# jondo2010/rust-ida

Hardware: AMD Instinct MI355X
Metric: Newton iters/sec (fp64), batched dense DAE N=512 B=4096 (higher is better)
Workload: dtype f64

## Files before the change

### bindings/rust/ida-hip-sys/src/lib.rs

```rust
#![allow(non_camel_case_types, non_upper_case_globals)]
use std::os::raw::{c_char, c_double, c_int, c_long, c_void};

#[repr(C)]
pub struct idahip_ctx {
    _private: [u8; 0],
}
#[repr(C)]
pub struct idaens {
    _private: [u8; 0],
}

pub type idahip_res_fn = Option<
    unsafe extern "C" fn(sys: c_int, tt: c_double, yy: *const c_double, yp: *const c_double, resval: *mut c_double, user: *mut c_void) -> c_int,
>;
pub type idahip_jac_fn = Option<
    unsafe extern "C" fn(
        sys: c_int,
        tt: c_double,
        cj: c_double,
        yy: *const c_double,
        yp: *const c_double,
        resvec: *const c_double,
        jac: *mut c_double,
        user: *mut c_void,
    ) -> c_int,
>;
pub type idahip_band_jac_fn = Option<
    unsafe extern "C" fn(
        sys: c_int,
        tt: c_double,
        cj: c_double,
        yy: *const c_double,
        yp: *const c_double,
        resvec: *const c_double,
        jac: *mut c_double,
        ldab: c_int,
        user: *mut c_void,
    ) -> c_int,
>;
pub type idaens_root_fn = Option<
    unsafe extern "C" fn(user: *mut c_void, sys: i32, t: c_double, yy: *const c_double, yp: *const c_double, nroots: i32, gout: *mut c_double) -> c_int,
>;

#[repr(C)]
pub struct idahip_root_state {
    pub glo: [c_double; 4],
    pub ghi: [c_double; 4],
    pub grout: [c_double; 4],
    pub iroots: [c_double; 4],
    pub gactive: [i32; 4],
}

#[repr(C)]
pub struct idahip_tiny_call {
    pub touts: *const c_double,
    pub ntout: c_int,
    pub recycle: c_int,
    pub resume: c_int,
    pub max_rounds: c_long,
    pub mxstep: c_long,
    pub maxord: c_int,
    pub maxnef: c_long,
    pub maxncf: c_long,
    pub epcon: c_double,
    pub hmax_inv: c_double,
    pub t0: c_double,
    pub start_round: *const i64,
    pub round_base: i64,
    pub nroots: c_int,
    pub root_comps: *const i32,
    pub root_thresholds: *const c_double,
    pub root_states: *mut idahip_root_state,
}

pub const IDAHIP_ROBERTS: c_int = 0;
pub const IDAHIP_LORENZ63: c_int = 1;
pub const IDAHIP_LINEAR_DENSE: c_int = 2;
pub const IDAHIP_HEAT1D: c_int = 3;
pub const IDAHIP_HOST_CALLBACK: c_int = 4;
pub const IDAHIP_F_YY: c_int = 0;
pub const IDAHIP_F_YP: c_int = 1;
pub const IDAHIP_F_YYPREDICT: c_int = 2;
pub const IDAHIP_F_YPPREDICT: c_int = 3;
pub const IDAHIP_F_EWT: c_int = 4;
pub const IDAHIP_F_EE: c_int = 5;
pub const IDAHIP_F_DELTA: c_int = 6;
pub const IDAHIP_F_SAVRES: c_int = 7;
pub const IDAHIP_F_PHI0: c_int = 8;
pub const IDAHIP_F_PHI5: c_int = 13;
pub const IDAHIP_LS_DIRECT: c_int = 0;
pub const IDAHIP_LS_ITERATIVE: c_int = 1;
pub const IDAHIP_LS_MATRIX_ITERATIVE: c_int = 2;
pub const IDAHIP_K_NEWTON_ITER: c_int = 0;
pub const IDAHIP_K_SYS: c_int = 1;
pub const IDAHIP_K_JAC: c_int = 2;
pub const IDAHIP_K_LU: c_int = 3;
pub const IDAHIP_K_VECTOR: c_int = 4;
pub const IDAHIP_K_SOLVE: c_int = 5;
pub const IDAHIP_K_SYS_JAC: c_int = 6;
pub const IDAHIP_K_LU_PANEL: c_int = 7;
pub const IDAHIP_K_LU_TRAIL: c_int = 8;
pub const IDAHIP_K_LU_FINALIZE: c_int = 9;
pub const IDAHIP_K_COUNT: c_int = 10;

pub const IDAENS_NORMAL: c_int = 0;
pub const IDAENS_ONE_STEP: c_int = 1;
pub const IDAENS_SUCCESS: c_int = 0;
pub const IDAENS_TSTOP_RETURN: c_int = 1;
pub const IDAENS_ROOT_RETURN: c_int = 2;
pub const IDAENS_UNFINISHED: c_int = 99;
pub const IDAENS_TOO_MUCH_WORK: c_int = -1;
pub const IDAENS_TOO_MUCH_ACC: c_int = -2;
pub const IDAENS_ERR_FAIL: c_int = -3;
pub const IDAENS_CONV_FAIL: c_int = -4;
pub const IDAENS_LSETUP_FAIL: c_int = -6;
pub const IDAENS_CLOSE_ROOTS: c_int = -10;
pub const IDAENS_RTFUNC_FAIL: c_int = -12;
pub const IDAENS_ILL_INPUT: c_int = -22;
pub const IDAENS_BAD_K: c_int = -25;
pub const IDAENS_BAD_T: c_int = -26;
pub const IDAENS_C_NST: c_int = 0;
pub const IDAENS_C_NRE: c_int = 1;
pub const IDAENS_C_NJE: c_int = 2;
pub const IDAENS_C_NSETUPS: c_int = 3;
pub const IDAENS_C_NNI: c_int = 4;
pub const IDAENS_C_NETF: c_int = 5;
pub const IDAENS_C_NCFN: c_int = 6;
pub const IDAENS_C_NATTEMPTS: c_int = 7;
pub const IDAENS_C_NLS_NCONVFAILS: c_int = 8;
pub const IDAENS_C_KUSED: c_int = 9;
pub const IDAENS_C_KK: c_int = 10;
pub const IDAENS_C_NGE: c_int = 11;
pub const IDAENS_C_NLUFAIL: c_int = 12;
pub const IDAENS_C_NCONV_JCUR: c_int = 13;
pub const IDAENS_C_NFAIL_FIRST: c_int = 14;
pub const IDAENS_C_NLI: c_int = 15;
pub const IDAENS_C_NCFL: c_int = 16;
pub const IDAENS_C_NRE_DQ: c_int = 17;
pub const IDAENS_R_TN: c_int = 0;
pub const IDAENS_R_HUSED: c_int = 1;
pub const IDAENS_R_HH: c_int = 2;
pub const IDAENS_R_H0U: c_int = 3;
pub const IDAENS_R_TOLSF: c_int = 4;

#[link(name = "idahip")]
extern "C" {
    pub fn idahip_create(ctx: *mut *mut idahip_ctx, device: c_int, n: c_int, batch: c_int, kind: c_int, hip_stream: *mut c_void) -> c_int;
    pub fn idahip_destroy(ctx: *mut idahip_ctx) -> c_int;
    pub fn idahip_create_band(ctx: *mut *mut idahip_ctx, device: c_int, n: c_int, batch: c_int, kind: c_int, hip_stream: *mut c_void, ml: c_int, mu: c_int) -> c_int;
    pub fn idahip_band(ctx: *const idahip_ctx, ml: *mut c_int, mu: *mut c_int) -> c_int;
    pub fn idahip_set_host_band_problem(ctx: *mut idahip_ctx, res: idahip_res_fn, bjac: idahip_band_jac_fn, user: *mut c_void) -> c_int;
    pub fn idahip_download_lu_band(ctx: *mut idahip_ctx, sys: c_int, h_ab: *mut c_double, h_piv: *mut i64) -> c_int;
    pub fn idahip_ls_setup_band(ctx: *mut idahip_ctx, ml: c_int, mu: c_int, d_ab: *mut c_double, d_piv: *mut i64, h_info: *mut i32, h_idx: *const i32, nsys: c_int) -> c_int;
    pub fn idahip_ls_solve_band(ctx: *mut idahip_ctx, ml: c_int, mu: c_int, d_ab: *const c_double, d_piv: *const i64, d_x: *mut c_double, d_b: *const c_double, tol: c_double, h_idx: *const i32, nsys: c_int) -> c_int;
    pub fn idahip_concurrent_streams(device: c_int, count: c_int, streams_out: *mut *mut c_void, nconcurrent: *mut c_int) -> c_int;
    pub fn idahip_release_streams(device: c_int, count: c_int, streams: *mut *mut c_void) -> c_int;
    pub fn idahip_stream_pair_share(device: c_int, stream_a: *mut c_void, stream_b: *mut c_void, frac: *mut c_double) -> c_int;
    pub fn idahip_last_error(ctx: *const idahip_ctx) -> *const c_char;
    pub fn idahip_sync(ctx: *mut idahip_ctx) -> c_int;
    pub fn idahip_n(ctx: *const idahip_ctx) -> c_int;
    pub fn idahip_batch(ctx: *const idahip_ctx) -> c_int;
    pub fn idahip_kind(ctx: *const idahip_ctx) -> c_int;
    pub fn idahip_set_tolerances(ctx: *mut idahip_ctx, rtol: c_double, h_atol: *const c_double, natol: c_int) -> c_int;
    pub fn idahip_set_problem_params(ctx: *mut idahip_ctx, first: c_int, count: c_int, h_params: *const c_double, nparam: c_int) -> c_int;
    pub fn idahip_set_linear_dense(ctx: *mut idahip_ctx, first: c_int, count: c_int, h_a: *const c_double, h_b: *const c_double, h_c: *const c_double) -> c_int;
    pub fn idahip_set_host_problem(ctx: *mut idahip_ctx, res: idahip_res_fn, jac: idahip_jac_fn, user: *mut c_void) -> c_int;
    pub fn idahip_upload(ctx: *mut idahip_ctx, f: c_int, first: c_int, count: c_int, h: *const c_double) -> c_int;
    pub fn idahip_download(ctx: *mut idahip_ctx, f: c_int, first: c_int, count: c_int, h: *mut c_double) -> c_int;
    pub fn idahip_download_lu(ctx: *mut idahip_ctx, sys: c_int, h_lu: *mut c_double, h_piv: *mut i64) -> c_int;
    pub fn idahip_dev_alloc(ctx: *mut idahip_ctx, bytes: usize) -> *mut c_void;
    pub fn idahip_dev_free(ctx: *mut idahip_ctx, d: *mut c_void) -> c_int;
    pub fn idahip_memcpy_h2d(ctx: *mut idahip_ctx, d: *mut c_void, h: *const c_void, bytes: usize) -> c_int;
    pub fn idahip_memcpy_d2h(ctx: *mut idahip_ctx, h: *mut c_void, d: *const c_void, bytes: usize) -> c_int;
    pub fn idahip_ls_setup(ctx: *mut idahip_ctx, d_a: *mut c_double, d_piv: *mut i64, h_info: *mut i32, h_idx: *const i32, nsys: c_int) -> c_int;
    pub fn idahip_ls_solve(ctx: *mut idahip_ctx, d_lu: *const c_double, d_piv: *const i64, d_x: *mut c_double, d_b: *const c_double, tol: c_double, h_idx: *const i32, nsys: c_int) -> c_int;
    pub fn idahip_ls_type(ctx: *const idahip_ctx) -> c_int;
    pub fn idahip_ls_num_iters(ctx: *const idahip_ctx) -> c_int;
    pub fn idahip_ls_res_norm(ctx: *const idahip_ctx) -> c_double;
    pub fn idahip_wrms(ctx: *mut idahip_ctx, d_x: *const c_double, d_w: *const c_double, h_out: *mut c_double, h_idx: *const i32, nsys: c_int) -> c_int;
    pub fn idahip_nls_sys_setup(ctx: *mut idahip_ctx, h_tn: *const c_double, h_cj: *const c_double, reset_ee: c_int, h_info: *mut i32, h_idx: *const i32, nsys: c_int) -> c_int;
    pub fn idahip_nls_sys(ctx: *mut idahip_ctx, h_tn: *const c_double, h_cj: *const c_double, reset_ee: c_int, h_idx: *const i32, nsys: c_int) -> c_int;
    pub fn idahip_nls_lsetup(ctx: *mut idahip_ctx, h_tn: *const c_double, h_cj: *const c_double, h_info: *mut i32, h_idx: *const i32, nsys: c_int) -> c_int;
    pub fn idahip_set_jacobian_dq(ctx: *mut idahip_ctx, on: c_int) -> c_int;
    pub fn idahip_jacobian_dq(ctx: *const idahip_ctx) -> c_int;
    pub fn idahip_set_host_residual(ctx: *mut idahip_ctx, res: idahip_res_fn, user: *mut c_void) -> c_int;
    pub fn idahip_nls_lsetup_dq(ctx: *mut idahip_ctx, h_tn: *const c_double, h_cj: *const c_double, h_hh: *const c_double, h_info: *mut i32, h_idx: *const i32, nsys: c_int) -> c_int;
    pub fn idahip_jac_dq(ctx: *mut idahip_ctx, h_tn: *const c_double, h_cj: *const c_double, h_hh: *const c_double, h_j: *mut c_double, h_idx: *const i32, nsys: c_int) -> c_int;
    pub fn idahip_newton_iter(ctx: *mut idahip_ctx, h_scale: *const c_double, h_delnrm: *mut c_double, h_idx: *const i32, nsys: c_int) -> c_int;
    pub fn idahip_newton_iter2(ctx: *mut idahip_ctx, h_scale: *const c_double, h_tn: *const c_double, h_cj: *const c_double, h_toldel: *const c_double, h_ss: *const c_double, h_eps_newt: *const c_double, h_delnrm: *mut c_double, h_conv: *mut i32, h_idx: *const i32, nsys: c_int) -> c_int;
    pub fn idahip_init_first(ctx: *mut idahip_ctx, h_ypnorm: *mut c_double, h_phi0_nrm: *mut c_double, h_idx: *const i32, nsys: c_int) -> c_int;
    pub fn idahip_scale_phi1(ctx: *mut idahip_ctx, h_fac: *const c_double, h_idx: *const i32, nsys: c_int) -> c_int;
    pub fn idahip_predict(ctx: *mut idahip_ctx, h_kk_ns: *const i32, h_beta: *const c_double, h_gamma: *const c_double, h_idx: *const i32, nsys: c_int) -> c_int;
    pub fn idahip_post_newton(ctx: *mut idahip_ctx, h_cj: *const c_double, h_kk: *const i32, h_norms: *mut c_double, h_idx: *const i32, nsys: c_int) -> c_int;
    pub fn idahip_restore(ctx: *mut idahip_ctx, h_kk_ns: *const i32, h_cvals: *const c_double, h_idx: *const i32, nsys: c_int) -> c_int;
    pub fn idahip_complete_step(ctx: *mut idahip_ctx, h_kused: *const i32, h_ck: *const c_double, maxord: c_int, h_phi0_nrm: *mut c_double, h_ewt_bad: *mut i32, h_idx: *const i32, nsys: c_int) -> c_int;
    pub fn idahip_get_solution(ctx: *mut idahip_ctx, h_kord: *const i32, h_cvals: *const c_double, h_dvals: *const c_double, h_idx: *const i32, nsys: c_int) -> c_int;
    pub fn idahip_get_dky(ctx: *mut idahip_ctx, h_kfirst: *const i32, h_klast: *const i32, h_cjk: *const c_double, h_out: *mut c_double, h_idx: *const i32, nsys: c_int) -> c_int;
    pub fn idahip_snapshot_initial(ctx: *mut idahip_ctx) -> c_int;
    pub fn idahip_restore_initial(ctx: *mut idahip_ctx, h_idx: *const i32, nsys: c_int) -> c_int;
    pub fn idahip_tiny_solve(ctx: *mut idahip_ctx, h_sys: *mut c_void, sys_bytes: usize, call: *const idahip_tiny_call, h_rounds_done: *mut i64, h_acc: *mut u64, h_yout: *mut c_double, h_ypout: *mut c_double) -> c_int;
    pub fn idahip_pow_batch(ctx: *mut idahip_ctx, h_x: *const c_double, h_y: *const c_double, h_out: *mut c_double, count: usize) -> c_int;
    pub fn idahip_round_solve(ctx: *mut idahip_ctx, h_sys: *mut c_void, sys_bytes: usize, call: *const idahip_tiny_call, h_rounds_done: *mut i64, h_acc: *mut u64, h_yout: *mut c_double, h_ypout: *mut c_double, rounds_run: *mut i64) -> c_int;
    pub fn idahip_set_lu_variant(ctx: *mut idahip_ctx, variant: c_int) -> c_int;
    pub fn idahip_lu_variant(ctx: *const idahip_ctx) -> c_int;
    pub fn idahip_set_lu_superpanel(ctx: *mut idahip_ctx, on: c_int) -> c_int;
    pub fn idahip_lu_superpanel(ctx: *const idahip_ctx) -> c_int;
    pub fn idahip_set_lu_period(ctx: *mut idahip_ctx, rounds: c_int) -> c_int;
    pub fn idahip_lu_period(ctx: *const idahip_ctx) -> c_int;
    pub fn idahip_timing_build() -> c_int;
    pub fn idahip_timing_enable(ctx: *mut idahip_ctx, on: c_int) -> c_int;
    pub fn idahip_timing_get(ctx: *mut idahip_ctx, k: c_int, ms: *mut c_double, launches: *mut i64, systems: *mut i64) -> c_int;
    pub fn idahip_timing_reset(ctx: *mut idahip_ctx) -> c_int;
}

#[link(name = "idaens")]
extern "C" {
    pub fn idaens_create(e: *mut *mut idaens, ctx: *mut idahip_ctx, h_yy0: *const c_double, h_yp0: *const c_double) -> c_int;
    pub fn idaens_destroy(e: *mut idaens) -> c_int;
    pub fn idaens_last_error(e: *const idaens) -> *const c_char;
    pub fn idaens_set_max_num_steps(e: *mut idaens, mxstep: c_long) -> c_int;
    pub fn idaens_set_max_ord(e: *mut idaens, maxord: c_int) -> c_int;
    pub fn idaens_set_fused_newton(e: *mut idaens, on: c_int) -> c_int;
    pub fn idaens_set_device_controller(e: *mut idaens, on: c_int) -> c_int;
    pub fn idaens_device_controller_active(e: *const idaens) -> c_int;
    pub fn idaens_set_roots(e: *mut idaens, nroots: c_int, comps: *const i32, thresholds: *const c_double) -> c_int;
    pub fn idaens_get_roots(e: *const idaens, out: *mut i32) -> c_int;
    pub fn idaens_set_root_fn(e: *mut idaens, nroots: c_int, fn_: idaens_root_fn, user: *mut c_void) -> c_int;
    pub fn idaens_solve(e: *mut idaens, tout: c_double, itask: c_int, h_tret: *mut c_double, h_status: *mut i32, max_rounds: c_long) -> c_int;
    pub fn idaens_solve_schedule(e: *mut idaens, touts: *const c_double, ntout: c_int, h_tret: *mut c_double, h_status: *mut i32, h_reached: *mut i32, h_yout: *mut c_double, h_ypout: *mut c_double, max_rounds: c_long) -> c_int;
    pub fn idaens_stream(e: *mut idaens, touts: *const c_double, ntout: c_int, max_rounds: c_long, stagger_rounds: c_long, passes_done: *mut i64) -> c_int;
    pub fn idaens_stream_group(ens: *mut *mut idaens, ngroups: c_int, touts: *const c_double, ntout: c_int, max_rounds: c_long, stagger_rounds: c_long, offset_us: c_long, passes_done: *mut i64) -> c_int;
    pub fn idaens_solve_schedule_group(ens: *mut *mut idaens, ngroups: c_int, touts: *const c_double, ntout: c_int, h_tret: *mut *mut c_double, h_status: *mut *mut i32, h_reached: *mut *mut i32, max_rounds: c_long) -> c_int;
    pub fn idaens_get_counter(e: *const idaens, which: c_int, out: *mut i64) -> c_int;
    pub fn idaens_get_real(e: *const idaens, which: c_int, out: *mut c_double) -> c_int;
    pub fn idaens_get_yy(e: *mut idaens, h_yy: *mut c_double) -> c_int;
    pub fn idaens_get_yp(e: *mut idaens, h_yp: *mut c_double) -> c_int;
    pub fn idaens_get_dky(e: *mut idaens, t: c_double, k: c_int, h_dky: *mut c_double, h_status: *mut i32) -> c_int;
    pub fn idaens_total_newton_iters(e: *const idaens) -> i64;
    pub fn idaens_total_rounds(e: *const idaens) -> i64;
    pub fn idaens_trace_system(e: *mut idaens, sys: c_int) -> c_int;
    pub fn idaens_trace_len(e: *const idaens) -> c_long;
    pub fn idaens_trace_get(e: *const idaens, out: *mut c_double) -> c_int;
}
```

### include/ida_hip.h

```cpp
#ifndef IDA_HIP_H
#define IDA_HIP_H

#include <stddef.h>
#include <stdint.h>

#ifdef __cplusplus
extern "C" {
#endif

typedef struct idahip_ctx idahip_ctx;

typedef enum {
    IDAHIP_ROBERTS = 0,
    IDAHIP_LORENZ63 = 1,
    IDAHIP_LINEAR_DENSE = 2,
    IDAHIP_HEAT1D = 3,
    IDAHIP_HOST_CALLBACK = 4
} idahip_problem;

typedef int (*idahip_res_fn)(int sys, double tt, const double* yy, const double* yp, double* resval, void* user);
typedef int (*idahip_jac_fn)(int sys, double tt, double cj, const double* yy, const double* yp, const double* resvec, double* J,
                             void* user);

typedef int (*idahip_band_jac_fn)(int sys, double tt, double cj, const double* yy, const double* yp, const double* resvec, double* AB,
                                  int ldab, void* user);

typedef enum {
    IDAHIP_F_YY = 0,
    IDAHIP_F_YP = 1,
    IDAHIP_F_YYPREDICT = 2,
    IDAHIP_F_YPPREDICT = 3,
    IDAHIP_F_EWT = 4,
    IDAHIP_F_EE = 5,
    IDAHIP_F_DELTA = 6,
    IDAHIP_F_SAVRES = 7,
    IDAHIP_F_PHI0 = 8,
    IDAHIP_F_PHI5 = 13
} idahip_field;

int idahip_create(idahip_ctx** ctx, int device, int n, int batch, idahip_problem kind, void* hip_stream );
int idahip_destroy(idahip_ctx* ctx);
int idahip_create_band(idahip_ctx** ctx, int device, int n, int batch, idahip_problem kind, void* hip_stream, int ml, int mu);
int idahip_band(const idahip_ctx* ctx, int* ml, int* mu);
int idahip_set_host_band_problem(idahip_ctx* ctx, idahip_res_fn res, idahip_band_jac_fn bjac, void* user);
int idahip_download_lu_band(idahip_ctx* ctx, int sys, double* hAB, int64_t* hPiv);
int idahip_ls_setup_band(idahip_ctx* ctx, int ml, int mu, double* dAB, int64_t* dPiv, int32_t* hInfo, const int32_t* hIdx, int nsys);
int idahip_ls_solve_band(idahip_ctx* ctx, int ml, int mu, const double* dAB, const int64_t* dPiv, double* dX, const double* dB, double tol,
                         const int32_t* hIdx, int nsys);
int idahip_concurrent_streams(int device, int count, void** streams_out, int* nconcurrent);
int idahip_release_streams(int device, int count, void** streams);
int idahip_stream_pair_share(int device, void* streamA, void* streamB, double* frac);
const char* idahip_last_error(const idahip_ctx* ctx);
int idahip_sync(idahip_ctx* ctx);
int idahip_n(const idahip_ctx* ctx);
int idahip_batch(const idahip_ctx* ctx);
int idahip_kind(const idahip_ctx* ctx);

int idahip_set_tolerances(idahip_ctx* ctx, double rtol, const double* hAtol, int natol);
int idahip_set_problem_params(idahip_ctx* ctx, int first, int count, const double* hParams, int nparam);
int idahip_set_linear_dense(idahip_ctx* ctx, int first, int count, const double* hA, const double* hB, const double* hC);
int idahip_set_host_problem(idahip_ctx* ctx, idahip_res_fn res, idahip_jac_fn jac, void* user);
int idahip_upload(idahip_ctx* ctx, idahip_field f, int first, int count, const double* h);
int idahip_download(idahip_ctx* ctx, idahip_field f, int first, int count, double* h);
int idahip_download_lu(idahip_ctx* ctx, int sys, double* hLU, int64_t* hPiv);

void* idahip_dev_alloc(idahip_ctx* ctx, size_t bytes);
int idahip_dev_free(idahip_ctx* ctx, void* d);
int idahip_memcpy_h2d(idahip_ctx* ctx, void* d, const void* h, size_t bytes);
int idahip_memcpy_d2h(idahip_ctx* ctx, void* h, const void* d, size_t bytes);

int idahip_ls_setup(idahip_ctx* ctx, double* dA, int64_t* dPiv, int32_t* hInfo, const int32_t* hIdx, int nsys);
int idahip_ls_solve(idahip_ctx* ctx, const double* dLU, const int64_t* dPiv, double* dX, const double* dB, double tol,
                    const int32_t* hIdx, int nsys);
typedef enum { IDAHIP_LS_DIRECT = 0, IDAHIP_LS_ITERATIVE = 1, IDAHIP_LS_MATRIX_ITERATIVE = 2 } idahip_ls_kind;
int idahip_ls_type(const idahip_ctx* ctx);
int idahip_ls_num_iters(const idahip_ctx* ctx);
double idahip_ls_res_norm(const idahip_ctx* ctx);
int idahip_wrms(idahip_ctx* ctx, const double* dX, const double* dW, double* hOut, const int32_t* hIdx, int nsys);

int idahip_nls_sys_setup(idahip_ctx* ctx, const double* hTn, const double* hCj, int reset_ee, int32_t* hInfo,
                         const int32_t* hIdx, int nsys);

int idahip_nls_sys(idahip_ctx* ctx, const double* hTn, const double* hCj, int reset_ee, const int32_t* hIdx, int nsys);
int idahip_nls_lsetup(idahip_ctx* ctx, const double* hTn, const double* hCj, int32_t* hInfo, const int32_t* hIdx, int nsys);

int idahip_set_jacobian_dq(idahip_ctx* ctx, int on);
int idahip_jacobian_dq(const idahip_ctx* ctx);
int idahip_set_host_residual(idahip_ctx* ctx, idahip_res_fn res, void* user);
int idahip_nls_lsetup_dq(idahip_ctx* ctx, const double* hTn, const double* hCj, const double* hHh, int32_t* hInfo, const int32_t* hIdx,
                         int nsys);
int idahip_jac_dq(idahip_ctx* ctx, const double* hTn, const double* hCj, const double* hHh, double* hJ, const int32_t* hIdx, int nsys);
int idahip_newton_iter(idahip_ctx* ctx, const double* hScale, double* hDelnrm, const int32_t* hIdx, int nsys);
int idahip_newton_iter2(idahip_ctx* ctx, const double* hScale, const double* hTn, const double* hCj, const double* hToldel,
                        const double* hSs, const double* hEpsNewt, double* hDelnrm, int32_t* hConv, const int32_t* hIdx, int nsys);

int idahip_init_first(idahip_ctx* ctx, double* hYpnorm, double* hPhi0Nrm, const int32_t* hIdx, int nsys);
int idahip_scale_phi1(idahip_ctx* ctx, const double* hFac, const int32_t* hIdx, int nsys);
int idahip_predict(idahip_ctx* ctx, const int32_t* hKkNs, const double* hBeta, const double* hGamma, const int32_t* hIdx, int nsys);
int idahip_post_newton(idahip_ctx* ctx, const double* hCj, const int32_t* hKk, double* hNorms, const int32_t* hIdx, int nsys);
int idahip_restore(idahip_ctx* ctx, const int32_t* hKkNs, const double* hCvals, const int32_t* hIdx, int nsys);
int idahip_complete_step(idahip_ctx* ctx, const int32_t* hKused, const double* hCk, int maxord, double* hPhi0Nrm,
                         int32_t* hEwtBad, const int32_t* hIdx, int nsys);
int idahip_get_solution(idahip_ctx* ctx, const int32_t* hKord, const double* hCvals, const double* hDvals,
                        const int32_t* hIdx, int nsys);
int idahip_get_dky(idahip_ctx* ctx, const int32_t* hKfirst, const int32_t* hKlast, const double* hCjk , double* hOut,
                   const int32_t* hIdx, int nsys);

int idahip_snapshot_initial(idahip_ctx* ctx);
int idahip_restore_initial(idahip_ctx* ctx, const int32_t* hIdx, int nsys);

#define IDAHIP_MAX_ROOTS 4
typedef struct idahip_root_state {
    double glo[IDAHIP_MAX_ROOTS], ghi[IDAHIP_MAX_ROOTS], grout[IDAHIP_MAX_ROOTS], iroots[IDAHIP_MAX_ROOTS];
    int32_t gactive[IDAHIP_MAX_ROOTS];
} idahip_root_state;
typedef struct idahip_tiny_call {
    const double* touts;
    int ntout;
    int recycle;
    int resume;
    long max_rounds;
    long mxstep;
    int maxord;
    long maxnef, maxncf;
    double epcon, hmax_inv, t0;
    const int64_t* start_round;
    int64_t round_base;
    int nroots;
    const int32_t* root_comps;
    const double* root_thresholds;
    idahip_root_state* root_states;
} idahip_tiny_call;
int idahip_tiny_solve(idahip_ctx* ctx, void* hSys, size_t sys_bytes, const idahip_tiny_call* call, int64_t* hRoundsDone, uint64_t* hAcc,
                      double* hYout, double* hYPout);
int idahip_pow_batch(idahip_ctx* ctx, const double* hX, const double* hY, double* hOut, size_t count);
int idahip_round_solve(idahip_ctx* ctx, void* hSys, size_t sys_bytes, const idahip_tiny_call* call, int64_t* hRoundsDone, uint64_t* hAcc,
                       double* hYout, double* hYPout, int64_t* rounds_run);

int idahip_set_lu_variant(idahip_ctx* ctx, int variant);
int idahip_lu_variant(const idahip_ctx* ctx);
int idahip_set_lu_superpanel(idahip_ctx* ctx, int on);
int idahip_lu_superpanel(const idahip_ctx* ctx);
int idahip_set_lu_period(idahip_ctx* ctx, int rounds);
int idahip_lu_period(const idahip_ctx* ctx);
int idahip_timing_build(void);

typedef enum {
    IDAHIP_K_NEWTON_ITER = 0, IDAHIP_K_SYS = 1, IDAHIP_K_JAC = 2, IDAHIP_K_LU = 3, IDAHIP_K_VECTOR = 4, IDAHIP_K_SOLVE = 5,
    IDAHIP_K_SYS_JAC = 6,
    IDAHIP_K_LU_PANEL = 7,
    IDAHIP_K_LU_TRAIL = 8,
    IDAHIP_K_LU_FINALIZE = 9,
    IDAHIP_K_COUNT = 10
} idahip_kclass;
int idahip_timing_enable(idahip_ctx* ctx, int on);
int idahip_timing_get(idahip_ctx* ctx, idahip_kclass k, double* ms, int64_t* launches, int64_t* systems);
int idahip_timing_reset(idahip_ctx* ctx);

#ifdef __cplusplus
}
#endif
#endif
```

### rust-ida_amd/csrc/common.hpp

```cpp
#pragma once
#include <hip/hip_runtime.h>

#include <cstdarg>
#include <cstdlib>
#include <cstdint>
#include <cstdio>
#include <cstring>
#include <string>
#include <type_traits>
#include <vector>

#include "../../include/ida_hip.h"
#include "exp_switches.hpp"

namespace idahip {

constexpr int MXORDP1 = 6;
constexpr int TINY_N = 8;
constexpr int LU_NB = 32;
constexpr int LU_MAX_N = 1024;
constexpr int LU_WIDE_ROWS = 2048;
constexpr int LU_ZMAP_MIN_N = 2048;
constexpr int LU_BIG_MAX_N = 4096;
constexpr int NSLOT = 8;

struct Slot {
    char* h = nullptr;
    char* d = nullptr;
    hipEvent_t done = nullptr;
    bool pending = false;
};

}

struct idahip_ctx {
    int device = 0;
    int n = 0;
    int batch = 0;
    int npad16 = 0;
    int simds = 0;
    idahip_problem kind = IDAHIP_ROBERTS;
    hipStream_t stream = nullptr;
    bool own_stream = false;
    std::string err;

    double rtol = 0.0;
    double atol_s = 0.0;
    double* d_atol_v = nullptr;

    double *yy = nullptr, *yp = nullptr, *yypredict = nullptr, *yppredict = nullptr, *ewt = nullptr, *ee = nullptr,
           *delta = nullptr, *savres = nullptr;
    double* phi = nullptr;

    double* lu = nullptr;
    double* jw = nullptr;
    int64_t* piv = nullptr;
    int32_t* perm = nullptr;
    int32_t *lu_pos = nullptr, *lu_live = nullptr, *lu_prow = nullptr, *lu_info = nullptr, *lu_redo = nullptr, *lu_nzb = nullptr, *lu_bz = nullptr;
    int32_t* lu_jwzero = nullptr;
    uint8_t* lu_dirty = nullptr;
    uint8_t* lu_zmap = nullptr;
    double* lu_l11 = nullptr;
    int band = 0, ml = 0, mu = 0, ldab = 0;
    double* bab = nullptr;
    double *ic_y = nullptr, *ic_yp = nullptr;
    double* dky = nullptr;
    int lu_variant = 4;
    int lu_superpanel = 0;
    int lu_period = 1;

    void* tiny_sys = nullptr;
    double *tiny_touts = nullptr, *tiny_yout = nullptr, *tiny_ypout = nullptr;
    int64_t *tiny_start = nullptr, *tiny_rounds = nullptr;
    uint64_t* tiny_acc = nullptr;
    void* tiny_roots = nullptr;
    int tiny_ntout_cap = 0, tiny_yout_cap = 0;

    int32_t* rnd_i = nullptr;
    double* rnd_d = nullptr;
    int32_t* rnd_host = nullptr;

    unsigned long long* dbg_stamps = nullptr;

    double* params = nullptr;
    int nparam = 0;
    double *A = nullptr, *B = nullptr, *C = nullptr;
    idahip_res_fn cb_res = nullptr;
    idahip_jac_fn cb_jac = nullptr;
    idahip_band_jac_fn cb_bjac = nullptr;
    void* cb_user = nullptr;
    double* cb_stage = nullptr;
    std::vector<double> cb_host;
    double *cb_jpin = nullptr, *cb_jdev = nullptr;
    size_t cb_jcap = 0;
    int jac_dq = 0;
    int dq_locked = 0;
    double* dq_stage = nullptr;
    size_t dq_stage_cap = 0;
    double* dq_out = nullptr;
    size_t dq_out_cap = 0;
    double* dq_hh = nullptr;

    std::vector<uint64_t> list_seen;

    idahip::Slot slots[idahip::NSLOT];
    size_t slot_cap = 0;
    int next_slot = 0;

    int timing = 0;
    hipEvent_t ev0 = nullptr, ev1 = nullptr, ev2 = nullptr, ev3 = nullptr;
    hipEvent_t ev_cnt = nullptr;
    double k_ms[IDAHIP_K_COUNT] = {0};
    int64_t k_launches[IDAHIP_K_COUNT] = {0};
    int64_t k_systems[IDAHIP_K_COUNT] = {0};
};

namespace idahip {

inline int fail(idahip_ctx* c, int code, const char* fmt, ...) {
    char buf[512];
    va_list ap;
    va_start(ap, fmt);
    vsnprintf(buf, sizeof buf, fmt, ap);
    va_end(ap);
    if (c) c->err = buf;
    return code;
}

#define IDAHIP_HIP(c, call)                                                                              \
    do {                                                                                                 \
        hipError_t e__ = (call);                                                                         \
        if (e__ != hipSuccess) return idahip::fail((c), -100, "%s failed: %s", #call, hipGetErrorString(e__)); \
    } while (0)

struct DevGuard {
    int prev = -1;
    bool switched = false;
    explicit DevGuard(int dev) {
        if (dev >= 0 && hipGetDevice(&prev) == hipSuccess && prev != dev) switched = hipSetDevice(dev) == hipSuccess;
    }
    explicit DevGuard(const idahip_ctx* c) : DevGuard(c ? c->device : -1) {}
    ~DevGuard() {
        if (switched) (void)hipSetDevice(prev);
    }
    DevGuard(const DevGuard&) = delete;
    DevGuard& operator=(const DevGuard&) = delete;
};

struct ArgPack {
    idahip_ctx* c;
    Slot* s;
    size_t in_bytes = 0;
    size_t off = 0;
    size_t out_begin = 0, out_end = 0;
    bool overflow = false;

    int begin(idahip_ctx* ctx) {
        c = ctx;
        s = &ctx->slots[ctx->next_slot];
        ctx->next_slot = (ctx->next_slot + 1) % NSLOT;
        if (s->pending) {
            IDAHIP_HIP(c, hipEventSynchronize(s->done));
            s->pending = false;
        }
        off = 0;
        return 0;
    }
    static size_t align(size_t x) { return (x + 63) & ~(size_t)63; }
    template <class T>
    const T* in(const T* src, size_t count) {
        off = align(off);
        if (off + count * sizeof(T) > c->slot_cap) {
            overflow = true;
            return (const T*)s->d;
        }
        memcpy(s->h + off, src, count * sizeof(T));
        const T* d = (const T*)(s->d + off);
        off += count * sizeof(T);
        in_bytes = off;
        return d;
    }
    int upload() {
        if (overflow) return fail(c, -5, "argument staging slot too small (%zu bytes)", c->slot_cap);
        if (in_bytes) IDAHIP_HIP(c, hipMemcpyAsync(s->d, s->h, in_bytes, hipMemcpyHostToDevice, c->stream));
        return 0;
    }
    template <class T>
    T* out(size_t count) {
        off = align(off);
        if (off + count * sizeof(T) > c->slot_cap) {
            overflow = true;
            return nullptr;
        }
        if (out_begin == 0 && out_end == 0) out_begin = off;
        T* d = (T*)(s->d + off);
        off += count * sizeof(T);
        out_end = off;
        return d;
    }
    template <class T>
    const T* host_of(const T* dptr) const { return (const T*)(s->h + ((const char*)dptr - s->d)); }
    int ok() { return overflow ? fail(c, -5, "argument staging slot too small (%zu bytes)", c->slot_cap) : 0; }
    int fetch() {
        if (overflow) return ok();
        if (out_end > out_begin)
            IDAHIP_HIP(c, hipMemcpyAsync(s->h + out_begin, s->d + out_begin, out_end - out_begin, hipMemcpyDeviceToHost, c->stream));
        IDAHIP_HIP(c, hipStreamSynchronize(c->stream));
        return 0;
    }
    int finish_async() {
        IDAHIP_HIP(c, hipEventRecord(s->done, c->stream));
        s->pending = true;
        return 0;
    }
};

struct KTimer {
    idahip_ctx* c;
    idahip_kclass k;
    bool on;
    hipEvent_t e0, e1;
    KTimer(idahip_ctx* ctx, idahip_kclass kc, int nsys) : c(ctx), k(kc) {
        const bool sub = kc >= IDAHIP_K_LU_PANEL;
        on = sub ? c->timing >= 2 : c->timing >= 1;
        e0 = sub ? c->ev2 : c->ev0;
        e1 = sub ? c->ev3 : c->ev1;
        c->k_launches[k] += 1;
        c->k_systems[k] += nsys;
        if (on) (void)hipEventRecord(e0, c->stream);
    }
    ~KTimer() {
        if (on) {
            (void)hipEventRecord(e1, c->stream);
            (void)hipEventSynchronize(e1);
            float ms = 0.f;
            (void)hipEventElapsedTime(&ms, e0, e1);
            c->k_ms[k] += (double)ms;
        }
    }
};

template <class T>
__device__ __forceinline__ T ldc(const T* p) {
    typedef const T __attribute__((address_space(4))) * cptr;
    return *reinterpret_cast<cptr>(reinterpret_cast<uintptr_t>(p));
}

__device__ __forceinline__ double readlane_f64(double v, int lane ) {
    const int lo = __builtin_amdgcn_readlane(__double2loint(v), lane);
    const int hi = __builtin_amdgcn_readlane(__double2hiint(v), lane);
    return __hiloint2double(hi, lo);
}

template <int CTRL, int ROW_MASK>
__device__ __forceinline__ int dpp_mov_i32(int x) {
    return __builtin_amdgcn_update_dpp(x, x, CTRL, ROW_MASK, 0xf, false);
}
template <int CTRL, int ROW_MASK>
__device__ __forceinline__ double dpp_mov_f64(double x) {
    const int lo = dpp_mov_i32<CTRL, ROW_MASK>(__double2loint(x));
    const int hi = dpp_mov_i32<CTRL, ROW_MASK>(__double2hiint(x));
    return __hiloint2double(hi, lo);
}
__device__ __forceinline__ double wave_max_f64(double v) {
    double o;
    o = dpp_mov_f64<0x111, 0xf>(v); v = o > v ? o : v;
    o = dpp_mov_f64<0x112, 0xf>(v); v = o > v ? o : v;
    o = dpp_mov_f64<0x114, 0xf>(v); v = o > v ? o : v;
    o = dpp_mov_f64<0x118, 0xf>(v); v = o > v ? o : v;
    o = dpp_mov_f64<0x142, 0xa>(v); v = o > v ? o : v;
    o = dpp_mov_f64<0x143, 0xc>(v); v = o > v ? o : v;
    const int lo = __builtin_amdgcn_readlane(__double2loint(v), 63);
    const int hi = __builtin_amdgcn_readlane(__double2hiint(v), 63);
    return __hiloint2double(hi, lo);
}
__device__ __forceinline__ int wave_min_i32(int v) {
    int o;
    o = dpp_mov_i32<0x111, 0xf>(v); v = o < v ? o : v;
    o = dpp_mov_i32<0x112, 0xf>(v); v = o < v ? o : v;
    o = dpp_mov_i32<0x114, 0xf>(v); v = o < v ? o : v;
    o = dpp_mov_i32<0x118, 0xf>(v); v = o < v ? o : v;
    o = dpp_mov_i32<0x142, 0xa>(v); v = o < v ? o : v;
    o = dpp_mov_i32<0x143, 0xc>(v); v = o < v ? o : v;
    return __builtin_amdgcn_readlane(v, 63);
}

template <int CTRL, int ROW_MASK>
__device__ __forceinline__ unsigned dpp_umax(unsigned x) {
    const unsigned o = (unsigned)__builtin_amdgcn_update_dpp(0, (int)x, CTRL, ROW_MASK, 0xf, true);
    return o > x ? o : x;
}
template <int CTRL, int ROW_MASK>
__device__ __forceinline__ int dpp_imin(int x) {
    const int o = __builtin_amdgcn_update_dpp(0x7fffffff, x, CTRL, ROW_MASK, 0xf, false);
    return o < x ? o : x;
}
template <bool ROWS16>
__device__ __forceinline__ unsigned wave_max_u32(unsigned v) {
    v = dpp_umax<0x111, 0xf>(v);
    v = dpp_umax<0x112, 0xf>(v);
    v = dpp_umax<0x114, 0xf>(v);
    v = dpp_umax<0x118, 0xf>(v);
    if (ROWS16) return (unsigned)__builtin_amdgcn_readlane((int)v, 15);
    v = dpp_umax<0x142, 0xa>(v);
    v = dpp_umax<0x143, 0xc>(v);
    return (unsigned)__builtin_amdgcn_readlane((int)v, 63);
}
template <bool ROWS16>
__device__ __forceinline__ int wave_min_i32f(int v) {
    v = dpp_imin<0x111, 0xf>(v);
    v = dpp_imin<0x112, 0xf>(v);
    v = dpp_imin<0x114, 0xf>(v);
    v = dpp_imin<0x118, 0xf>(v);
    if (ROWS16) return __builtin_amdgcn_readlane(v, 15);
    v = dpp_imin<0x142, 0xa>(v);
    v = dpp_imin<0x143, 0xc>(v);
    return __builtin_amdgcn_readlane(v, 63);
}

template <int I, int N, class F>
__device__ __forceinline__ void static_for(F&& f) {
    if constexpr (I < N) {
        f(std::integral_constant<int, I>{});
        static_for<I + 1, N>(f);
    }
}

__device__ __forceinline__ double upd(double a, double u, double l) { return a - u * l; }

__device__ __forceinline__ double buf_load_f64(__amdgpu_buffer_rsrc_t rsrc, unsigned voffset, int soffset) {
    typedef unsigned v2u __attribute__((ext_vector_type(2)));
    const v2u r = __builtin_amdgcn_raw_buffer_load_b64(rsrc, (int)voffset, soffset, 0);
    return __hiloint2double((int)r.y, (int)r.x);
}

__device__ __forceinline__ void buf_store_f64(__amdgpu_buffer_rsrc_t rsrc, unsigned voffset, int soffset, double v) {
    typedef unsigned v2u __attribute__((ext_vector_type(2)));
    v2u d;
    d.x = (unsigned)__double2loint(v);
    d.y = (unsigned)__double2hiint(v);
    __builtin_amdgcn_raw_buffer_store_b64(d, rsrc, (int)voffset, soffset, 0);
}

__device__ __forceinline__ double shfl_xor_f64(double v, int mask) {
    const int lo = __shfl_xor(__double2loint(v), mask);
    const int hi = __shfl_xor(__double2hiint(v), mask);
    return __hiloint2double(hi, lo);
}

}
```

### rust-ida_amd/csrc/idahip.hip

```cpp
#include "common.hpp"
#include "lu_kernels.hpp"
#include "lu_driver.hpp"
#include "problem_kernels.hpp"
#include "solve_kernels.hpp"
#include "band_kernels.hpp"
#include "dq_kernels.hpp"
#include "vector_kernels.hpp"
#include "tiny_ida.hpp"
#include "round_ida.hpp"

using namespace idahip;

namespace {

template <class T>
int dalloc(idahip_ctx* c, T** p, size_t count) {
    *p = nullptr;
    if (count == 0) return 0;
    IDAHIP_HIP(c, hipMalloc((void**)p, count * sizeof(T)));
    return 0;
}

int check_list(idahip_ctx* c, const int32_t* hIdx, int nsys) {
    if (!c) return -1;
    if (nsys < 0 || nsys > c->batch) return fail(c, -2, "nsys = %d out of range (batch = %d)", nsys, c->batch);
    if (nsys > 0 && !hIdx) return fail(c, -2, "null system list");
    for (int s = 0; s < nsys; ++s)
        if (hIdx[s] < 0 || hIdx[s] >= c->batch) return fail(c, -2, "system id %d out of range at list position %d", hIdx[s], s);
    uint64_t* seen = c->list_seen.data();
    int dup = -1;
    for (int s = 0; s < nsys && dup < 0; ++s) {
        const uint64_t bit = 1ull << (hIdx[s] & 63);
        if (seen[hIdx[s] >> 6] & bit) dup = s;
        seen[hIdx[s] >> 6] |= bit;
    }
    for (int s = 0; s < (dup < 0 ? nsys : dup); ++s) seen[hIdx[s] >> 6] = 0;
    if (dup >= 0) return fail(c, -2, "system id %d listed twice (again at list position %d)", hIdx[dup], dup);
    return 0;
}

double* field_ptr(idahip_ctx* c, idahip_field f) {
    switch (f) {
        case IDAHIP_F_YY: return c->yy;
        case IDAHIP_F_YP: return c->yp;
        case IDAHIP_F_YYPREDICT: return c->yypredict;
        case IDAHIP_F_YPPREDICT: return c->yppredict;
        case IDAHIP_F_EWT: return c->ewt;
        case IDAHIP_F_EE: return c->ee;
        case IDAHIP_F_DELTA: return c->delta;
        case IDAHIP_F_SAVRES: return c->savres;
        default: break;
    }
    if (f >= IDAHIP_F_PHI0 && f <= IDAHIP_F_PHI5) return c->phi + (size_t)(f - IDAHIP_F_PHI0) * c->batch * c->n;
    return nullptr;
}

VecState vec_state(idahip_ctx* c) {
    VecState s;
    s.phi = c->phi;
    s.phistride = (long)c->batch * c->n;
    s.yy = c->yy; s.yp = c->yp; s.yypredict = c->yypredict; s.yppredict = c->yppredict;
    s.ewt = c->ewt; s.ee = c->ee; s.delta = c->delta;
    s.n = c->n;
    s.rtol = c->rtol; s.atol_s = c->atol_s; s.atol_v = c->d_atol_v;
    return s;
}

int post_launch(idahip_ctx* c, const char* what) {
    hipError_t e = hipGetLastError();
    if (e != hipSuccess) return fail(c, -101, "launch of %s failed: %s", what, hipGetErrorString(e));
    return 0;
}

int band_spw(const idahip_ctx* c, int nsys) {
    int spw = 64;
    const int simds = c->simds > 0 ? c->simds : 1024;
    while (spw > 1 && (long)(nsys + spw / 2 - 1) / (spw / 2) <= simds) spw >>= 1;
    if (const char* e = std::getenv("IDAHIP_BAND_SPW")) {
        const int v = (int)std::strtol(e, nullptr, 10);
        if (v == 1 || v == 2 || v == 4 || v == 8 || v == 16 || v == 32 || v == 64) spw = v;
    }
    return spw;
}

int band_factor(idahip_ctx* c, double* dAB, long sstride, int64_t* dPiv, long pstride, int ml, int mu, const int* d_idx, int nsys,
                const int* d_cnt = nullptr) {
    if (nsys == 0) return 0;
    BandArgs g;
    g.ab = dAB; g.sstride = sstride; g.piv = (long long*)dPiv; g.pstride = pstride; g.n = c->n; g.ml = ml; g.mu = mu;
    g.idx = d_idx; g.nsys = nsys; g.cnt = d_cnt; g.info = c->lu_info;
    const int spw = band_spw(c, nsys);
    const dim3 grid((nsys + spw - 1) / spw), blk(spw);
    if (ml == 1 && mu == 1) hipLaunchKernelGGL((band_getrf_reg_kernel<1, 1>), grid, blk, 0, c->stream, g);
    else hipLaunchKernelGGL(band_getrf_kernel, grid, blk, 0, c->stream, g);
    return post_launch(c, "band_getrf");
}

int create_ctx(idahip_ctx** out, int device, int n, int batch, idahip_problem kind, void* hip_stream, bool band, int ml, int mu) {
    if (!out) return -1;
    *out = nullptr;
    if (n < 1 || batch < 1) return -2;
    if ((int)kind < 0 || (int)kind > (int)IDAHIP_HOST_CALLBACK) return -2;
    if ((kind == IDAHIP_ROBERTS || kind == IDAHIP_LORENZ63) && n != 3) return -2;
    idahip_ctx* c = new idahip_ctx();
    c->device = device; c->n = n; c->batch = batch; c->kind = kind;
    if (band) {
        c->band = 1; c->ml = ml; c->mu = mu; c->ldab = 2 * ml + mu + 1;
    }
    c->npad16 = (n + 15) & ~15;
    c->list_seen.assign(((size_t)batch + 63) / 64, 0);
    c->lu_superpanel = kind == IDAHIP_HEAT1D ? 1 : 0;
    if (const char* sp = std::getenv("IDAHIP_LU_SUPERPANEL")) c->lu_superpanel = std::strtol(sp, nullptr, 10) != 0 ? 1 : 0;
    if (const char* sp = std::getenv("IDAHIP_LU_PERIOD")) {
        const int v = (int)std::strtol(sp, nullptr, 10);
        if (v >= 1 && v <= 64) c->lu_period = v;
    }
    int ndev = 0;
    if (device < 0 || hipGetDeviceCount(&ndev) != hipSuccess || device >= ndev) { delete c; return -100; }
    DevGuard dev_guard__(device);
    if (hipSetDevice(device) != hipSuccess) { delete c; return -100; }
    {
        int cus = 0;
        if (hipDeviceGetAttribute(&cus, hipDeviceAttributeMultiprocessorCount, device) == hipSuccess && cus > 0) c->simds = 4 * cus;
    }
    if (hip_stream) {
        c->stream = (hipStream_t)hip_stream;
    } else {
        if (hipStreamCreate(&c->stream) != hipSuccess) { delete c; return -100; }
        c->own_stream = true;
    }
    const size_t bn = (size_t)batch * n, bnn = bn * n;
    int rc = 0;
    rc |= dalloc(c, &c->yy, bn); rc |= dalloc(c, &c->yp, bn); rc |= dalloc(c, &c->yypredict, bn); rc |= dalloc(c, &c->yppredict, bn);
    rc |= dalloc(c, &c->ewt, bn); rc |= dalloc(c, &c->ee, bn); rc |= dalloc(c, &c->delta, bn); rc |= dalloc(c, &c->savres, bn);
    rc |= dalloc(c, &c->phi, (size_t)MXORDP1 * bn);
    rc |= dalloc(c, &c->piv, bn); rc |= dalloc(c, &c->perm, bn);
    rc |= dalloc(c, &c->lu_info, (size_t)batch);
    rc |= dalloc(c, &c->lu_redo, (size_t)batch);
    rc |= dalloc(c, &c->lu_nzb, (size_t)batch);
    if (band) rc |= dalloc(c, &c->bab, bn * c->ldab);
    if (!band) rc |= dalloc(c, &c->lu, bnn);
    if (!band && n > LU_MAX_N) rc |= dalloc(c, &c->lu_bz, (size_t)batch * 64);
    if (!band && n >= LU_ZMAP_MIN_N) rc |= dalloc(c, &c->lu_zmap, (size_t)batch * 4096);
    if (!band && n >= LU_ZMAP_MIN_N) rc |= dalloc(c, &c->lu_dirty, (size_t)batch * 4096);
    if (!band && n >= LU_ZMAP_MIN_N) rc |= dalloc(c, &c->lu_jwzero, (size_t)batch);
    if (!band && n > TINY_N) {
        rc |= dalloc(c, &c->jw, bnn);
        rc |= dalloc(c, &c->lu_pos, bn); rc |= dalloc(c, &c->lu_live, bn); rc |= dalloc(c, &c->lu_prow, bn);
        rc |= dalloc(c, &c->lu_l11, (size_t)batch * L11_STRIDE);
    }
    if (kind == IDAHIP_LINEAR_DENSE) {
        rc |= dalloc(c, &c->A, bnn); rc |= dalloc(c, &c->B, bnn); rc |= dalloc(c, &c->C, bn);
    }
    if (kind == IDAHIP_LORENZ63) { c->nparam = 3; rc |= dalloc(c, &c->params, (size_t)batch * 3); }
    if (kind == IDAHIP_HEAT1D) { c->nparam = 1; rc |= dalloc(c, &c->params, (size_t)batch); }
    if (kind == IDAHIP_HOST_CALLBACK) rc |= dalloc(c, &c->cb_stage, 3 * bn);
    c->slot_cap = (size_t)batch * 256 + 4096;
    for (int i = 0; i < NSLOT && !rc; ++i) {
        if (hipHostMalloc((void**)&c->slots[i].h, c->slot_cap) != hipSuccess) rc = -100;
        else if (hipMalloc((void**)&c->slots[i].d, c->slot_cap) != hipSuccess) rc = -100;
        else if (hipEventCreateWithFlags(&c->slots[i].done, hipEventDisableTiming) != hipSuccess) rc = -100;
    }
    if (!rc && (hipEventCreate(&c->ev0) != hipSuccess || hipEventCreate(&c->ev1) != hipSuccess || hipEventCreate(&c->ev2) != hipSuccess ||
                hipEventCreate(&c->ev3) != hipSuccess || hipEventCreateWithFlags(&c->ev_cnt, hipEventDisableTiming) != hipSuccess))
        rc = -100;

    if (rc) {
        idahip_destroy(c);
        return -100;
    }
    (void)hipMemsetAsync(c->ee, 0, bn * sizeof(double), c->stream);
    (void)hipMemsetAsync(c->delta, 0, bn * sizeof(double), c->stream);
    (void)hipMemsetAsync(c->phi, 0, (size_t)MXORDP1 * bn * sizeof(double), c->stream);
    (void)hipMemsetAsync(c->lu_info, 0, (size_t)batch * sizeof(int), c->stream);
    (void)hipMemsetAsync(c->piv, 0, bn * sizeof(int64_t), c->stream);
    (void)hipMemsetAsync(c->perm, 0, bn * sizeof(int32_t), c->stream);
    (void)hipMemsetAsync(c->lu_redo, 0, (size_t)batch * sizeof(int), c->stream);
    if (c->bab) (void)hipMemsetAsync(c->bab, 0, bn * c->ldab * sizeof(double), c->stream);
    if (c->lu_dirty) {
        (void)hipMemsetAsync(c->lu, 0, bnn * sizeof(double), c->stream);
        (void)hipMemsetAsync(c->lu_dirty, 0, (size_t)batch * 4096, c->stream);
        (void)hipMemsetAsync(c->lu_jwzero, 0, (size_t)batch * sizeof(int), c->stream);
    }
    (void)hipStreamSynchronize(c->stream);
    *out = c;
    return 0;
}

}

extern "C" {

int idahip_create(idahip_ctx** out, int device, int n, int batch, idahip_problem kind, void* hip_stream) {
    return create_ctx(out, device, n, batch, kind, hip_stream, false, 0, 0);
}

int idahip_create_band(idahip_ctx** out, int device, int n, int batch, idahip_problem kind, void* hip_stream, int ml, int mu) {
    if (!out) return -1;
    *out = nullptr;
    if (kind != IDAHIP_HEAT1D && kind != IDAHIP_HOST_CALLBACK) {
        std::fprintf(stderr, "idahip_create_band: problem kind %d has no band form (IDAHIP_HEAT1D or IDAHIP_HOST_CALLBACK)\n", (int)kind);
        return -2;
    }
    if (n <= TINY_N || n > LU_BIG_MAX_N) {
        std::fprintf(stderr, "idahip_create_band: n = %d outside %d < n <= %d\n", n, TINY_N, LU_BIG_MAX_N);
        return -2;
    }
    if (ml < 0 || mu < 0 || ml >= n || mu >= n || (kind == IDAHIP_HEAT1D && (ml < 1 || mu < 1))) {
        std::fprintf(stderr, "idahip_create_band: bandwidths ml = %d, mu = %d outside 0 <= ml, mu < n (>= 1 for IDAHIP_HEAT1D)\n", ml, mu);
        return -2;
    }
    return create_ctx(out, device, n, batch, kind, hip_stream, true, ml, mu);
}

int idahip_band(const idahip_ctx* c, int* ml, int* mu) {
    if (!c) return -1;
    if (c->band) {
        if (ml) *ml = c->ml;
        if (mu) *mu = c->mu;
    }
    return c->band;
}

int idahip_destroy(idahip_ctx* c) {
    DevGuard dev_guard__(c);
    if (!c) return 0;
    if (c->stream) (void)hipStreamSynchronize(c->stream);
    void* ptrs[] = {c->dq_stage, c->dq_out, c->dq_hh, c->yy, c->yp, c->yypredict, c->yppredict, c->ewt, c->ee, c->delta, c->savres, c->phi, c->lu, c->jw, c->piv, c->perm,
                    c->lu_pos, c->lu_live, c->lu_prow, c->lu_info, c->lu_redo, c->lu_nzb, c->lu_bz, c->lu_zmap, c->lu_dirty, c->lu_jwzero, c->lu_l11, c->params, c->A, c->B, c->C, c->d_atol_v, c->ic_y,
                    c->ic_yp, c->bab, c->dky, c->cb_stage, c->tiny_sys, c->tiny_touts, c->tiny_yout, c->tiny_ypout, c->tiny_start, c->tiny_rounds,
                    c->tiny_acc, c->tiny_roots, c->rnd_i, c->rnd_d};
    for (void* p : ptrs)
        if (p) (void)hipFree(p);
    if (c->rnd_host) (void)hipHostFree(c->rnd_host);
    if (c->cb_jpin) (void)hipHostFree(c->cb_jpin);
    if (c->cb_jdev) (void)hipFree(c->cb_jdev);
    for (int i = 0; i < NSLOT; ++i) {
        if (c->slots[i].h) (void)hipHostFree(c->slots[i].h);
        if (c->slots[i].d) (void)hipFree(c->slots[i].d);
        if (c->slots[i].done) (void)hipEventDestroy(c->slots[i].done);
    }
    if (c->ev0) (void)hipEventDestroy(c->ev0);
    if (c->ev1) (void)hipEventDestroy(c->ev1);
    if (c->ev2) (void)hipEventDestroy(c->ev2);
    if (c->ev3) (void)hipEventDestroy(c->ev3);
    if (c->ev_cnt) (void)hipEventDestroy(c->ev_cnt);
    if (c->own_stream && c->stream) (void)hipStreamDestroy(c->stream);
    delete c;
    return 0;
}

const char* idahip_last_error(const idahip_ctx* c) { return c ? c->err.c_str() : "null ctx"; }
int idahip_n(const idahip_ctx* c) { return c ? c->n : -1; }
int idahip_batch(const idahip_ctx* c) { return c ? c->batch : -1; }

int idahip_sync(idahip_ctx* c) {
    DevGuard dev_guard__(c);
    if (!c) return -1;
    IDAHIP_HIP(c, hipStreamSynchronize(c->stream));
    return 0;
}

__global__ void stream_probe_kernel(unsigned long long* out, long long ticks) {
    const unsigned long long t0 = wall_clock64();
    while ((long long)(wall_clock64() - t0) < ticks) __builtin_amdgcn_s_sleep(16);
    if (threadIdx.x == 0) {
        out[0] = t0;
        out[1] = wall_clock64();
    }
}

int idahip_concurrent_streams(int device, int count, void** streams_out, int* nconcurrent) {
    if (!streams_out || count < 1 || count > 64) return -2;
    int ndev = 0;
    if (device < 0 || hipGetDeviceCount(&ndev) != hipSuccess || device >= ndev) return -100;
    DevGuard dev_guard__(device);
    if (hipSetDevice(device) != hipSuccess) return -100;
    unsigned long long* stamps = nullptr;
    if (hipHostMalloc((void**)&stamps, sizeof(unsigned long long) * 2 * (size_t)(count + 1)) != hipSuccess) return -100;
    std::vector<hipStream_t> sel, rejected;
    int rc = 0;
    const long long ticks = 30000;
    for (int attempt = 0; attempt < 6 * count + 8 && (int)sel.size() < count && !rc; ++attempt) {
        hipStream_t s = nullptr;
        if (hipStreamCreateWithFlags(&s, hipStreamNonBlocking) != hipSuccess) { rc = -100; break; }
        if (sel.empty()) {
            sel.push_back(s);
            continue;
        }
        const int k = (int)sel.size();
        for (int i = 0; i <= k; ++i) stamps[2 * i] = stamps[2 * i + 1] = 0ull;
        for (int i = 0; i < k; ++i) hipLaunchKernelGGL(stream_probe_kernel, dim3(1), dim3(64), 0, sel[i], stamps + 2 * i, ticks);
        hipLaunchKernelGGL(stream_probe_kernel, dim3(1), dim3(64), 0, s, stamps + 2 * k, ticks);
        bool ok = hipGetLastError() == hipSuccess;
        for (int i = 0; i < k; ++i) ok = (hipStreamSynchronize(sel[i]) == hipSuccess) && ok;
        ok = (hipStreamSynchronize(s) == hipSuccess) && ok;
        if (!ok) { rc = -100; (void)hipStreamDestroy(s); break; }
        bool overlaps_all = stamps[2 * k + 1] > stamps[2 * k];
        for (int i = 0; i < k; ++i)
            overlaps_all = overlaps_all && stamps[2 * k] < stamps[2 * i + 1] && stamps[2 * i] < stamps[2 * k + 1];
        (overlaps_all ? sel : rejected).push_back(s);
    }
    const int found = (int)sel.size();
    while (!rc && (int)sel.size() < count) {
        if (!rejected.empty()) {
            sel.push_back(rejected.back());
            rejected.pop_back();
        } else {
            hipStream_t s = nullptr;
            if (hipStreamCreateWithFlags(&s, hipStreamNonBlocking) != hipSuccess) rc = -100;
            else sel.push_back(s);
        }
    }
    for (hipStream_t s : rejected) (void)hipStreamDestroy(s);
    (void)hipHostFree(stamps);
    if (rc) {
        for (hipStream_t s : sel) (void)hipStreamDestroy(s);
        return rc;
    }
    for (int i = 0; i < count; ++i) streams_out[i] = (void*)sel[i];
    if (nconcurrent) *nconcurrent = found;
    return 0;
}

__global__ void stream_share_kernel(unsigned long long* out, long long ticks) {
    extern __shared__ unsigned char pad_lds[];
    const unsigned long long t0 = wall_clock64();
    if (threadIdx.x == 0) pad_lds[0] = 1;
    while ((long long)(wall_clock64() - t0) < ticks) __builtin_amdgcn_s_sleep(16);
    if (threadIdx.x == 0) {
        atomicMin(out, t0);
        atomicMax(out + 1, wall_clock64());
    }
}

int idahip_stream_pair_share(int device, void* streamA, void* streamB, double* frac) {
    if (!streamA || !streamB || !frac) return -2;
    DevGuard dev_guard__(device);
    unsigned long long* st = nullptr;
    if (hipHostMalloc((void**)&st, 4 * sizeof(unsigned long long)) != hipSuccess) return -100;
    st[0] = st[2] = ~0ull;
    st[1] = st[3] = 0ull;
    static bool attr_set = false;
    if (!attr_set) {
        (void)hipFuncSetAttribute((const void*)stream_share_kernel, hipFuncAttributeMaxDynamicSharedMemorySize, 65536);
        attr_set = true;
    }
    hipLaunchKernelGGL(stream_share_kernel, dim3(2048), dim3(64), 65536, (hipStream_t)streamA, st, 2000ll);
    hipLaunchKernelGGL(stream_share_kernel, dim3(2048), dim3(64), 65536, (hipStream_t)streamB, st + 2, 2000ll);
    int rc = hipGetLastError() == hipSuccess ? 0 : -100;
    if (hipStreamSynchronize((hipStream_t)streamA) != hipSuccess) rc = -100;
    if (hipStreamSynchronize((hipStream_t)streamB) != hipSuccess) rc = -100;
    if (!rc) {
        const double lo = (double)(st[0] < st[2] ? st[0] : st[2]), hi = (double)(st[1] > st[3] ? st[1] : st[3]);
        const double olo = (double)(st[0] > st[2] ? st[0] : st[2]), ohi = (double)(st[1] < st[3] ? st[1] : st[3]);
        *frac = hi > lo ? (ohi > olo ? (ohi - olo) / (hi - lo) : 0.0) : 0.0;
    }
    (void)hipHostFree(st);
    return rc;
}

int idahip_release_streams(int device, int count, void** streams) {
    if (!streams || count < 0) return -2;
    DevGuard dev_guard__(device);
    int rc = 0;
    for (int i = 0; i < count; ++i)
        if (streams[i] && hipStreamDestroy((hipStream_t)streams[i]) != hipSuccess) rc = -100;
    return rc;
}

int idahip_set_tolerances(idahip_ctx* c, double rtol, const double* hAtol, int natol) {
    DevGuard dev_guard__(c);
    if (!c || !hAtol) return -1;
    if (natol != 1 && natol != c->n) return fail(c, -2, "natol must be 1 or n");
    c->rtol = rtol;
    if (natol == 1 && c->n != 1) {
        c->atol_s = hAtol[0];
        if (c->d_atol_v) { (void)hipFree(c->d_atol_v); c->d_atol_v = nullptr; }
    } else {
        c->atol_s = hAtol[0];
        if (!c->d_atol_v) { int rc = dalloc(c, &c->d_atol_v, (size_t)c->n); if (rc) return rc; }
        IDAHIP_HIP(c, hipMemcpy(c->d_atol_v, hAtol, sizeof(double) * c->n, hipMemcpyHostToDevice));
    }
    return 0;
}

int idahip_set_problem_params(idahip_ctx* c, int first, int count, const double* hParams, int nparam) {
    DevGuard dev_guard__(c);
    if (!c || !hParams) return -1;
    if (!c->params || nparam != c->nparam) return fail(c, -2, "problem kind takes %d parameters per system", c->nparam);
    if (first < 0 || count < 0 || first + count > c->batch) return fail(c, -2, "system range out of bounds");
    IDAHIP_HIP(c, hipMemcpy(c->params + (size_t)first * nparam, hParams, sizeof(double) * count * nparam, hipMemcpyHostToDevice));
    return 0;
}

int idahip_set_linear_dense(idahip_ctx* c, int first, int count, const double* hA, const double* hB, const double* hC) {
    DevGuard dev_guard__(c);
    if (!c || !hA || !hB || !hC) return -1;
    if (c->kind != IDAHIP_LINEAR_DENSE) return fail(c, -2, "not a LINEAR_DENSE ctx");
    if (c->band) return fail(c, -2, "idahip_set_linear_dense on a band ctx");
    if (first < 0 || count < 0 || first + count > c->batch) return fail(c, -2, "system range out of bounds");
    const size_t nn = (size_t)c->n * c->n;
    IDAHIP_HIP(c, hipMemcpy(c->A + first * nn, hA, sizeof(double) * count * nn, hipMemcpyHostToDevice));
    IDAHIP_HIP(c, hipMemcpy(c->B + first * nn, hB, sizeof(double) * count * nn, hipMemcpyHostToDevice));
    IDAHIP_HIP(c, hipMemcpy(c->C + (size_t)first * c->n, hC, sizeof(double) * count * c->n, hipMemcpyHostToDevice));
    return 0;
}

int idahip_set_host_problem(idahip_ctx* c, idahip_res_fn res, idahip_jac_fn jac, void* user) {
    if (!c || !res || !jac) return -1;
    if (c->kind != IDAHIP_HOST_CALLBACK) return fail(c, -2, "not an IDAHIP_HOST_CALLBACK ctx");
    if (c->band) return fail(c, -2, "a band ctx takes a band Jacobian: idahip_set_host_band_problem");
    c->cb_res = res;
    c->cb_jac = jac;
    c->cb_bjac = nullptr;
// ... 1007 lines not shown
int idahip_pow_batch(idahip_ctx* c, const double* hX, const double* hY, double* hOut, size_t count) {
    DevGuard dev_guard__(c);
    if (!c) return -1;
    if (!hX || !hY || !hOut) return fail(c, -2, "null argument");
    if (count == 0) return 0;
    double *dx = nullptr, *dy = nullptr, *dout = nullptr;
    int rc = dalloc(c, &dx, count);
    if (!rc) rc = dalloc(c, &dy, count);
    if (!rc) rc = dalloc(c, &dout, count);
    if (!rc) {
        hipError_t e = hipMemcpyAsync(dx, hX, count * sizeof(double), hipMemcpyHostToDevice, c->stream);
        if (e == hipSuccess) e = hipMemcpyAsync(dy, hY, count * sizeof(double), hipMemcpyHostToDevice, c->stream);
        if (e == hipSuccess) {
            hipLaunchKernelGGL(pow_batch_kernel, dim3((unsigned)((count + 255) / 256)), dim3(256), 0, c->stream, (const double*)dx,
                               (const double*)dy, dout, count);
            e = hipMemcpyAsync(hOut, dout, count * sizeof(double), hipMemcpyDeviceToHost, c->stream);
        }
        if (e == hipSuccess) e = hipStreamSynchronize(c->stream);
        if (e != hipSuccess) rc = fail(c, -100, "idahip_pow_batch: %s", hipGetErrorString(e));
    }
    if (dx) (void)hipFree(dx);
    if (dy) (void)hipFree(dy);
    if (dout) (void)hipFree(dout);
    return rc;
}

static int stepper_buffers(idahip_ctx* c, const idahip_tiny_call* call, bool outputs);

static FlowArgs flow_args(idahip_ctx* c, const idahip_tiny_call* call) {
    FlowArgs f;
    f.touts = c->tiny_touts; f.ntout = call->ntout; f.recycle = call->recycle; f.resume = call->resume;
    f.mxstep = call->mxstep; f.maxord = call->maxord; f.maxnef = call->maxnef; f.maxncf = call->maxncf;
    f.epcon = call->epcon; f.hmax_inv = call->hmax_inv; f.t0 = call->t0;
    f.start_round = call->start_round ? (const long long*)c->tiny_start : nullptr;
    f.acc = (unsigned long long*)c->tiny_acc;
    f.batch = c->batch;
    f.nrt = call->nroots;
    for (int i = 0; i < call->nroots && i < IDAHIP_MAX_ROOTS; ++i) {
        f.rt_comp[i] = call->root_comps[i];
        f.rt_thr[i] = call->root_thresholds[i];
    }
    return f;
}

int idahip_tiny_solve(idahip_ctx* c, void* hSys, size_t sys_bytes, const idahip_tiny_call* call, int64_t* hRoundsDone, uint64_t* hAcc,
                      double* hYout, double* hYPout) {
    DevGuard dev_guard__(c);
    if (!c) return -1;
    if (!hSys || !call || !hRoundsDone || !hAcc || !call->touts || call->ntout < 1) return fail(c, -2, "null argument");
    if (sys_bytes != sizeof(idactl::SysCore)) return fail(c, -2, "controller state of %zu bytes, this library expects %zu", sys_bytes, sizeof(idactl::SysCore));
    if (c->n != 3 || (c->kind != IDAHIP_ROBERTS && c->kind != IDAHIP_LORENZ63))
        return fail(c, -2, "the device-resident stepper takes the Roberts and Lorenz63 problems (n = 3)");
    if (call->recycle && (!c->ic_y || !c->ic_yp)) return fail(c, -2, "recycle needs idahip_snapshot_initial");
    if (call->recycle && call->max_rounds < 1) return fail(c, -2, "recycle needs a round limit");
    const int batch = c->batch, n = c->n;
    int rc = stepper_buffers(c, call, hYout || hYPout);
    if (rc) return rc;
    const size_t ysz = (size_t)call->ntout * batch * n;
    IDAHIP_HIP(c, hipMemcpyAsync(c->tiny_sys, hSys, (size_t)batch * sizeof(idactl::SysCore), hipMemcpyHostToDevice, c->stream));
    IDAHIP_HIP(c, hipMemcpyAsync(c->tiny_touts, call->touts, sizeof(double) * call->ntout, hipMemcpyHostToDevice, c->stream));
    if (call->start_round)
        IDAHIP_HIP(c, hipMemcpyAsync(c->tiny_start, call->start_round, sizeof(int64_t) * batch, hipMemcpyHostToDevice, c->stream));
    IDAHIP_HIP(c, hipMemsetAsync(c->tiny_acc, 0, 2 * sizeof(uint64_t), c->stream));
    TinyIdaArgs a;
    a.sys = (idactl::SysCore*)c->tiny_sys;
    a.v = vec_state(c);
    a.savres = c->savres; a.lu = c->lu; a.piv = (long long*)c->piv; a.params = c->params; a.nparam = c->nparam;
    a.ic_y = c->ic_y; a.ic_yp = c->ic_yp;
    a.f = flow_args(c, call);
    a.roots = (idahip_root_state*)c->tiny_roots;
    a.jac_dq = c->jac_dq;
    a.max_rounds = call->max_rounds;
    a.round_base = call->round_base;
    a.yout = hYout ? c->tiny_yout : nullptr;
    a.ypout = hYPout ? c->tiny_ypout : nullptr;
    a.rounds_done = (long long*)c->tiny_rounds;
    {
        KTimer kt(c, IDAHIP_K_VECTOR, batch);
        int spw = 64;
        {
            const int simds = c->simds > 0 ? c->simds : 1024;
            while (spw > 1 && (long)(batch + spw / 2 - 1) / (spw / 2) <= simds / 4) spw >>= 1;
            if (const char* e = std::getenv("IDAHIP_TINY_SPW")) {
                const int v = (int)std::strtol(e, nullptr, 10);
                if (v == 1 || v == 2 || v == 4 || v == 8 || v == 16 || v == 32 || v == 64) spw = v;
            }
        }
        const size_t lds_state = (size_t)spw * sizeof(idactl::SysCore), lds_all = lds_state + (size_t)spw * sizeof(double) * tiny_lds_doubles(n);
        const bool roots = call->nroots > 0;
        auto kern = c->kind == IDAHIP_ROBERTS ? (roots ? tiny_ida_kernel<IDAHIP_ROBERTS, true> : tiny_ida_kernel<IDAHIP_ROBERTS, false>)
                                              : (roots ? tiny_ida_kernel<IDAHIP_LORENZ63, true> : tiny_ida_kernel<IDAHIP_LORENZ63, false>);
        const int lds_vec = hipFuncSetAttribute((const void*)kern, hipFuncAttributeMaxDynamicSharedMemorySize, (int)(64 * (sizeof(idactl::SysCore) + sizeof(double) * tiny_lds_doubles(n)))) == hipSuccess ? 1 : 0;
        if (!lds_vec) (void)hipGetLastError();
        const size_t shm = lds_vec ? lds_all : lds_state;
        hipLaunchKernelGGL(kern, dim3((batch + spw - 1) / spw), dim3(spw), shm, c->stream, a, lds_vec);
        if ((rc = post_launch(c, "tiny_ida"))) return rc;
    }
    IDAHIP_HIP(c, hipMemcpyAsync(hSys, c->tiny_sys, (size_t)batch * sizeof(idactl::SysCore), hipMemcpyDeviceToHost, c->stream));
    if (call->nroots > 0)
        IDAHIP_HIP(c, hipMemcpyAsync(call->root_states, c->tiny_roots, (size_t)batch * sizeof(idahip_root_state), hipMemcpyDeviceToHost, c->stream));
    IDAHIP_HIP(c, hipMemcpyAsync(hRoundsDone, c->tiny_rounds, sizeof(int64_t) * batch, hipMemcpyDeviceToHost, c->stream));
    IDAHIP_HIP(c, hipMemcpyAsync(hAcc, c->tiny_acc, 2 * sizeof(uint64_t), hipMemcpyDeviceToHost, c->stream));
    if (hYout) IDAHIP_HIP(c, hipMemcpyAsync(hYout, c->tiny_yout, sizeof(double) * ysz, hipMemcpyDeviceToHost, c->stream));
    if (hYPout) IDAHIP_HIP(c, hipMemcpyAsync(hYPout, c->tiny_ypout, sizeof(double) * ysz, hipMemcpyDeviceToHost, c->stream));
    IDAHIP_HIP(c, hipStreamSynchronize(c->stream));
    return 0;
}

static int stepper_buffers(idahip_ctx* c, const idahip_tiny_call* call, bool outputs) {
    const int batch = c->batch, n = c->n;
    int rc = 0;
    if (!c->tiny_sys) IDAHIP_HIP(c, hipMalloc(&c->tiny_sys, (size_t)batch * sizeof(idactl::SysCore)));
    if (!c->tiny_start) rc |= dalloc(c, &c->tiny_start, (size_t)batch);
    if (!c->tiny_rounds) rc |= dalloc(c, &c->tiny_rounds, (size_t)batch);
    if (!c->tiny_acc) rc |= dalloc(c, &c->tiny_acc, (size_t)2);
    if (rc) return rc;
    if (call->nroots < 0 || call->nroots > IDAHIP_MAX_ROOTS) return fail(c, -2, "the device steppers take at most %d root functions", IDAHIP_MAX_ROOTS);
    if (call->nroots > 0) {
        if (!call->root_comps || !call->root_thresholds || !call->root_states) return fail(c, -2, "root functions without their arrays");
        for (int i = 0; i < call->nroots; ++i)
            if (call->root_comps[i] < 0 || call->root_comps[i] >= n) return fail(c, -2, "root function %d watches component %d of %d", i, call->root_comps[i], n);
        if (call->recycle) return fail(c, -2, "root finding and idaens_stream's restarts do not combine");
        if (!c->tiny_roots) IDAHIP_HIP(c, hipMalloc(&c->tiny_roots, (size_t)batch * sizeof(idahip_root_state)));
        IDAHIP_HIP(c, hipMemcpyAsync(c->tiny_roots, call->root_states, (size_t)batch * sizeof(idahip_root_state), hipMemcpyHostToDevice, c->stream));
    }
    if (call->ntout > c->tiny_ntout_cap) {
        if (c->tiny_touts) (void)hipFree(c->tiny_touts);
        c->tiny_touts = nullptr;
        if ((rc = dalloc(c, &c->tiny_touts, (size_t)call->ntout))) return rc;
        c->tiny_ntout_cap = call->ntout;
    }
    if (outputs && call->ntout > c->tiny_yout_cap) {
        const size_t ysz = (size_t)call->ntout * batch * n;
        if (c->tiny_yout) (void)hipFree(c->tiny_yout);
        if (c->tiny_ypout) (void)hipFree(c->tiny_ypout);
        c->tiny_yout = c->tiny_ypout = nullptr;
        if ((rc = dalloc(c, &c->tiny_yout, ysz))) return rc;
        if ((rc = dalloc(c, &c->tiny_ypout, ysz))) return rc;
        c->tiny_yout_cap = call->ntout;
    }
    return 0;
}

int idahip_round_solve(idahip_ctx* c, void* hSys, size_t sys_bytes, const idahip_tiny_call* call, int64_t* hRoundsDone, uint64_t* hAcc,
                       double* hYout, double* hYPout, int64_t* rounds_run) {
    DevGuard dev_guard__(c);
    if (!c) return -1;
    if (!hSys || !call || !hRoundsDone || !hAcc || !rounds_run || !call->touts || call->ntout < 1) return fail(c, -2, "null argument");
    if (sys_bytes != sizeof(idactl::SysCore)) return fail(c, -2, "controller state of %zu bytes, this library expects %zu", sys_bytes, sizeof(idactl::SysCore));
    const bool lin = c->kind == IDAHIP_LINEAR_DENSE && c->n <= LU_BIG_MAX_N;
    const bool heat = c->kind == IDAHIP_HEAT1D && c->n <= LU_BIG_MAX_N;
    if (c->n <= TINY_N || !(lin || heat) || c->lu_variant < 4)
        return fail(c, -2, "the device-resident lock-step stepper takes linear dense and heat problems with %d < n <= %d (LU variant 4)", TINY_N, LU_BIG_MAX_N);
    if (call->recycle && (!c->ic_y || !c->ic_yp)) return fail(c, -2, "recycle needs idahip_snapshot_initial");
    if (call->recycle && call->max_rounds < 1) return fail(c, -2, "recycle needs a round limit");
    const int batch = c->batch, n = c->n;
    const long nn = (long)n * n;
    int rc = stepper_buffers(c, call, hYout || hYPout);
    if (rc) return rc;
    if (!c->rnd_i) rc |= dalloc(c, &c->rnd_i, (size_t)8 * batch + 8 + 2 * IDAHIP_K_COUNT);
    if (!c->rnd_d) rc |= dalloc(c, &c->rnd_d, (size_t)4 * batch);
    if (rc) return rc;
    if (!c->rnd_host) IDAHIP_HIP(c, hipHostMalloc((void**)&c->rnd_host, 4 * sizeof(int32_t)));
    const size_t ysz = (size_t)call->ntout * batch * n;
    IDAHIP_HIP(c, hipMemcpyAsync(c->tiny_sys, hSys, (size_t)batch * sizeof(idactl::SysCore), hipMemcpyHostToDevice, c->stream));
    IDAHIP_HIP(c, hipMemcpyAsync(c->tiny_touts, call->touts, sizeof(double) * call->ntout, hipMemcpyHostToDevice, c->stream));
    if (call->start_round)
        IDAHIP_HIP(c, hipMemcpyAsync(c->tiny_start, call->start_round, sizeof(int64_t) * batch, hipMemcpyHostToDevice, c->stream));
    IDAHIP_HIP(c, hipMemsetAsync(c->tiny_acc, 0, 2 * sizeof(uint64_t), c->stream));
    RoundArgs a;
    a.f = flow_args(c, call);
    a.sys = (idactl::SysCore*)c->tiny_sys;
    a.v = vec_state(c);
    a.ic_y = c->ic_y; a.ic_yp = c->ic_yp;
    a.yout = hYout ? c->tiny_yout : nullptr;
    a.ypout = hYPout ? c->tiny_ypout : nullptr;
    a.round_base = call->round_base;
    a.fused_jac = (c->kind == IDAHIP_LINEAR_DENSE && !c->jac_dq) ? 1 : 0;
    if (c->jac_dq && !c->dq_hh && (rc = dalloc(c, &c->dq_hh, (size_t)batch))) return rc;
    a.lu_period = c->lu_period;
    a.roots = (idahip_root_state*)c->tiny_roots;
    int* ib = c->rnd_i;
    a.stepping = ib; a.in_newton = ib + batch; a.skipP = ib + 2 * batch; a.skipL = ib + 3 * batch; a.skipI = ib + 4 * batch;
    a.skipS = ib + 5 * batch; a.ident = ib + 6 * batch; a.lu_list = ib + 7 * batch; a.lu_cnt = ib + 8 * batch; a.summary = ib + 8 * batch + 1; a.lu_wait = ib + 8 * batch + 3;
    a.stats = (unsigned long long*)(ib + 8 * batch + 4);
    if (((uintptr_t)a.stats & 7) != 0) a.stats = (unsigned long long*)(ib + 8 * batch + 5);
    IDAHIP_HIP(c, hipMemsetAsync(a.stats, 0, IDAHIP_K_COUNT * sizeof(unsigned long long), c->stream));
    a.lu_info = c->lu_info;
    a.tn = c->rnd_d; a.cj = c->rnd_d + batch; a.scale = c->rnd_d + 2 * batch; a.nrm_out = c->rnd_d + 3 * batch;
    a.rounds_done = (long long*)c->tiny_rounds;
    hipLaunchKernelGGL(round_init_kernel, dim3((batch + 255) / 256), dim3(256), 0, c->stream, a);
    IDAHIP_HIP(c, hipMemsetAsync(a.summary, 0, 2 * sizeof(int), c->stream));
    const size_t shm_wg = sizeof(double) * (4 * (size_t)n + 8);
    const size_t shm_it = 2 * sizeof(double) * n;
    SysArgs sa;
    fill_sys_args(c, sa, 1);
    sa.idx = a.ident; sa.tn = a.tn; sa.cj = a.cj;
    int64_t r = 0;
    for (;; ++r) {
        if (call->max_rounds > 0 && r >= call->max_rounds) break;
        a.round = r;
        a.first_round = r == 0;
        {
            KTimer kt(c, IDAHIP_K_VECTOR, 0);
            if (call->nroots > 0) hipLaunchKernelGGL(round_begin_kernel<true>, dim3(batch), dim3(WG_NT), shm_wg, c->stream, a);
            else hipLaunchKernelGGL(round_begin_kernel<false>, dim3(batch), dim3(WG_NT), shm_wg, c->stream, a);
            hipLaunchKernelGGL(round_lists_kernel, dim3(1), dim3(1024), 0, c->stream, a);
        }
        const bool lu_cnt_on_host = n > LU_MAX_N && !c->band;
        if (lu_cnt_on_host) {
            IDAHIP_HIP(c, hipMemcpyAsync(c->rnd_host + 2, a.lu_cnt, sizeof(int), hipMemcpyDeviceToHost, c->stream));
            IDAHIP_HIP(c, hipEventRecord(c->ev_cnt, c->stream));
        }
        {
            KTimer kt(c, IDAHIP_K_SYS, 0);
            sa.reset_ee = 1; sa.skip = a.skipP;
            if ((rc = launch_sys(c, sa, batch, nullptr))) return rc;
        }
        if (a.fused_jac) {
            KTimer kt(c, IDAHIP_K_SYS_JAC, 0);
            sa.skip = a.skipL;
            if ((rc = launch_sys(c, sa, batch, c->jw))) return rc;
        } else {
            {
                KTimer kt(c, IDAHIP_K_SYS, 0);
                sa.skip = a.skipL;
                if ((rc = launch_sys(c, sa, batch, nullptr))) return rc;
            }
            KTimer kt(c, IDAHIP_K_JAC, 0);
            if (c->jac_dq)
                hipLaunchKernelGGL(dq_round_prep_kernel, dim3((batch + 255) / 256), dim3(256), 0, c->stream, a.sys, (const int*)a.skipL, c->dq_hh,
                                   batch, dq_evals(c));
            if ((rc = launch_jac(c, c->jw, a.ident, a.cj, batch, nullptr, nullptr, nullptr, a.skipL, c->dq_hh))) return rc;
        }
        {
            int nlu = batch;
            const int* d_cnt = a.lu_cnt;
            if (lu_cnt_on_host) {
                IDAHIP_HIP(c, hipEventSynchronize(c->ev_cnt));
                nlu = c->rnd_host[2];
                d_cnt = nullptr;
                if (nlu < 0 || nlu > batch) return fail(c, -4, "list length %d outside 0..%d", nlu, batch);
            }
            KTimer kt(c, IDAHIP_K_LU, 0);
            if (c->band) rc = band_factor(c, c->bab, (long)c->ldab * n, c->piv, n, c->ml, c->mu, a.lu_list, nlu, d_cnt);
            else rc = lu_factor_batched(c, c->jw, nn, c->lu, nn, (long long*)c->piv, n, c->perm, a.lu_list, nlu, d_cnt);
            if (rc) return rc;
            if ((rc = post_launch(c, "lu"))) return rc;
        }
        hipLaunchKernelGGL(round_newton_ctl_kernel, dim3((batch + 255) / 256), dim3(256), 0, c->stream, a, 0);
        for (int m = 1; m <= idactl::MAXNLSIT; ++m) {
            {
                KTimer kt(c, IDAHIP_K_NEWTON_ITER, 0);
                if ((rc = launch_newton_iter(c, a.ident, a.scale, a.nrm_out, a.skipI, batch))) return rc;
            }
            hipLaunchKernelGGL(round_newton_ctl_kernel, dim3((batch + 255) / 256), dim3(256), 0, c->stream, a, m);
            if (m < idactl::MAXNLSIT) {
                KTimer kt(c, IDAHIP_K_SYS, 0);
                sa.reset_ee = 0; sa.skip = a.skipS;
                if ((rc = launch_sys(c, sa, batch, nullptr))) return rc;
            }
        }
        IDAHIP_HIP(c, hipMemsetAsync(a.summary, 0, sizeof(int), c->stream));
        {
            KTimer kt(c, IDAHIP_K_VECTOR, 0);
            if (call->nroots > 0) hipLaunchKernelGGL(round_end_kernel<true>, dim3(batch), dim3(WG_NT), shm_wg, c->stream, a);
            else hipLaunchKernelGGL(round_end_kernel<false>, dim3(batch), dim3(WG_NT), shm_wg, c->stream, a);
            if ((rc = post_launch(c, "round_end"))) return rc;
        }
        if (!call->recycle) {
            IDAHIP_HIP(c, hipMemcpyAsync(c->rnd_host, a.summary, 2 * sizeof(int), hipMemcpyDeviceToHost, c->stream));
            IDAHIP_HIP(c, hipStreamSynchronize(c->stream));
            if (c->rnd_host[0] == 0) {
                ++r;
                break;
            }
        }
    }
    (void)shm_it;
    *rounds_run = r;
    IDAHIP_HIP(c, hipMemcpyAsync(hSys, c->tiny_sys, (size_t)batch * sizeof(idactl::SysCore), hipMemcpyDeviceToHost, c->stream));
    if (call->nroots > 0)
        IDAHIP_HIP(c, hipMemcpyAsync(call->root_states, c->tiny_roots, (size_t)batch * sizeof(idahip_root_state), hipMemcpyDeviceToHost, c->stream));
    IDAHIP_HIP(c, hipMemcpyAsync(hRoundsDone, c->tiny_rounds, sizeof(int64_t) * batch, hipMemcpyDeviceToHost, c->stream));
    IDAHIP_HIP(c, hipMemcpyAsync(hAcc, c->tiny_acc, 2 * sizeof(uint64_t), hipMemcpyDeviceToHost, c->stream));
    if (hYout) IDAHIP_HIP(c, hipMemcpyAsync(hYout, c->tiny_yout, sizeof(double) * ysz, hipMemcpyDeviceToHost, c->stream));
    if (hYPout) IDAHIP_HIP(c, hipMemcpyAsync(hYPout, c->tiny_ypout, sizeof(double) * ysz, hipMemcpyDeviceToHost, c->stream));
    unsigned long long hstats[IDAHIP_K_COUNT];
    IDAHIP_HIP(c, hipMemcpyAsync(hstats, a.stats, sizeof hstats, hipMemcpyDeviceToHost, c->stream));
    IDAHIP_HIP(c, hipStreamSynchronize(c->stream));
    for (int k = 0; k < IDAHIP_K_COUNT; ++k) c->k_systems[k] += (int64_t)hstats[k];
    c->k_systems[IDAHIP_K_VECTOR] += 2 * r * (int64_t)batch;
    return 0;
}

int idahip_lu_variant(const idahip_ctx* c) { return c ? c->lu_variant : -1; }
int idahip_timing_build(void) { return tb::TIMING_BUILD ? 1 : 0; }
int idahip_set_lu_superpanel(idahip_ctx* c, int on) {
    if (!c) return -1;
    c->lu_superpanel = on != 0 ? 1 : 0;
    return 0;
}
int idahip_lu_superpanel(const idahip_ctx* c) { return c ? c->lu_superpanel : -1; }
int idahip_set_lu_period(idahip_ctx* c, int rounds) {
    if (!c || rounds < 1 || rounds > 64) return -1;
    c->lu_period = rounds;
    return 0;
}
int idahip_lu_period(const idahip_ctx* c) { return c ? c->lu_period : -1; }

int idahip_ls_type(const idahip_ctx* c) { return c ? IDAHIP_LS_DIRECT : -1; }
int idahip_ls_num_iters(const idahip_ctx* c) { return c ? 0 : -1; }
double idahip_ls_res_norm(const idahip_ctx* c) { (void)c; return 0.0; }

#ifdef IDAHIP_STAMPS
void* idahip_debug_stamps(idahip_ctx* c, size_t words) {
    if (!c) return nullptr;
    if (!c->dbg_stamps && hipMalloc((void**)&c->dbg_stamps, words * 8) != hipSuccess) return nullptr;
    (void)hipMemset(c->dbg_stamps, 0, words * 8);
    return c->dbg_stamps;
}
#endif

int idahip_set_lu_variant(idahip_ctx* c, int variant) {
    DevGuard dev_guard__(c);
    if (!c || variant < 3 || variant > 4) return -1;
    c->lu_variant = variant;
    return 0;
}

int idahip_timing_enable(idahip_ctx* c, int on) {
    DevGuard dev_guard__(c);
    if (!c) return -1;
    c->timing = on < 0 ? 0 : (on > 2 ? 2 : on);
    return 0;
}
int idahip_timing_get(idahip_ctx* c, idahip_kclass k, double* ms, int64_t* launches, int64_t* systems) {
    DevGuard dev_guard__(c);
    if (!c || k < 0 || k >= IDAHIP_K_COUNT) return -1;
    if (ms) *ms = c->k_ms[k];
    if (launches) *launches = c->k_launches[k];
    if (systems) *systems = c->k_systems[k];
    return 0;
}
int idahip_timing_reset(idahip_ctx* c) {
    DevGuard dev_guard__(c);
    if (!c) return -1;
    for (int k = 0; k < IDAHIP_K_COUNT; ++k) {
        c->k_ms[k] = 0.0;
        c->k_launches[k] = 0;
        c->k_systems[k] = 0;
    }
    return 0;
}

}
```

### rust-ida_amd/csrc/lu_driver.hpp

```cpp
#pragma once
#include "lu_kernels.hpp"
#include "lu_wavepanel.hpp"
#include "lu_superpanel.hpp"

namespace idahip {

inline int lu_factor_batched(idahip_ctx* c, double* work, long wstride, double* out, long ostride, long long* piv, long pstride,
                             int* perm, const int* d_idx, int nsys, const int* d_cnt = nullptr) {
    const int n = c->n;
    if (nsys == 0) return 0;
    if (n <= TINY_N) {
        hipLaunchKernelGGL(tiny_getrf_kernel, dim3((nsys + 63) / 64), dim3(64), 0, c->stream, work, wstride, d_idx, nsys, n, piv,
                           pstride, perm, c->lu_info);
        return 0;
    }
    if (n > LU_BIG_MAX_N) return fail(c, -3, "blocked LU supports n <= %d in this build (n = %d)", LU_BIG_MAX_N, n);
    if (d_cnt && c->lu_variant < 4) return fail(c, -3, "a device-side list length needs LU variant 4");
    LuWs w;
    w.mats = work; w.mstride = wstride; w.idx = d_idx; w.cnt = d_cnt; w.n = n;
    w.pos = c->lu_pos; w.live = c->lu_live; w.prow = c->lu_prow; w.piv = piv; w.pstride = pstride; w.info = c->lu_info; w.redo = c->lu_redo; w.nzb = c->lu_nzb; w.bz = c->lu_bz;
    w.zmap = (out == c->lu) ? c->lu_zmap : nullptr;
    w.dirty = (out == c->lu) ? c->lu_dirty : nullptr;
    w.jwzero = (w.dirty && work == c->jw && c->lu_superpanel && n > LU_MAX_N) ? c->lu_jwzero : nullptr;
    if (!w.jwzero && c->lu_jwzero && (work == c->jw || out == c->jw))
        (void)hipMemsetAsync(c->lu_jwzero, 0, (size_t)c->batch * sizeof(int), c->stream);
    w.l11 = c->lu_l11; w.stamps = c->dbg_stamps; w.out = out; w.ostride = ostride; w.l11ld = 64;
    hipLaunchKernelGGL(lu_init_kernel, dim3(nsys), dim3(256), 0, c->stream, w);
    const int nsys8 = ((nsys + 7) / 8) * 8;
    constexpr int NB = LU_NB;
    auto panel2 = [&](int k0, int lbase) {
        const int threads = (((n - k0 + 1) / 2 + 63) / 64) * 64;
        hipLaunchKernelGGL((lu_panel2_kernel<NB, 512, 2>), dim3(nsys), dim3(threads), 0, c->stream, w, k0, lbase);
    };
    for (int k0 = 0; k0 < n; k0 += 64) {
        if (n - k0 > LU_MAX_N) {
            KTimer kt(c, IDAHIP_K_LU_PANEL, nsys);
            const int cend = (k0 + 64 < n) ? k0 + 64 : n;
            if (c->lu_superpanel) {
                if (n - k0 > LU_WIDE_ROWS) {
                    const int threads = (((n - k0 + 7) / 8 + 63) / 64) * 64;
                    hipLaunchKernelGGL((lu_superpanel_kernel<8, 512, 2>), dim3(nsys), dim3(threads), 0, c->stream, w, k0);
                } else {
                    const int threads = (((n - k0 + 3) / 4 + 63) / 64) * 64;
                    hipLaunchKernelGGL((lu_superpanel_kernel<4, 512, 2>), dim3(nsys), dim3(threads), 0, c->stream, w, k0);
                }
            } else {
            auto narrow_split = [&](int kk, int nbs) {
                const int ntiles = (n - kk - nbs + 63) / 64;
                return ntiles >= 32 ? 8 : ntiles >= 16 ? 4 : ntiles >= 8 ? 2 : 1;
            };
            if (n - k0 > LU_WIDE_ROWS) {
                constexpr int NBS = 8;
                const int threads = (((n - k0 + 7) / 8 + 63) / 64) * 64;
                for (int lb = 0; lb < 64 && k0 + lb < n; lb += NBS) {
                    hipLaunchKernelGGL((lu_panelr_kernel<NBS, 8, 512, 2>), dim3(nsys), dim3(threads), 0, c->stream, w, k0 + lb, lb);
                    if (k0 + lb + NBS < cend) {
                        const int nsplit = narrow_split(k0 + lb, NBS);
                        hipLaunchKernelGGL((lu_trail_kernel<NBS, LU_BIG_MAX_N, 4>), dim3(nsys8 * nsplit), dim3(256), 0, c->stream, w, k0 + lb, nsys, 1,
                                           cend, lb * 65, nsplit);
                    }
                }
            } else {
                constexpr int NBS = 16;
                const int threads = (((n - k0 + 3) / 4 + 63) / 64) * 64;
                for (int lb = 0; lb < 64 && k0 + lb < n; lb += NBS) {
                    hipLaunchKernelGGL((lu_panelr_kernel<NBS, 4, 512, 2>), dim3(nsys), dim3(threads), 0, c->stream, w, k0 + lb, lb);
                    if (k0 + lb + NBS < cend) {
                        const int nsplit = narrow_split(k0 + lb, NBS);
                        hipLaunchKernelGGL((lu_trail_kernel<NBS, LU_BIG_MAX_N, 4>), dim3(nsys8 * nsplit), dim3(256), 0, c->stream, w, k0 + lb, nsys, 1,
                                           cend, lb * 65, nsplit);
                    }
                }
            }
            }
        } else if (c->lu_superpanel && c->lu_variant >= 4 && n > LU_MAX_N && n - k0 >= 64) {
            KTimer kt(c, IDAHIP_K_LU_PANEL, nsys);
            const int threads = (((n - k0 + 1) / 2 + 63) / 64) * 64;
            hipLaunchKernelGGL((lu_superpanel_kernel<2, 512, 2>), dim3(nsys), dim3(threads), 0, c->stream, w, k0);
        } else if (c->lu_variant >= 4 && n - k0 <= WP_MAX_ROWS) {
            KTimer kt(c, IDAHIP_K_LU_PANEL, nsys);
            const int ns = (n - k0 + 63) / 64;
#define IDAHIP_WP_LAUNCH(NSV) \
    hipLaunchKernelGGL((lu_wavepanel_kernel<false, NSV>), dim3(nsys), dim3(64), 0, c->stream, w, k0)
#define IDAHIP_WP_SWITCH()                                                                                    \
    switch (ns) {                                                                                              \
        case 1: IDAHIP_WP_LAUNCH(1); break;                                                                 \
        case 2: IDAHIP_WP_LAUNCH(2); break;                                                                 \
        case 3: IDAHIP_WP_LAUNCH(3); break;                                                                 \
        case 4: IDAHIP_WP_LAUNCH(4); break;                                                                 \
        case 5: IDAHIP_WP_LAUNCH(5); break;                                                                 \
        case 6: IDAHIP_WP_LAUNCH(6); break;                                                                 \
        case 7: IDAHIP_WP_LAUNCH(7); break;                                                                 \
        default: IDAHIP_WP_LAUNCH(8); break;                                                                \
    }
            IDAHIP_WP_SWITCH()
            hipLaunchKernelGGL((lu_wavepanel_kernel<true, 0>), dim3(nsys), dim3(64), 0, c->stream, w, k0);
#undef IDAHIP_WP_SWITCH
#undef IDAHIP_WP_LAUNCH
        } else {
            KTimer kt(c, IDAHIP_K_LU_PANEL, nsys);
            panel2(k0, 0);
            if (n - k0 > NB) {
                const int cend = (k0 + 64 < n) ? k0 + 64 : n;
                hipLaunchKernelGGL((lu_trail_kernel<NB, LU_MAX_N, 2>), dim3(nsys8), dim3(256), 0, c->stream, w, k0, nsys, 1, cend, 0, 1);
                panel2(k0 + NB, NB);
            }
        }
        const int ntrail = n - k0 - 64;
        if (ntrail > 0) {
            KTimer kt(c, IDAHIP_K_LU_TRAIL, nsys);
            const int ncb = (ntrail + 63) / 64;
            if (n > LU_MAX_N) {
                const int nstrips = (ntrail + 15) / 16;
                int nsplit = nstrips >= 64 ? 8 : nstrips >= 32 ? 4 : nstrips >= 16 ? 2 : 1;
                while (!d_cnt && nsplit > 1 && nsys * nsplit > 512) nsplit >>= 1;
                const int nbs = nsplit > 1 ? std::min(ncb, LU_SPLIT_BLOCKS) : 0;
                hipLaunchKernelGGL(lu_u12_zero_kernel, dim3(nsys8 * ncb), dim3(256), 0, c->stream, w, k0, nsys, ncb);
                hipLaunchKernelGGL(lu_trail64w_kernel<LU_BIG_MAX_N>, dim3(nsys8 * (ncb + (nsplit - 1) * nbs)), dim3(256), 0, c->stream, w, k0, nsys, ncb, nsplit);
            } else
                hipLaunchKernelGGL(lu_trail64w_kernel<LU_MAX_N>, dim3(nsys8 * ncb), dim3(256), 0, c->stream, w, k0, nsys, ncb, 1);
        }
    }
    {
        KTimer kt(c, IDAHIP_K_LU_FINALIZE, nsys);
        hipLaunchKernelGGL(lu_finalize_kernel, dim3(nsys, (n + 31) / 32), dim3(256), 0, c->stream, w, out, ostride, perm, 32, NB,
                           n > LU_MAX_N ? (c->lu_superpanel ? 64 : 8) : 0,
                           c->lu_variant >= 4 ? ((c->lu_superpanel && n > LU_MAX_N) ? LU_MAX_N : WP_MAX_ROWS) : 0);
    }
    return 0;
}

}
```

### rust-ida_amd/csrc/lu_kernels.hpp

```cpp
#pragma once
#include <type_traits>
#include "common.hpp"

namespace idahip {

constexpr int LU_SPLIT_BLOCKS = 2;
constexpr int LU_SPARSE_COLS = 8;

struct LuWs {
    double* mats;
    long mstride;
    const int* idx;
    const int* cnt;
    int n;
    int* pos;
    int* live;
    int* prow;
    long long* piv;
    long pstride;
    int* info;
    int* nzb;
    int* bz;
    unsigned char* zmap;
    unsigned char* dirty;
// ... 458 lines not shown
            const int kq = lbase + lim[i];
            const double* __restrict__ src = A + (long)(k0 - lbase) * n + r[i];
            for (int j0 = 0; j0 < lbase; j0 += 8) {
                double v[8];
#pragma unroll
                for (int u = 0; u < 8; ++u) v[u] = (j0 + u < lbase) ? src[(long)(j0 + u) * n] : 0.0;
#pragma unroll
                for (int u = 0; u < 8; ++u)
                    if (j0 + u < lbase) l11[(j0 + u) * w.l11ld + kq] = v[u];
            }
#pragma unroll
            for (int j = 0; j < NB; ++j)
                if (j < lim[i]) l11[(lbase + j) * w.l11ld + kq] = a[i][j];
        }
    }
    unsigned long long bal[R];
#pragma unroll
    for (int i = 0; i < R; ++i) {
        bal[i] = __ballot(alive[i]);
        if (lane == 0) s_cnt[i][wave] = __popcll(bal[i]);
    }
    __syncthreads();
    const int nwaves = T >> 6;
    int base = 0;
#pragma unroll
    for (int i = 0; i < R; ++i) {
        int mine = base;
        for (int q = 0; q < nwaves; ++q) {
            const int c = s_cnt[i][q];
            if (q < wave) mine += c;
            base += c;
        }
        if (alive[i]) live[mine + __popcll(bal[i] & ((1ull << lane) - 1ull))] = r[i];
    }
    STAMP(3);
#undef STAMP
}

__global__ __launch_bounds__(256) void lu_u12_zero_kernel(LuWs w, int k0, int nsys, int ncb) {
    const int xcd = blockIdx.x & 7, slot = blockIdx.x >> 3;
    const int cbi = slot % ncb, mi = (slot / ncb) * 8 + xcd;
    if (mi >= (w.cnt ? ldc(w.cnt) : nsys)) return;
    const int b = w.idx[mi];
    if (w.info[b] != 0) return;
    const int n = w.n;
    const double* __restrict__ A = w.mats + (long)b * w.mstride;
    double* __restrict__ O = w.out + (long)b * w.ostride;
    const int cb0 = k0 + 64 + cbi * 64;
    const int ncols = (n - cb0) < 64 ? (n - cb0) : 64;
    const int t = threadIdx.x, lane = t & 63, wave = t >> 6;
    __shared__ int s_nz[4], s_bits[4];
    const int pr = w.prow[(long)b * n + k0 + lane];
    double g[16];
    bool nz = false, bits = false;
#pragma unroll
    for (int i = 0; i < 16; ++i) {
        const int cc = wave * 16 + i;
        g[i] = A[(long)(cb0 + (cc < ncols ? cc : 0)) * n + pr];
        nz = nz || (cc < ncols && g[i] != 0.0);
        bits = bits || (cc < ncols && __double_as_longlong(g[i]) != 0ll);
    }
    const bool wnz = __ballot(nz) != 0ull, wbits = __ballot(bits) != 0ull;
    if (lane == 0) { s_nz[wave] = wnz ? 1 : 0; s_bits[wave] = wbits ? 1 : 0; }
    __syncthreads();
    const int any = s_nz[0] | s_nz[1] | s_nz[2] | s_nz[3];
    const int anyb = s_bits[0] | s_bits[1] | s_bits[2] | s_bits[3];
    const long blk = (long)b * 4096 + ((k0 >> 6) + 1 + cbi) * 64 + (k0 >> 6);
    if (t == 0) {
        w.bz[b * 64 + cbi] = any;
        if (any && k0 == 0) atomicAdd(w.nzb + b, 1);
        if (any && w.zmap) w.zmap[blk] = 1;
        if (anyb && w.dirty) w.dirty[blk] = 1;
    }
    if (any) return;
    if (w.dirty && !anyb && w.dirty[blk] == 0) return;
#pragma unroll
    for (int i = 0; i < 16; ++i) {
        const int cc = wave * 16 + i;
        if (cc < ncols) O[(long)(cb0 + cc) * n + k0 + lane] = g[i];
    }
}

template <int NB, int MAXROWS, int CJ>
__global__ __launch_bounds__(256) void lu_trail_kernel(LuWs w, int k0, int nsys, int ncb, int climit, int l11off, int nsplit) {
    const int xcd = blockIdx.x & 7, slot = blockIdx.x >> 3;
    const int split = slot % nsplit, cbi = (slot / nsplit) % ncb, mi = (slot / (nsplit * ncb)) * 8 + xcd;
    if (mi >= (w.cnt ? ldc(w.cnt) : nsys)) return;
    const int b = w.idx[mi];
    if (w.info[b] != 0) return;
    const int n = w.n;
    double* __restrict__ A = w.mats + (long)b * w.mstride;
    const int* __restrict__ live = w.live + (long)b * n;
    const int* __restrict__ prow = w.prow + (long)b * n + k0;
    const double* __restrict__ l11 = w.l11 + (long)b * L11_STRIDE + l11off;

    const int mrem = n - k0 - NB;
    const int cb0 = k0 + NB + cbi * 64;
    const int ncols = (climit - cb0) < 64 ? (climit - cb0) : 64;
    const int t = threadIdx.x, lane = t & 63;
    const int wave = __builtin_amdgcn_readfirstlane(t >> 6);

    constexpr int LD = 66;
    __shared__ __align__(16) double Us[NB][LD];
    __shared__ __align__(16) double Ls[2][NB][LD];
    __shared__ unsigned short s_live[MAXROWS];
    __shared__ int s_anyzero;
    __shared__ unsigned s_kmask;
    __shared__ unsigned long long s_cmask;
    __shared__ int s_nz[4];

    for (int i = t; i < mrem; i += 256) s_live[i] = (unsigned short)live[i];
    bool nz = false;
#pragma unroll
    for (int pass = 0; pass < NB / 4; ++pass) {
        const int k = pass * 4 + wave;
        const int pr = ldc(prow + k);
        const double g = (lane < ncols) ? A[(long)(cb0 + lane) * n + pr] : 0.0;
        nz = nz || (g != 0.0);
        Us[k][lane] = g;
    }
    if (lane == 0) s_nz[wave] = 0;
    if (__ballot(nz) != 0ull && lane == 0) s_nz[wave] = 1;
    if (t == 0) s_anyzero = 0;
    for (int e = t; e < NB * NB; e += 256) Ls[0][e / NB][e % NB] = l11[(e / NB) * w.l11ld + (e % NB)];
    __syncthreads();
    if ((s_nz[0] | s_nz[1] | s_nz[2] | s_nz[3]) == 0) {
        double* __restrict__ O = w.out + (long)b * w.ostride;
        if (split == 0) {
#pragma unroll 4
            for (int i = 0; i < 16; ++i) {
                const int cc = wave * 16 + i;
                if (cc < ncols && lane < NB) O[(long)(cb0 + cc) * n + k0 + lane] = Us[lane][cc];
            }
        }
        return;
    }

    const int tx = t & 15, ty = t >> 4;
    const int ntiles = (mrem + 63) >> 6;
    int col[CJ];
    bool cok[CJ];
#pragma unroll
    for (int j = 0; j < CJ; ++j) {
        const int cj = ty + 16 * j;
        cok[j] = cj < ncols;
        col[j] = cb0 + (cok[j] ? cj : 0);
    }
    constexpr int LPT = NB / 4;
    double lreg[LPT], creg[4][CJ];
    int crow[4];
    bool rok[4];

    auto load_tile = [&](int rt, double (&lr_)[LPT], double (&cr_)[4][CJ], int (&crow_)[4], bool (&rok_)[4]) {
        const int lr = rt * 64 + lane;
        const int lrow = s_live[lr < mrem ? lr : mrem - 1];
#pragma unroll
        for (int i = 0; i < LPT; ++i) lr_[i] = A[(long)(k0 + wave * LPT + i) * n + lrow];
#pragma unroll
        for (int i = 0; i < 4; ++i) {
            const int ri = rt * 64 + tx + 16 * i;
            rok_[i] = ri < mrem;
            crow_[i] = s_live[rok_[i] ? ri : mrem - 1];
        }
#pragma unroll
        for (int j = 0; j < CJ; ++j)
#pragma unroll
            for (int i = 0; i < 4; ++i) cr_[i][j] = A[(long)col[j] * n + crow_[i]];
    };

    if (wave == 0) {
        double u[NB];
#pragma unroll
        for (int k = 0; k < NB; ++k) u[k] = Us[k][lane];
        const bool real = lane < ncols;
        bool anyz = false;
#pragma unroll
        for (int kk = 0; kk < NB; ++kk) {
            const double ukk = u[kk];
            const bool z = real && (ukk == 0.0);
            anyz = anyz || z;
            if (__ballot(z) == 0ull) {
#pragma unroll
                for (int k = 0; k < NB; ++k)
                    if (k > kk) u[k] -= ukk * Ls[0][kk][k];
            } else {
#pragma unroll
                for (int k = 0; k < NB; ++k)
                    if (k > kk) {
                        const double tn = u[k] - ukk * Ls[0][kk][k];
                        u[k] = z ? u[k] : tn;
                    }
            }
        }
#pragma unroll
        for (int k = 0; k < NB; ++k) Us[k][lane] = u[k];
        if (__ballot(anyz) != 0ull) {
            unsigned km = 0u;
            bool cnz = false;
#pragma unroll
            for (int k = 0; k < NB; ++k) {
                const bool e = real && u[k] != 0.0;
                cnz = cnz || e;
                km |= (__ballot(e) != 0ull) ? (1u << k) : 0u;
            }
            const unsigned long long cm = __ballot(cnz);
            if (lane == 0) {
                s_anyzero = 1;
                s_kmask = km;
                s_cmask = cm;
            }
        }
        load_tile(split, lreg, creg, crow, rok);
    } else {
        load_tile(split, lreg, creg, crow, rok);
    }
    __syncthreads();
    const bool slow = s_anyzero != 0;
    const unsigned kmask = slow ? (unsigned)__builtin_amdgcn_readfirstlane((int)s_kmask) : 0xffffffffu;
    if (split == 0) {
        double* __restrict__ O = w.out + (long)b * w.ostride;
#pragma unroll 4
        for (int i = 0; i < 16; ++i) {
            const int cc = wave * 16 + i;
            if (cc < ncols && lane < NB) O[(long)(cb0 + cc) * n + k0 + lane] = Us[lane][cc];
        }
    }

    if (kmask == 0u) return;
    if (MAXROWS > 1024 && slow) {
        const unsigned long long cmask = s_cmask;
        if (__popcll(cmask) <= LU_SPARSE_COLS) {
            for (int ri = split * 256 + t; ri < mrem; ri += 256 * nsplit) {
                const int row = s_live[ri];
                for (unsigned long long cmm = cmask; cmm != 0ull; cmm &= cmm - 1ull) {
                    const int c = __builtin_ctzll(cmm);
                    double v = A[(long)(cb0 + c) * n + row];
                    for (unsigned mk = kmask; mk != 0u; mk &= mk - 1u) {
                        const int kk = __builtin_ctz(mk);
                        const double u = Us[kk][c];
                        if (u != 0.0) v = v - u * A[(long)(k0 + kk) * n + row];
                    }
                    A[(long)(cb0 + c) * n + row] = v;
                }
            }
            return;
        }
    }
#pragma unroll 1
    for (int rt = split, it = 0; rt < ntiles; rt += nsplit, ++it) {
        const int buf = it & 1;
#pragma unroll
        for (int i = 0; i < LPT; ++i) Ls[buf][wave * LPT + i][lane] = lreg[i];
        asm volatile("s_waitcnt lgkmcnt(0)\n\ts_barrier" ::: "memory");
        double c[4][CJ];
        int srow[4];
        bool sok[4];
#pragma unroll
        for (int i = 0; i < 4; ++i) {
            srow[i] = crow[i];
            sok[i] = rok[i];
#pragma unroll
            for (int j = 0; j < CJ; ++j) c[i][j] = creg[i][j];
        }
        if (rt + nsplit < ntiles) load_tile(rt + nsplit, lreg, creg, crow, rok);
        if (!slow) {
#pragma unroll
            for (int k = 0; k < NB; ++k) {
                double lv[4], uv[CJ];
#pragma unroll
                for (int i = 0; i < 4; ++i) lv[i] = Ls[buf][k][tx + 16 * i];
#pragma unroll
                for (int j = 0; j < CJ; ++j) uv[j] = Us[k][ty + 16 * j];
#pragma unroll
                for (int j = 0; j < CJ; ++j)
#pragma unroll
                    for (int i = 0; i < 4; ++i) c[i][j] -= uv[j] * lv[i];
            }
        } else {
            for (unsigned mk = kmask; mk != 0u; mk &= mk - 1u) {
                const int k = __builtin_ctz(mk);
                double lv[4], uv[CJ];
#pragma unroll
                for (int i = 0; i < 4; ++i) lv[i] = Ls[buf][k][tx + 16 * i];
#pragma unroll
                for (int j = 0; j < CJ; ++j) uv[j] = Us[k][ty + 16 * j];
#pragma unroll
                for (int j = 0; j < CJ; ++j)
#pragma unroll
                    for (int i = 0; i < 4; ++i) {
                        const double tn = c[i][j] - uv[j] * lv[i];
                        c[i][j] = (uv[j] != 0.0) ? tn : c[i][j];
                    }
            }
        }
#pragma unroll
        for (int j = 0; j < CJ; ++j)
#pragma unroll
            for (int i = 0; i < 4; ++i)
                if (cok[j] && sok[i]) A[(long)col[j] * n + srow[i]] = c[i][j];
    }
}

template <int MAXROWS>
__global__ __launch_bounds__(256, MAXROWS <= 1024 ? 3 : 2) void lu_trail64w_kernel(LuWs w, int k0, int nsys, int ncb, int nsplit_arg) {
    constexpr int NB = 64, KC = 32;
    constexpr bool NOPRO = tb::NOPRO;
    const int nsplit = MAXROWS > 1024 ? nsplit_arg : 1;
    const int nbs = nsplit > 1 ? (ncb < LU_SPLIT_BLOCKS ? ncb : LU_SPLIT_BLOCKS) : 0;
    const int hs = nsplit > 1 ? nsplit - 1 : 1;
    const int wpm = ncb + hs * nbs;
    const int xcd = blockIdx.x & 7, slot = blockIdx.x >> 3;
    const int sm = slot % wpm, mi = (slot / wpm) * 8 + xcd;
    const int cbi = sm < ncb ? sm : (sm - ncb) / hs;
    const int split = sm < ncb ? 0 : 1 + (sm - ncb) % hs;
    if (mi >= (w.cnt ? ldc(w.cnt) : nsys)) return;
    const int b = w.idx[mi];
    if (w.info[b] != 0) return;
    if (MAXROWS > 1024 && ldc(w.bz + b * 64 + cbi) == 0) return;
    int nsp = 1;
    if (nsplit > 1) {
        const int nzb = ldc(w.nzb + b);
        const bool banded = k0 > 0 && nzb * 4 <= (w.n - 1) / 64;
        int eff = nsplit;
        if (w.cnt) {
            const int cntv = ldc(w.cnt);
            while (eff > 1 && cntv * eff > 512) eff >>= 1;
        }
        if (banded && cbi < nzb && cbi < nbs && split < eff) nsp = eff;
        else if (split != 0) return;
    }
    const int n = w.n;
    double* __restrict__ A = w.mats + (long)b * w.mstride;
    const int* __restrict__ live = w.live + (long)b * n;
    const int* __restrict__ prow = w.prow + (long)b * n + k0;
    const double* __restrict__ l11 = w.l11 + (long)b * L11_STRIDE;

    const int mrem = n - k0 - NB;
    const int cb0 = k0 + NB + cbi * 64;
    const int ncols = (n - cb0) < 64 ? (n - cb0) : 64;
    const int t = threadIdx.x, lane = t & 63;
    const int wave = __builtin_amdgcn_readfirstlane(t >> 6);
    const int pl = 4 * (lane & 15) + (lane >> 4);
    unsigned long long* tst = (tb::STAMPS >= 0 && k0 == tb::STAMPS && w.stamps) ? w.stamps + (size_t)blockIdx.x * 8 : nullptr;
#define TSTAMP(i) do { if (tb::STAMPS >= 0 && tst && t == 0) tst[i] = wall_clock64(); } while (0)
    TSTAMP(0);

    __shared__ __align__(16) double Us[NB][64 + tb::US_PAD];
    __shared__ __align__(16) double Ls[KC][64];
    __shared__ unsigned short s_live[MAXROWS];
    __shared__ int s_anyzero;
    __shared__ int s_nz[4];
    __shared__ unsigned s_kmask[2];
    __shared__ unsigned long long s_cmask[2];

    if (MAXROWS <= 1024)
        for (int i = t; i < mrem; i += 256) s_live[i] = (unsigned short)live[i];
    const int s0 = wave + 4 * split, sstep = 4 * nsp;

    const int a = lane & 3, q = lane >> 2;
    const int nstrips = (mrem + 15) >> 4;
    int coff[4];
    bool cok[4];
#pragma unroll
    for (int j = 0; j < 4; ++j) {
        const int cj = q + 16 * j;
        cok[j] = cj < ncols;
        coff[j] = (cb0 + (cok[j] ? cj : 0)) * n;
    }
    constexpr int LPT = KC / 4;
    const int kq = lane >> 4, lr16 = lane & 15;
    const int lslot = 4 * (lr16 & 3) + (lr16 >> 2);
    double lreg[LPT], creg[4][4];
    int crow[4];
    bool rok[4];

    auto load_L = [&](int s, int h) {
        const int lr = s * 16 + lr16;
        const int lrow = s_live[lr < mrem ? lr : mrem - 1];
#pragma unroll
        for (int i = 0; i < LPT; ++i) lreg[i] = A[(k0 + h * KC + 4 * i + kq) * n + lrow];
    };
    auto load_C = [&](int s) {
#pragma unroll
        for (int i = 0; i < 4; ++i) {
            const int ri = s * 16 + a + 4 * i;
            rok[i] = ri < mrem;
            crow[i] = s_live[rok[i] ? ri : mrem - 1];
        }
#pragma unroll
        for (int j = 0; j < 4; ++j)
#pragma unroll
            for (int i = 0; i < 4; ++i) creg[i][j] = A[coff[j] + crow[i]];
    };


    __shared__ int s_fz[4];
    bool fast_ok = false;
    if constexpr (MAXROWS <= 1024 && tb::TRAIL_QUAD) {
      if (!NOPRO) {
        const int part = lane & 3, qc = wave * 16 + (lane >> 2);
        const bool real = qc < ncols;
        double l11r[16], u[16];
#pragma unroll
        for (int i = 0; i < 16; ++i) l11r[i] = l11[i * 256 + t];
        {
            const double* __restrict__ colp = A + (long)(cb0 + (real ? qc : 0)) * n;
#pragma unroll
            for (int i = 0; i < 16; ++i) {
                const int p0 = ldc(prow + 4 * i), p1 = ldc(prow + 4 * i + 1), p2 = ldc(prow + 4 * i + 2), p3 = ldc(prow + 4 * i + 3);
                const int pr = part == 0 ? p0 : part == 1 ? p1 : part == 2 ? p2 : p3;
                if constexpr (tb::NOGATHER) u[i] = 1.0e-3 * (double)(1 + ((i + pr) & 7));
                else u[i] = colp[pr];
            }
        }
        double* __restrict__ Lq = &Us[0][0];
#pragma unroll
        for (int i = 0; i < 16; ++i) {
            const int e = i * 256 + t, kk = e >> 6, k = e & 63;
            Lq[kk * 66 + (k & 3) * 16 + (k >> 2) + 2 * ((k & 3) >> 1)] = l11r[i];
        }
        if (t == 0) s_anyzero = 0;
        lds_barrier();
        TSTAMP(1);
        if (s0 < nstrips) {
            load_C(s0);
            load_L(s0, 0);
        }
        const double* __restrict__ Lp = Lq + part * 16 + 2 * (part >> 1);
        bool anyz = false;
        static_for<0, 64>([&](auto kt) {
            constexpr int kk = decltype(kt)::value;
            constexpr int p0 = kk & 3, i0 = kk >> 2;
            const double ukk = dpp_mov_f64<p0 * 0x55, 0xf>(u[i0]);
            anyz = anyz || (ukk == 0.0);
            if constexpr (p0 < 3) {
                const double tn = upd(u[i0], ukk, Lp[kk * 66 + i0]);
                u[i0] = (part > p0) ? tn : u[i0];
            }
            static_for<i0 + 1, 16>([&](auto it) {
                constexpr int i = decltype(it)::value;
                u[i] = upd(u[i], ukk, Lp[kk * 66 + i]);
            });
        });
        TSTAMP(2);
        const unsigned long long zb = __ballot(anyz && real);
        if (lane == 0) s_fz[wave] = zb != 0ull ? 1 : 0;
        lds_barrier();
        fast_ok = (s_fz[0] | s_fz[1] | s_fz[2] | s_fz[3]) == 0;
        if (fast_ok) {
            const int qpl = 4 * (qc & 15) + (qc >> 4);
#pragma unroll
            for (int i = 0; i < 16; ++i) Us[4 * i + part][qpl] = real ? u[i] : 0.0;
        }
        lds_barrier();
        TSTAMP(3);
      }
    }
    if (!fast_ok) {
    bool nz = NOPRO;
    if (NOPRO) {
#pragma unroll
        for (int pass = 0; pass < NB / 4; ++pass) Us[pass * 4 + wave][pl] = 1.0e-4 * (double)(1 + ((pass + lane) & 7));
        if (t == 0) { s_kmask[0] = 0xffffffffu; s_kmask[1] = 0xffffffffu; s_cmask[0] = ~0ull; s_cmask[1] = ~0ull; }
    } else if (MAXROWS > 1024) {
        const int pr = prow[lane];
#pragma unroll 4
        for (int i = 0; i < 16; ++i) {
            const int cc = wave * 16 + i;
            const double g = (cc < ncols) ? A[(long)(cb0 + cc) * n + pr] : 0.0;
            nz = nz || (g != 0.0);
            Us[lane][4 * (cc & 15) + (cc >> 4)] = g;
        }
    } else {
#pragma unroll
        for (int pass = 0; pass < NB / 4; ++pass) {
            const int k = pass * 4 + wave;
            const int pr = ldc(prow + k);
            const double g = (lane < ncols) ? A[(long)(cb0 + lane) * n + pr] : 0.0;
            nz = nz || (g != 0.0);
            Us[k][pl] = g;
        }
    }
    if (lane == 0) s_nz[wave] = 0;
    if (__ballot(nz) != 0ull && lane == 0) s_nz[wave] = 1;
    if (t == 0) s_anyzero = 0;
    auto stage_l11 = [&](const int R0) {
#pragma unroll
        for (int i = 0; i < (KC * 64) / 256; ++i) {
            const int e = i * 256 + t;
            Ls[e >> 6][e & 63] = l11[(R0 + (e >> 6)) * NB + (e & 63)];
        }
    };
    if (MAXROWS <= 1024 && !NOPRO) stage_l11(0);
    lds_barrier();
    if ((s_nz[0] | s_nz[1] | s_nz[2] | s_nz[3]) == 0) {
        if (split != 0) return;
        double* __restrict__ O = w.out + (long)b * w.ostride;
#pragma unroll 4
        for (int i = 0; i < 16; ++i) {
            const int cc = wave * 16 + i;
            if (cc < ncols) O[(long)(cb0 + cc) * n + k0 + lane] = Us[lane][4 * (cc & 15) + (cc >> 4)];
        }
        return;
    }
    if (MAXROWS > 1024) {
        for (int i = t; i < mrem; i += 256) s_live[i] = (unsigned short)live[i];
        stage_l11(0);
        lds_barrier();
    }
    auto trsm32 = [&](const int R0) {
        double u[KC];
#pragma unroll
        for (int k = 0; k < KC; ++k) u[k] = Us[R0 + k][pl];
        const bool real = lane < ncols;
        bool anyz = false;
#pragma unroll
        for (int kk = 0; kk < KC; ++kk) {
            const double ukk = u[kk];
            const bool z = real && (ukk == 0.0);
            anyz = anyz || z;
            if (__ballot(z) == 0ull) {
#pragma unroll
                for (int k = 0; k < KC; ++k)
                    if (k > kk) u[k] = upd(u[k], ukk, Ls[kk][R0 + k]);
            } else if (MAXROWS > 1024 && __ballot(real && !z) == 0ull) {
            } else {
#pragma unroll
                for (int k = 0; k < KC; ++k)
                    if (k > kk) {
                        const double tn = upd(u[k], ukk, Ls[kk][R0 + k]);
                        u[k] = z ? u[k] : tn;
                    }
            }
        }
#pragma unroll
        for (int k = 0; k < KC; ++k) Us[R0 + k][pl] = u[k];
        unsigned km = 0xffffffffu;
        unsigned long long cm = ~0ull;
        if (__ballot(anyz) != 0ull || s_anyzero != 0) {
            km = 0u;
            bool cnz = false;
#pragma unroll
            for (int k = 0; k < KC; ++k) {
                const bool e = real && u[k] != 0.0;
                cnz = cnz || e;
                km |= (__ballot(e) != 0ull) ? (1u << k) : 0u;
            }
            cm = __ballot(cnz);
        }
        if (lane == 0) {
            s_kmask[R0 / KC] = km;
            s_cmask[R0 / KC] = cm;
            if (__ballot(anyz) != 0ull) s_anyzero = 1;
        }
    };

    if (wave == 0 && !NOPRO) trsm32(0);
    else if (s0 < nstrips) {
        load_C(s0);
        load_L(s0, 0);
    }
    lds_barrier();
    if (!NOPRO) {
        const bool zpath = s_anyzero != 0;
        double v[8];
#pragma unroll
        for (int i = 0; i < 8; ++i) v[i] = Us[KC + wave * 8 + i][pl];
        if (!zpath) {
#pragma unroll
            for (int kk = 0; kk < KC; ++kk) {
                const double ut = Us[kk][pl];
#pragma unroll
                for (int i = 0; i < 8; ++i) v[i] = upd(v[i], ut, Ls[kk][KC + wave * 8 + i]);
            }
        } else {
#pragma unroll 4
            for (int kk = 0; kk < KC; ++kk) {
                const double ut = Us[kk][pl];
                if (MAXROWS > 1024 && __ballot(ut != 0.0) == 0ull) continue;
#pragma unroll
                for (int i = 0; i < 8; ++i) {
                    const double tn = upd(v[i], ut, Ls[kk][KC + wave * 8 + i]);
                    v[i] = (ut != 0.0) ? tn : v[i];
                }
            }
        }
#pragma unroll
        for (int i = 0; i < 8; ++i) Us[KC + wave * 8 + i][pl] = v[i];
    }
    if (!NOPRO) {
    lds_barrier();
    stage_l11(KC);
    lds_barrier();
    if (wave == 0) {
        trsm32(KC);
        if (s0 < nstrips) {
            load_C(s0);
            load_L(s0, 0);
        }
    }
    }
    lds_barrier();
    }
    const bool slow = s_anyzero != 0;
    if (split == 0) {
        double* __restrict__ O = w.out + (long)b * w.ostride;
#pragma unroll 4
        for (int i = 0; i < 16; ++i) {
            const int cc = wave * 16 + i;
            if (cc < ncols) O[(long)(cb0 + cc) * n + k0 + lane] = Us[lane][4 * (cc & 15) + (cc >> 4)];
        }
    }
    if constexpr (tb::NOUPD) return;
    TSTAMP(4);
    const unsigned kmask0 = (unsigned)__builtin_amdgcn_readfirstlane((int)s_kmask[0]);
    const unsigned kmask1 = (unsigned)__builtin_amdgcn_readfirstlane((int)s_kmask[1]);
    if (slow && (kmask0 | kmask1) == 0u) return;
    if (MAXROWS > 1024 && slow) {
        const unsigned long long cmask = s_cmask[0] | s_cmask[1];
        if (__popcll(cmask) <= LU_SPARSE_COLS) {
            for (int ri = split * 256 + t; ri < mrem; ri += 256 * nsp) {
                const int row = s_live[ri];
                for (unsigned long long cmm = cmask; cmm != 0ull; cmm &= cmm - 1ull) {
                    const int c = __builtin_ctzll(cmm);
                    const int cs = 4 * (c & 15) + (c >> 4);
                    double v = A[(long)(cb0 + c) * n + row];
                    for (unsigned mk = kmask0; mk != 0u; mk &= mk - 1u) {
                        const int kk = __builtin_ctz(mk);
                        const double u = Us[kk][cs];
                        if (u != 0.0) v = upd(v, u, A[(long)(k0 + kk) * n + row]);
                    }
                    for (unsigned mk = kmask1; mk != 0u; mk &= mk - 1u) {
                        const int kk = KC + __builtin_ctz(mk);
                        const double u = Us[kk][cs];
                        if (u != 0.0) v = upd(v, u, A[(long)(k0 + kk) * n + row]);
                    }
                    A[(long)(cb0 + c) * n + row] = v;
                }
            }
            return;
        }
    }
    double (*__restrict__ Lw)[16] = reinterpret_cast<double (*)[16]>(&Ls[0][0] + wave * (KC * 16));

    auto chunk = [&](double (&c)[4][4], const int kbase) {
        if (!slow) {
            double lvA[4], uvA[4], lvB[4], uvB[4];
            auto rd = [&](const int k, double (&lv)[4], double (&uv)[4]) {
#pragma unroll
                for (int i = 0; i < 4; ++i) lv[i] = Lw[k][4 * a + i];
#pragma unroll
                for (int j = 0; j < 4; ++j) uv[j] = Us[kbase + k][4 * q + j];
            };
            auto mac = [&](const double (&lv)[4], const double (&uv)[4]) {
#pragma unroll
                for (int j = 0; j < 4; ++j)
#pragma unroll
                    for (int i = 0; i < 4; ++i) c[i][j] = upd(c[i][j], uv[j], lv[i]);
            };
            if constexpr (tb::TRAIL_PIPE) {
                rd(0, lvA, uvA);
#pragma unroll
                for (int k = 0; k < KC; k += 2) {
                    rd(k + 1, lvB, uvB);
                    __builtin_amdgcn_sched_barrier(0);
                    mac(lvA, uvA);
                    if (k + 2 < KC) rd(k + 2, lvA, uvA);
                    __builtin_amdgcn_sched_barrier(0);
                    mac(lvB, uvB);
                }
            } else {
#pragma unroll
                for (int k = 0; k < KC; ++k) {
                    rd(k, lvA, uvA);
                    mac(lvA, uvA);
                }
            }
        } else {
            for (unsigned mk = kbase == 0 ? kmask0 : kmask1; mk != 0u; mk &= mk - 1u) {
                const int k = __builtin_ctz(mk);
                double lv[4], uv[4];
#pragma unroll
                for (int i = 0; i < 4; ++i) lv[i] = Lw[k][4 * a + i];
#pragma unroll
                for (int j = 0; j < 4; ++j) uv[j] = Us[kbase + k][4 * q + j];
#pragma unroll
                for (int j = 0; j < 4; ++j)
#pragma unroll
                    for (int i = 0; i < 4; ++i) {
                        const double tn = upd(c[i][j], uv[j], lv[i]);
                        c[i][j] = (uv[j] != 0.0) ? tn : c[i][j];
                    }
            }
        }
    };

#pragma unroll 1
    for (int s = s0; s < nstrips; s += sstep) {
#pragma unroll
        for (int i = 0; i < LPT; ++i) Lw[4 * i + kq][lslot] = lreg[i];
        load_L(s, 1);
        double c[4][4];
        int srow[4];
        bool sok[4];
#pragma unroll
        for (int i = 0; i < 4; ++i) {
            srow[i] = crow[i];
            sok[i] = rok[i];
#pragma unroll
            for (int j = 0; j < 4; ++j) c[i][j] = creg[i][j];
        }
        if constexpr (tb::STAMPS >= 0) {
            if (s == s0) { asm volatile("s_waitcnt vmcnt(0)" ::: "memory"); TSTAMP(5); }
        }
        chunk(c, 0);
        if constexpr (tb::STAMPS >= 0) {
            if (s == s0) TSTAMP(6);
        }
#pragma unroll
        for (int i = 0; i < LPT; ++i) Lw[4 * i + kq][lslot] = lreg[i];
        if (s + sstep < nstrips) {
            load_C(s + sstep);
            load_L(s + sstep, 0);
        }
        chunk(c, KC);
#pragma unroll
        for (int j = 0; j < 4; ++j)
#pragma unroll
            for (int i = 0; i < 4; ++i)
                if (cok[j] && sok[i]) A[coff[j] + srow[i]] = c[i][j];
    }
    TSTAMP(7);
#undef TSTAMP
}

__global__ __launch_bounds__(256) void lu_finalize_kernel(LuWs w, double* __restrict__ out, long ostride, int* __restrict__ perm,
                                                          int cols_per_block, int sp, int sp_lead, int wp_rows) {
    if (w.cnt && (int)blockIdx.x >= *w.cnt) return;
    const int b = w.idx[blockIdx.x];
    if (w.info[b] != 0) return;
    const int n = w.n;
    double* __restrict__ A = w.mats + (long)b * w.mstride;
    double* __restrict__ O = out + (long)b * ostride;
    const int* __restrict__ pos = w.pos + (long)b * n;
    const int jbeg = blockIdx.y * cols_per_block;
    const bool clearw = w.jwzero != nullptr && w.dirty != nullptr;
    if (clearw && blockIdx.y == 0 && threadIdx.x == 0) w.jwzero[b] = 1;
    const int jend = (jbeg + cols_per_block < n) ? jbeg + cols_per_block : n;
    for (int r = threadIdx.x; r < n; r += blockDim.x) {
        const int p = pos[r];
        if (blockIdx.y == 0 && perm) perm[(long)b * n + p] = r;
        int je = jend;
        if (sp > 0) {
            const int liv = n - (p & ~63);
            const int w_ = (wp_rows > 0 && liv <= wp_rows) ? 64 : (sp_lead > 0 && liv > LU_MAX_N) ? (sp_lead >= 64 ? 64 : liv > LU_WIDE_ROWS ? sp_lead : 2 * sp_lead) : sp;
            const int spend = (p / w_ + 1) * w_;
            je = je < spend ? je : spend;
        }
        if (w.zmap && w.dirty) {
            unsigned char* __restrict__ zm = w.zmap + (long)b * 4096;
            unsigned char* __restrict__ dm = w.dirty + (long)b * 4096;
            const int blk = (jbeg >> 6) * 64 + (p >> 6);
            const bool was_dirty = dm[blk] != 0;
            bool anybits = false, anynz = false;
            unsigned cmask = 0u;
            for (int j0 = jbeg; j0 < je; j0 += 8) {
                double v[8];
#pragma unroll
                for (int u = 0; u < 8; ++u) v[u] = (j0 + u < je) ? A[(long)(j0 + u) * n + r] : 0.0;
#pragma unroll
                for (int u = 0; u < 8; ++u) {
                    const bool bits = __double_as_longlong(v[u]) != 0ll;
                    anybits = anybits || bits;
                    anynz = anynz || (v[u] != 0.0);
                    if (j0 + u < je && (bits || was_dirty)) O[(long)(j0 + u) * n + p] = v[u];
                    if (bits && j0 + u < je) cmask |= 1u << (j0 + u - jbeg);
                }
            }
            if (anybits && !was_dirty) dm[blk] = 1;
            if (anynz) zm[blk] = 1;
            if (clearw)
                for (unsigned m = cmask; m != 0u; m &= m - 1u) A[(long)(jbeg + __builtin_ctz(m)) * n + r] = 0.0;
            if (clearw && je <= jbeg && dm[blk] != 0)
                for (int j = jbeg; j < jend; ++j) A[(long)j * n + r] = 0.0;
        } else if (w.zmap) {
            unsigned char* __restrict__ zm = w.zmap + (long)b * 4096;
            for (int j = jbeg; j < je; ++j) {
                const double v = A[(long)j * n + r];
                O[(long)j * n + p] = v;
                if (v != 0.0) zm[(j >> 6) * 64 + (p >> 6)] = 1;
            }
        } else {
            for (int j = jbeg; j < je; ++j) O[(long)j * n + p] = A[(long)j * n + r];
        }
    }
}

__device__ inline int tiny_getrf(double* __restrict__ a, int n, long long* __restrict__ pivot, int* __restrict__ perm) {
    for (int i = 0; i < n; ++i) perm[i] = i;
    for (int k = 0; k < n; ++k) {
        double* col_k = a + k * n;
        int l = k;
        for (int i = k + 1; i < n; ++i)
            if (fabs(col_k[i]) > fabs(col_k[l])) l = i;
        pivot[k] = l;
        if (col_k[l] == 0.0) return k + 1;
        if (l != k) {
            for (int i = 0; i < n; ++i) {
                const double tmp = a[i * n + k];
                a[i * n + k] = a[i * n + l];
                a[i * n + l] = tmp;
            }
            const int tp = perm[k];
            perm[k] = perm[l];
            perm[l] = tp;
        }
        const double mult = 1.0 / a[k * n + k];
        for (int i = k + 1; i < n; ++i) a[k * n + i] *= mult;
        for (int j = k + 1; j < n; ++j) {
            const double a_kj = a[j * n + k];
            if (a_kj != 0.0) {
                for (int i = k + 1; i < n; ++i) a[j * n + i] -= a_kj * a[k * n + i];
            }
        }
    }
    return 0;
}

__global__ void tiny_getrf_kernel(double* mats, long mstride, const int* idx, int nsys, int n, long long* piv, long pstride,
                                  int* perm, int* info) {
    const int s = blockIdx.x * blockDim.x + threadIdx.x;
    if (s >= nsys) return;
    const int b = idx[s];
    int lperm[TINY_N];
    info[b] = tiny_getrf(mats + (long)b * mstride, n, piv + (long)b * pstride, lperm);
    if (perm)
        for (int i = 0; i < n; ++i) perm[(long)b * n + i] = lperm[i];
}

}
```

### rust-ida_amd/csrc/lu_wavepanel.hpp

```cpp
#pragma once
#include <type_traits>

#include "lu_kernels.hpp"

namespace idahip {

constexpr int WP_MAX_ROWS = 512;
constexpr int WP_RING(int ns) { return !tb::WP_DEEP_RING ? 2 : (ns >= 1 && ns <= 2) ? 8 : (ns >= 3 && ns <= 7) ? 4 : 2; }

template <bool SLOWK, int NS>
__global__ __launch_bounds__(64, SLOWK ? 1 : (NS > 0 && NS <= 3 ? 4 : 2)) void lu_wavepanel_kernel(LuWs w, const int k0) {
    constexpr int BIG = 1 << 20;
    if (w.cnt && (int)blockIdx.x >= *w.cnt) return;
    const int b = w.idx[blockIdx.x];
    if (w.info[b] != 0) return;
    const int n = w.n;
    double* __restrict__ A = w.mats + (long)b * w.mstride;
    int* __restrict__ pos = w.pos + (long)b * n;
    int* __restrict__ live = w.live + (long)b * n;
    int* __restrict__ prow = w.prow + (long)b * n;
    long long* __restrict__ piv = w.piv + (long)b * w.pstride;
    double* __restrict__ l11 = w.l11 + (long)b * L11_STRIDE;

    const __amdgpu_buffer_rsrc_t rsrc = __builtin_amdgcn_make_buffer_rsrc(A, 0, n * n * 8, 0x00020000);
    const int m = n - k0;
    const int wsp = m < 64 ? m : 64;
    const int lane = threadIdx.x;
    const int nslots = NS > 0 ? NS : (m + 63) >> 6;
    constexpr int NSC = NS > 0 ? NS : 8;

    __shared__ int ptab[64];

    int rowid[8], rpos[8], pstep[8];
    unsigned roff[8];
    static_for<0, NSC>([&](auto st) {
        constexpr int S = decltype(st)::value;
        const int li = S * 64 + lane;
        const bool has = li < m;
        rowid[S] = has ? live[li] : 0;
        rpos[S] = has ? pos[rowid[S]] : 0x7fffffff;
        pstep[S] = has ? BIG : -1;
        roff[S] = (unsigned)rowid[S] * 8u;
    });

    auto load_block = [&](double (&x)[8][8], const int b8, const int wb) {
        static_for<0, NSC>([&](auto st) {
            constexpr int S = decltype(st)::value;
            if (S < nslots) {
                const double* __restrict__ src = A + (long)(k0 + b8) * n + rowid[S];
#pragma unroll
                for (int j = 0; j < 8; ++j) x[S][j] = (j < wb) ? src[(long)j * n] : 0.0;
            } else {
#pragma unroll
                for (int j = 0; j < 8; ++j) x[S][j] = 0.0;
            }
        });
    };
    auto store_block = [&](const double (&x)[8][8], const int b8, const int wb) {
        static_for<0, NSC>([&](auto st) {
            constexpr int S = decltype(st)::value;
            if (S < nslots && pstep[S] >= 0) {
                double* __restrict__ dst = A + (long)(k0 + b8) * n + rowid[S];
#pragma unroll
                for (int j = 0; j < 8; ++j)
                    if (j < wb) dst[(long)j * n] = x[S][j];
            }
        });
    };

    auto process = [&](auto slow_tag, double (&x)[8][8], const int b8, const int wb) -> int {
        constexpr bool SLOW = decltype(slow_tag)::value;
        if (b8 > 0) {
            auto load_l = [&](double (&l)[8], const int k) {
                const int coloff = (k0 + k) * n * 8;
                static_for<0, NSC>([&](auto st) {
                    constexpr int S = decltype(st)::value;
                    l[S] = buf_load_f64(rsrc, roff[S], coloff);
                });
            };
            auto apply = [&](const double (&l)[8], const int k, const int ow) {
                const int pl = __builtin_amdgcn_readfirstlane(ow) & 63, ps = __builtin_amdgcn_readfirstlane(ow) >> 6;
                double uk[8];
                switch (ps) {
#define IDAHIP_WP_CASE(SV)                                                                     \
    case SV:                                                                                   \
        if constexpr (SV < NSC) {                                                              \
            _Pragma("unroll") for (int j = 0; j < 8; ++j) uk[j] = readlane_f64(x[SV][j], pl); \
        }                                                                                      \
        break;
                    IDAHIP_WP_CASE(1)
                    IDAHIP_WP_CASE(2)
                    IDAHIP_WP_CASE(3)
                    IDAHIP_WP_CASE(4)
                    IDAHIP_WP_CASE(5)
                    IDAHIP_WP_CASE(6)
                    IDAHIP_WP_CASE(7)
                    default:
                        IDAHIP_WP_CASE(0)
#undef IDAHIP_WP_CASE
                }
                double ukv[8];
                if (SLOW) {
#pragma unroll
                    for (int j = 0; j < 8; ++j) ukv[j] = opaque_vgpr(uk[j]);
                }
                static_for<0, NSC>([&](auto st) {
                    constexpr int S = decltype(st)::value;
                    if (S < nslots) {
                        if (pstep[S] > k) {
#pragma unroll
                            for (int j = 0; j < 8; ++j) {
                                if (SLOW) {
                                    const double tn = upd(x[S][j], ukv[j], l[S]);
                                    x[S][j] = (ukv[j] == 0.0) ? x[S][j] : tn;
                                } else {
                                    x[S][j] = upd(x[S][j], uk[j], l[S]);
                                }
                            }
                        }
                    }
                });
            };
            __builtin_amdgcn_s_waitcnt(0x0F70);
            constexpr int D = WP_RING(NS);
            double l[D][8];
            int ow[D];
            static_for<0, D>([&](auto dt) {
                constexpr int d = decltype(dt)::value;
                load_l(l[d], d);
                ow[d] = ptab[d];
            });
#pragma unroll 1
            for (int k = 0; k < b8; k += D) {
                static_for<0, D>([&](auto dt) {
                    constexpr int d = decltype(dt)::value;
                    apply(l[d], k + d, ow[d]);
                    const int kn = (k + d + D < b8) ? k + d + D : b8 - 1;
                    load_l(l[d], kn);
                    ow[d] = ptab[kn];
                });
            }
        }
        bool special = false;
        int status = 0, failcol = 0;
        static_for<0, 8>([&](auto kt) {
            constexpr int kk = decltype(kt)::value;
            const bool active = !SLOW || (status == 0 && kk < wb);
            const int kstep = b8 + kk, kc = k0 + kstep;
            unsigned kh[8], kl[8];
            static_for<0, NSC>([&](auto st) {
                constexpr int S = decltype(st)::value;
                const double v = x[S][kk];
                unsigned h = (unsigned)__double2hiint(v) | 0x80000000u, l = (unsigned)__double2loint(v);
                if (SLOW) {
                    if (v != v) {
                        h = (rpos[S] == kc) ? 0xfff00000u : 0u;
                        l = 0u;
                    }
                }
                kh[S] = (pstep[S] == BIG) ? h : 0u;
                kl[S] = l;
            });
            unsigned lm = kh[0];
#pragma unroll
            for (int s = 1; s < NSC; ++s) lm = kh[s] > lm ? kh[s] : lm;
            const unsigned mh = wave_max_u32<false>(lm);
            if (!SLOW) special = special || mh >= 0xfff00000u;
            int cnt = 0, slot = 0;
#pragma unroll
            for (int s = 0; s < NSC; ++s) {
                const bool e = kh[s] == mh;
                cnt += e ? 1 : 0;
                slot = e ? s : slot;
            }
            const unsigned long long bal = __ballot(cnt > 0);
            int pl = (int)__ffsll((unsigned long long)bal) - 1;
            int ps;
            if (__popcll(bal) == 1 && __builtin_amdgcn_readlane(cnt, pl) == 1) {
                ps = __builtin_amdgcn_readlane(slot, pl);
            } else {
                unsigned bl = 0u;
                int bp_ = 0x7fffffff, bs = 0;
#pragma unroll
                for (int s = 0; s < NSC; ++s) {
                    const bool e = kh[s] == mh;
                    const bool better = e && (kl[s] > bl || (kl[s] == bl && rpos[s] < bp_) || bp_ == 0x7fffffff);
                    bl = better ? kl[s] : bl;
                    bp_ = better ? rpos[s] : bp_;
                    bs = better ? s : bs;
                }
                const bool e1 = bp_ != 0x7fffffff;
                const unsigned ml = wave_max_u32<false>(e1 ? bl : 0u);
                const bool top = e1 && bl == ml;
                const int pm = wave_min_i32f<false>(top ? bp_ : 0x7fffffff);
                const unsigned long long b2 = __ballot(top && bp_ == pm);
                pl = (int)__ffsll((unsigned long long)b2) - 1;
                ps = __builtin_amdgcn_readlane(bs, pl);
            }
            double u[8];
            int bp = 0, pr = 0;
            switch (ps) {
#define IDAHIP_WP_CASE(SV)                                                                             \
    case SV:                                                                                           \
        if constexpr (SV < NSC) {                                                                      \
            _Pragma("unroll") for (int j = kk; j < 8; ++j) u[j] = readlane_f64(x[SV][j], pl);         \
            bp = __builtin_amdgcn_readlane(rpos[SV], pl);                                              \
            pr = __builtin_amdgcn_readlane(rowid[SV], pl);                                             \
        }                                                                                              \
        break;
                IDAHIP_WP_CASE(1)
                IDAHIP_WP_CASE(2)
                IDAHIP_WP_CASE(3)
                IDAHIP_WP_CASE(4)
                IDAHIP_WP_CASE(5)
                IDAHIP_WP_CASE(6)
                IDAHIP_WP_CASE(7)
                default:
                    IDAHIP_WP_CASE(0)
#undef IDAHIP_WP_CASE
            }
            bool go = active;
            if (active && u[kk] == 0.0) {
                status = 1;
                failcol = kc + 1;
                go = !SLOW;
            }
            const double recip = 1.0 / u[kk];
            if (go) {
                if (lane == 0) {
                    piv[kc] = (long long)bp;
                    prow[kc] = pr;
                    ptab[kstep] = pl | (ps << 6);
                }
                __builtin_amdgcn_fence(__ATOMIC_RELEASE, "wavefront");
                __builtin_amdgcn_wave_barrier();
                static_for<0, NSC>([&](auto st) {
                    constexpr int S = decltype(st)::value;
                    if (pstep[S] == BIG && rpos[S] == kc) rpos[S] = bp;
                    if (lane == pl && ps == S) {
                        pstep[S] = kstep;
                        rpos[S] = kc;
                    }
                });
            }
            double uv[8];
            if (SLOW) {
#pragma unroll
                for (int j = kk + 1; j < 8; ++j) uv[j] = opaque_vgpr(u[j]);
            }
            static_for<0, NSC>([&](auto st) {
                constexpr int S = decltype(st)::value;
                if (S < nslots) {
                    if (pstep[S] == BIG && go) {
                        const double l = x[S][kk] * recip;
                        x[S][kk] = l;
#pragma unroll
                        for (int j = kk + 1; j < 8; ++j) {
                            if (SLOW) {
                                const double tn = upd(x[S][j], uv[j], l);
                                x[S][j] = (uv[j] == 0.0) ? x[S][j] : tn;
                            } else {
                                x[S][j] = upd(x[S][j], u[j], l);
                            }
                        }
                    }
                }
            });
        });
        if (!SLOW) {
            bool z = false;
            static_for<0, NSC>([&](auto st) {
                constexpr int S = decltype(st)::value;
                bool zz = false;
#pragma unroll
                for (int j = 0; j < 8; ++j) zz = zz || (x[S][j] == 0.0 && j < wb);
                z = z || (zz && pstep[S] >= 0 && pstep[S] != BIG);
            });
            if (special || status != 0 || __ballot(z) != 0ull) return 2;
        }
        if (status == 1 && lane == 0) w.info[b] = failcol;
        return status;
    };

    int bstart = 0;
    if (SLOWK) {
        const int rd = w.redo[b];
        if (rd == 0) return;
        bstart = (rd - 1) * 8;
        for (int k = 0; k < bstart; ++k) {
            const int kc = k0 + k;
            const int bp = (int)piv[kc], pr = prow[kc];
            static_for<0, NSC>([&](auto st) {
                constexpr int S = decltype(st)::value;
                if (pstep[S] == BIG && rpos[S] == kc) rpos[S] = bp;
                const bool mine = pstep[S] >= 0 && rowid[S] == pr;
                if (mine) {
                    pstep[S] = k;
                    rpos[S] = kc;
                }
                const unsigned long long bm = __ballot(mine);
                if (bm != 0ull && lane == 0) ptab[k] = ((int)__ffsll((unsigned long long)bm) - 1) | (S << 6);
            });
            __builtin_amdgcn_fence(__ATOMIC_RELEASE, "wavefront");
            __builtin_amdgcn_wave_barrier();
        }
        if (lane == 0) w.redo[b] = 0;
    }
    for (int b8 = bstart; b8 < wsp; b8 += 8) {
        const int wb = (wsp - b8) < 8 ? (wsp - b8) : 8;
        double x[8][8];
        int st;
        if (SLOWK) {
            load_block(x, b8, wb);
            st = process(std::true_type{}, x, b8, wb);
        } else {
            if (wb != 8) {
                st = 2;
            } else {
                load_block(x, b8, 8);
                st = process(std::false_type{}, x, b8, 8);
            }
            if (st == 2) {
                if (lane == 0) w.redo[b] = 1 + (b8 >> 3);
                return;
            }
        }
        if (st != 0) return;
        store_block(x, b8, wb);
    }

    __syncthreads();
    static_for<0, NSC>([&](auto st) {
        constexpr int S = decltype(st)::value;
        if (pstep[S] >= 0) pos[rowid[S]] = rpos[S];
    });
    if (lane < wsp) {
        const double* __restrict__ src = A + (long)k0 * n + prow[k0 + lane];
        for (int j0 = 0; j0 < lane; j0 += 8) {
            double v[8];
#pragma unroll
            for (int u = 0; u < 8; ++u) v[u] = (j0 + u < lane) ? src[(long)(j0 + u) * n] : 0.0;
#pragma unroll
            for (int u = 0; u < 8; ++u)
                if (j0 + u < lane) l11[(j0 + u) * 64 + lane] = v[u];
        }
    }
    int base = 0;
    static_for<0, NSC>([&](auto st) {
        constexpr int S = decltype(st)::value;
        const bool al = pstep[S] == BIG;
        const unsigned long long bal = __ballot(al);
        if (al) live[base + __popcll(bal & ((1ull << lane) - 1ull))] = rowid[S];
        base += __popcll(bal);
    });
}

}
```

### rust-ida_amd/idahip/__init__.py

```python
import ctypes as C
import os

import numpy as np

_HERE = os.path.dirname(os.path.abspath(__file__))
_PKG = os.path.dirname(_HERE)
LIB_HIP = os.environ.get("IDAHIP_LIB_HIP", os.path.join(_PKG, "csrc", "libidahip.so"))
LIB_ENS = os.path.join(_PKG, "host", "libidaens.so")

dp = C.POINTER(C.c_double)
i32p = C.POINTER(C.c_int32)
i64p = C.POINTER(C.c_int64)

ROBERTS, LORENZ63, LINEAR_DENSE, HEAT1D, HOST_CALLBACK = 0, 1, 2, 3, 4
KIND = {"roberts": ROBERTS, "lorenz63": LORENZ63, "linear_dense": LINEAR_DENSE, "heat1d": HEAT1D, "host_callback": HOST_CALLBACK}
RES_FN = C.CFUNCTYPE(C.c_int, C.c_int, C.c_double, C.POINTER(C.c_double), C.POINTER(C.c_double), C.POINTER(C.c_double), C.c_void_p)
JAC_FN = C.CFUNCTYPE(C.c_int, C.c_int, C.c_double, C.c_double, C.POINTER(C.c_double), C.POINTER(C.c_double), C.POINTER(C.c_double),
                     C.POINTER(C.c_double), C.c_void_p)
BAND_JAC_FN = C.CFUNCTYPE(C.c_int, C.c_int, C.c_double, C.c_double, C.POINTER(C.c_double), C.POINTER(C.c_double), C.POINTER(C.c_double),
                          C.POINTER(C.c_double), C.c_int, C.c_void_p)
ROOT_FN = C.CFUNCTYPE(C.c_int, C.c_void_p, C.c_int32, C.c_double, C.POINTER(C.c_double), C.POINTER(C.c_double), C.c_int32, C.POINTER(C.c_double))
F_YY, F_YP, F_YYPREDICT, F_YPPREDICT, F_EWT, F_EE, F_DELTA, F_SAVRES, F_PHI0 = range(9)
K_NEWTON_ITER, K_SYS, K_JAC, K_LU, K_VECTOR, K_SOLVE, K_SYS_JAC = range(7)
K_NAMES = ["newton_iter", "sys", "jac", "lu", "vector", "solve", "sys_jac", "lu_panel", "lu_trail", "lu_finalize"]

HIP_SYMBOLS = [
    "idahip_create", "idahip_destroy", "idahip_last_error", "idahip_sync", "idahip_n", "idahip_batch", "idahip_kind", "idahip_set_tolerances",
    "idahip_set_problem_params", "idahip_set_linear_dense", "idahip_set_host_problem", "idahip_upload", "idahip_download", "idahip_download_lu",
    "idahip_dev_alloc", "idahip_dev_free", "idahip_memcpy_h2d", "idahip_memcpy_d2h", "idahip_ls_setup", "idahip_ls_solve",
    "idahip_wrms", "idahip_nls_sys", "idahip_nls_lsetup", "idahip_nls_sys_setup", "idahip_newton_iter", "idahip_newton_iter2", "idahip_init_first", "idahip_scale_phi1",
    "idahip_predict", "idahip_post_newton", "idahip_restore", "idahip_complete_step", "idahip_get_solution", "idahip_get_dky",
    "idahip_timing_enable", "idahip_timing_get", "idahip_timing_reset", "idahip_set_lu_variant", "idahip_snapshot_initial",
    "idahip_tiny_solve", "idahip_pow_batch", "idahip_round_solve", "idahip_lu_variant",
    "idahip_restore_initial", "idahip_ls_type", "idahip_ls_num_iters", "idahip_ls_res_norm", "idahip_timing_build", "idahip_concurrent_streams", "idahip_release_streams", "idahip_stream_pair_share", "idahip_set_lu_superpanel", "idahip_lu_superpanel", "idahip_set_lu_period", "idahip_lu_period",
    "idahip_create_band", "idahip_band", "idahip_set_host_band_problem", "idahip_download_lu_band", "idahip_ls_setup_band", "idahip_ls_solve_band",
    "idahip_set_jacobian_dq", "idahip_jacobian_dq", "idahip_set_host_residual", "idahip_jac_dq", "idahip_nls_lsetup_dq",
]
ENS_SYMBOLS = [
    "idaens_create", "idaens_destroy", "idaens_last_error", "idaens_set_max_num_steps", "idaens_set_max_ord", "idaens_set_fused_newton", "idaens_set_device_controller", "idaens_device_controller_active", "idaens_set_roots", "idaens_set_root_fn",
    "idaens_get_roots", "idaens_solve", "idaens_solve_schedule", "idaens_stream", "idaens_stream_group", "idaens_solve_schedule_group",
    "idaens_get_counter", "idaens_get_real", "idaens_get_yy", "idaens_get_yp", "idaens_get_dky", "idaens_total_newton_iters",
    "idaens_total_rounds", "idaens_trace_system", "idaens_trace_len", "idaens_trace_get",
]

_libs = None


def _f64(a):
    return np.ascontiguousarray(np.asarray(a, dtype=np.float64))


def _i32(a):
    return np.ascontiguousarray(np.asarray(a, dtype=np.int32))


def _p(a, t=dp):
    return None if a is None else a.ctypes.data_as(t)


def load():
    global _libs
    if _libs is not None:
        return _libs
    for p in (LIB_HIP, LIB_ENS):
        if not os.path.exists(p):
            raise OSError("%s is missing: the HIP extension is not built (run `python __graft_entry__.py`); "
                          "there is no CPU fallback" % p)
    H = C.CDLL(LIB_HIP, mode=C.RTLD_GLOBAL)
    H.idahip_timing_build.argtypes = []
    if H.idahip_timing_build() != 0 and os.environ.get("IDAHIP_ALLOW_TIMING_BUILD") != "1":
        raise OSError("%s is a timing build (-DIDAHIP_TIMING_BUILD, csrc/exp_switches.hpp): its results are garbage by design; "
                      "only the measurement tools load one, with IDAHIP_ALLOW_TIMING_BUILD=1" % LIB_HIP)
    E = C.CDLL(LIB_ENS)
    vp, ci, cd = C.c_void_p, C.c_int, C.c_double
    H.idahip_create.argtypes = [C.POINTER(vp), ci, ci, ci, ci, vp]
    H.idahip_destroy.argtypes = [vp]
    H.idahip_create_band.argtypes = [C.POINTER(vp), ci, ci, ci, ci, vp, ci, ci]
    H.idahip_band.argtypes = [vp, C.POINTER(ci), C.POINTER(ci)]
    H.idahip_set_host_band_problem.argtypes = [vp, RES_FN, BAND_JAC_FN, vp]
    H.idahip_download_lu_band.argtypes = [vp, ci, dp, i64p]
    H.idahip_ls_setup_band.argtypes = [vp, ci, ci, vp, vp, i32p, i32p, ci]
    H.idahip_ls_solve_band.argtypes = [vp, ci, ci, vp, vp, vp, vp, cd, i32p, ci]
    H.idahip_concurrent_streams.argtypes = [ci, ci, C.POINTER(vp), C.POINTER(ci)]
    H.idahip_release_streams.argtypes = [ci, ci, C.POINTER(vp)]
    H.idahip_stream_pair_share.argtypes = [ci, vp, vp, C.POINTER(cd)]
    H.idahip_set_lu_superpanel.argtypes = [vp, ci]
    H.idahip_lu_superpanel.argtypes = [vp]
    H.idahip_set_lu_period.argtypes = [vp, ci]
    H.idahip_lu_period.argtypes = [vp]
    H.idahip_last_error.argtypes = [vp]
    H.idahip_last_error.restype = C.c_char_p
    H.idahip_sync.argtypes = [vp]
    H.idahip_n.argtypes = [vp]
    H.idahip_batch.argtypes = [vp]
    H.idahip_set_tolerances.argtypes = [vp, cd, dp, ci]
    H.idahip_set_problem_params.argtypes = [vp, ci, ci, dp, ci]
    H.idahip_set_linear_dense.argtypes = [vp, ci, ci, dp, dp, dp]
    H.idahip_upload.argtypes = [vp, ci, ci, ci, dp]
    H.idahip_download.argtypes = [vp, ci, ci, ci, dp]
    H.idahip_download_lu.argtypes = [vp, ci, dp, i64p]
    H.idahip_dev_alloc.argtypes = [vp, C.c_size_t]
    H.idahip_dev_alloc.restype = vp
    H.idahip_dev_free.argtypes = [vp, vp]
    H.idahip_memcpy_h2d.argtypes = [vp, vp, vp, C.c_size_t]
    H.idahip_memcpy_d2h.argtypes = [vp, vp, vp, C.c_size_t]
    H.idahip_ls_setup.argtypes = [vp, vp, vp, i32p, i32p, ci]
    H.idahip_ls_solve.argtypes = [vp, vp, vp, vp, vp, cd, i32p, ci]
    H.idahip_wrms.argtypes = [vp, vp, vp, dp, i32p, ci]
    H.idahip_ls_type.argtypes = [vp]
    H.idahip_ls_num_iters.argtypes = [vp]
    H.idahip_ls_res_norm.argtypes = [vp]
    H.idahip_ls_res_norm.restype = cd
    H.idahip_nls_sys.argtypes = [vp, dp, dp, ci, i32p, ci]
    H.idahip_nls_lsetup.argtypes = [vp, dp, dp, i32p, i32p, ci]
    H.idahip_nls_sys_setup.argtypes = [vp, dp, dp, ci, i32p, i32p, ci]
    H.idahip_newton_iter.argtypes = [vp, dp, dp, i32p, ci]
    H.idahip_init_first.argtypes = [vp, dp, dp, i32p, ci]
    H.idahip_scale_phi1.argtypes = [vp, dp, i32p, ci]
    H.idahip_predict.argtypes = [vp, i32p, dp, dp, i32p, ci]
    H.idahip_post_newton.argtypes = [vp, dp, i32p, dp, i32p, ci]
    H.idahip_restore.argtypes = [vp, i32p, dp, i32p, ci]
    H.idahip_complete_step.argtypes = [vp, i32p, dp, ci, dp, i32p, i32p, ci]
    H.idahip_get_solution.argtypes = [vp, i32p, dp, dp, i32p, ci]
    H.idahip_get_dky.argtypes = [vp, i32p, i32p, dp, dp, i32p, ci]
    H.idahip_snapshot_initial.argtypes = [vp]
    H.idahip_restore_initial.argtypes = [vp, i32p, ci]
    H.idahip_set_lu_variant.argtypes = [vp, ci]
    H.idahip_pow_batch.argtypes = [vp, dp, dp, dp, C.c_size_t]
    H.idahip_newton_iter2.argtypes = [vp, dp, dp, dp, dp, dp, dp, dp, i32p, i32p, ci]
    H.idahip_set_host_problem.argtypes = [vp, RES_FN, JAC_FN, vp]
    H.idahip_set_jacobian_dq.argtypes = [vp, ci]
    H.idahip_jacobian_dq.argtypes = [vp]
    H.idahip_set_host_residual.argtypes = [vp, RES_FN, vp]
    H.idahip_jac_dq.argtypes = [vp, dp, dp, dp, dp, i32p, ci]
    H.idahip_nls_lsetup_dq.argtypes = [vp, dp, dp, dp, i32p, i32p, ci]
    H.idahip_timing_enable.argtypes = [vp, ci]
    H.idahip_timing_get.argtypes = [vp, ci, dp, i64p, i64p]
    H.idahip_timing_reset.argtypes = [vp]
    E.idaens_create.argtypes = [C.POINTER(vp), vp, dp, dp]
    E.idaens_destroy.argtypes = [vp]
    E.idaens_last_error.argtypes = [vp]
    E.idaens_last_error.restype = C.c_char_p
    E.idaens_set_max_num_steps.argtypes = [vp, C.c_long]
    E.idaens_set_max_ord.argtypes = [vp, ci]
    E.idaens_set_fused_newton.argtypes = [vp, ci]
    E.idaens_set_device_controller.argtypes = [vp, ci]
    E.idaens_device_controller_active.argtypes = [vp]
    E.idaens_stream_group.argtypes = [C.POINTER(vp), ci, dp, ci, C.c_long, C.c_long, C.c_long, i64p]
    E.idaens_solve_schedule_group.argtypes = [C.POINTER(vp), ci, dp, ci, C.POINTER(dp), C.POINTER(i32p), C.POINTER(i32p), C.c_long]
    E.idaens_set_roots.argtypes = [vp, ci, i32p, dp]
    E.idaens_set_root_fn.argtypes = [vp, ci, ROOT_FN, vp]
    E.idaens_get_roots.argtypes = [vp, i32p]
    E.idaens_solve.argtypes = [vp, cd, ci, dp, i32p, C.c_long]
    E.idaens_solve_schedule.argtypes = [vp, dp, ci, dp, i32p, i32p, dp, dp, C.c_long]
    E.idaens_stream.argtypes = [vp, dp, ci, C.c_long, C.c_long, i64p]
    E.idaens_get_counter.argtypes = [vp, ci, i64p]
    E.idaens_get_real.argtypes = [vp, ci, dp]
    E.idaens_get_yy.argtypes = [vp, dp]
    E.idaens_get_dky.argtypes = [vp, C.c_double, ci, dp, i32p]
    E.idaens_get_yp.argtypes = [vp, dp]
    E.idaens_total_newton_iters.argtypes = [vp]
    E.idaens_total_newton_iters.restype = C.c_int64
    E.idaens_total_rounds.argtypes = [vp]
    E.idaens_total_rounds.restype = C.c_int64
    E.idaens_trace_system.argtypes = [vp, ci]
    E.idaens_trace_len.argtypes = [vp]
    E.idaens_trace_len.restype = C.c_long
    E.idaens_trace_get.argtypes = [vp, dp]
    _libs = (H, E)
    return _libs


class IdaHipError(RuntimeError):
    pass


class Ctx:

    def __init__(self, kind, n, batch, device=0, stream=None, band=None):
        self.H, self.E = load()
        self.n, self.batch = int(n), int(batch)
        self.kind = KIND[kind] if isinstance(kind, str) else int(kind)
        h = C.c_void_p()
        if band is None:
            self.band = None
            rc = self.H.idahip_create(C.byref(h), int(device), self.n, self.batch, self.kind, stream)
            if rc != 0 or not h.value:
                raise IdaHipError("idahip_create failed (%d) -- is a GPU visible?" % rc)
        else:
            self.band = (int(band[0]), int(band[1]))
            rc = self.H.idahip_create_band(C.byref(h), int(device), self.n, self.batch, self.kind, stream, *self.band)
            if rc != 0 or not h.value:
                raise IdaHipError("idahip_create_band failed (%d) -- band form of this kind and size, and a GPU visible?" % rc)
        self.h = h

    @property
    def ldab(self):
        return None if self.band is None else 2 * self.band[0] + self.band[1] + 1

    def band_query(self):
        ml, mu = C.c_int(-1), C.c_int(-1)
        rc = self.H.idahip_band(self.h, C.byref(ml), C.byref(mu))
        return (ml.value, mu.value) if rc == 1 else None

    def close(self):
        if getattr(self, "h", None) is not None and self.h.value:
            if getattr(self, "_ensembles", 0) > 0:
                raise IdaHipError("close() of a Ctx with %d open Ensemble(s): close them first" % self._ensembles)
            self.H.idahip_destroy(self.h)
            self.h = C.c_void_p()

    def __del__(self):
        try:
            self._ensembles = 0
            self.close()
        except Exception:
            pass

    def _chk(self, rc, what):
        if rc < 0:
            self.fail("%s failed (%d): %s" % (what, rc, self.H.idahip_last_error(self.h).decode()))
        return rc

    def fail(self, message):
        cause, self._cb_error = getattr(self, "_cb_error", None), None
        if cause is not None:
            raise IdaHipError(message + " [Python callback raised %s: %s]" % (type(cause).__name__, cause)) from cause
        raise IdaHipError(message)

    def take_callback_error(self):
        err, self._cb_error = getattr(self, "_cb_error", None), None
        return err

    def all_idx(self):
        return np.arange(self.batch, dtype=np.int32)

    def set_tolerances(self, rtol, atol):
        a = _f64(np.atleast_1d(atol))
        self._chk(self.H.idahip_set_tolerances(self.h, float(rtol), _p(a), a.size), "set_tolerances")

    def set_problem_params(self, params, first=0):
        p = _f64(params).reshape(-1, _f64(params).shape[-1] if np.ndim(params) > 1 else 1)
        self._chk(self.H.idahip_set_problem_params(self.h, first, p.shape[0], _p(p), p.shape[1]), "set_problem_params")

    def set_linear_dense(self, A, B, c, first=0):
        A, B, c = _f64(A), _f64(B), _f64(c)
        self._chk(self.H.idahip_set_linear_dense(self.h, first, A.shape[0], _p(A), _p(B), _p(c)), "set_linear_dense")

    def set_host_problem(self, res, jac):
        n = self.n

        self._cb_error = None

        def c_res(sys, t, yy, yp, out, _user):
            try:
                r = res(sys, t, np.ctypeslib.as_array(yy, (n,)), np.ctypeslib.as_array(yp, (n,)))
                np.copyto(np.ctypeslib.as_array(out, (n,)), np.asarray(r, dtype=np.float64).reshape(n))
                return 0
            except Exception as e:
                self._cb_error = e
                return 1

        def c_jac(sys, t, cj, yy, yp, rv, J, _user):
            try:
                m = jac(sys, t, cj, np.ctypeslib.as_array(yy, (n,)), np.ctypeslib.as_array(yp, (n,)), np.ctypeslib.as_array(rv, (n,)))
                np.copyto(np.ctypeslib.as_array(J, (n, n)), np.asarray(m, dtype=np.float64).reshape(n, n).T)
                return 0
            except Exception as e:
                self._cb_error = e
                return 1

        self._cb = (RES_FN(c_res), JAC_FN(c_jac))
        self._chk(self.H.idahip_set_host_problem(self.h, self._cb[0], self._cb[1], None), "set_host_problem")

    def set_host_residual(self, res):
        n = self.n
        self._cb_error = None

        def c_res(sys, t, yy, yp, out, _user):
            try:
                r = res(sys, t, np.ctypeslib.as_array(yy, (n,)), np.ctypeslib.as_array(yp, (n,)))
                np.copyto(np.ctypeslib.as_array(out, (n,)), np.asarray(r, dtype=np.float64).reshape(n))
                return 0
            except Exception as e:
                self._cb_error = e
                return 1

        self._cb = (RES_FN(c_res),)
        self._chk(self.H.idahip_set_host_residual(self.h, self._cb[0], None), "set_host_residual")

    def set_jacobian_dq(self, on=True):
        self._chk(self.H.idahip_set_jacobian_dq(self.h, int(bool(on))), "set_jacobian_dq")

    def jacobian_dq(self):
        return bool(self._chk(self.H.idahip_jacobian_dq(self.h), "jacobian_dq"))

    def jac_dq(self, tn, cj, hh, idx=None):
        idx = self.all_idx() if idx is None else _i32(idx)
        tn, cj, hh = (_f64(np.broadcast_to(v, idx.shape)) for v in (tn, cj, hh))
        per = self.ldab if self.band else self.n
        out = np.zeros((idx.size, self.n, per), dtype=np.float64)
        self._chk(self.H.idahip_jac_dq(self.h, _p(tn), _p(cj), _p(hh), _p(out), _p(idx, i32p), idx.size), "jac_dq")
        return out

    def nls_lsetup_dq(self, tn, cj, hh, idx=None):
        idx = self.all_idx() if idx is None else _i32(idx)
        tn, cj, hh = (_f64(np.broadcast_to(v, idx.shape)) for v in (tn, cj, hh))
        info = np.zeros(idx.size, dtype=np.int32)
        rc = self._chk(self.H.idahip_nls_lsetup_dq(self.h, _p(tn), _p(cj), _p(hh), _p(info, i32p), _p(idx, i32p), idx.size), "nls_lsetup_dq")
        return rc, info

    def set_host_band_problem(self, res, bjac):
        n = self.n
        self._cb_error = None

        def c_res(sys, t, yy, yp, out, _user):
            try:
                r = res(sys, t, np.ctypeslib.as_array(yy, (n,)), np.ctypeslib.as_array(yp, (n,)))
                np.copyto(np.ctypeslib.as_array(out, (n,)), np.asarray(r, dtype=np.float64).reshape(n))
                return 0
            except Exception as e:
                self._cb_error = e
                return 1

        def c_bjac(sys, t, cj, yy, yp, rv, AB, ldab, _user):
            try:
                view = np.ctypeslib.as_array(AB, (n, ldab))
                m = bjac(sys, t, cj, np.ctypeslib.as_array(yy, (n,)), np.ctypeslib.as_array(yp, (n,)), np.ctypeslib.as_array(rv, (n,)), view)
                if m is not None:
                    np.copyto(view, np.asarray(m, dtype=np.float64).reshape(n, ldab))
                return 0
            except Exception as e:
                self._cb_error = e
                return 1

        self._cb = (RES_FN(c_res), BAND_JAC_FN(c_bjac))
        self._chk(self.H.idahip_set_host_band_problem(self.h, self._cb[0], self._cb[1], None), "set_host_band_problem")

    def download_lu_band(self, sys):
        ld = self.ldab if self.ldab is not None else 1
        ab = np.empty(self.n * ld)
        piv = np.empty(self.n, dtype=np.int64)
        self._chk(self.H.idahip_download_lu_band(self.h, sys, _p(ab), _p(piv, i64p)), "download_lu_band")
        return ab.reshape(self.n, ld), piv

    def upload(self, field, arr, first=0):
        a = _f64(arr).reshape(-1, self.n)
        self._chk(self.H.idahip_upload(self.h, field, first, a.shape[0], _p(a)), "upload")

    def download(self, field, first=0, count=None):
        count = self.batch - first if count is None else count
        out = np.empty((count, self.n))
        self._chk(self.H.idahip_download(self.h, field, first, count, _p(out)), "download")
        return out

    def download_lu(self, sys):
        lu = np.empty(self.n * self.n)
        piv = np.empty(self.n, dtype=np.int64)
        self._chk(self.H.idahip_download_lu(self.h, sys, _p(lu), _p(piv, i64p)), "download_lu")
        return lu.reshape(self.n, self.n).T.copy(), piv

    def dev_array(self, host):
        host = np.ascontiguousarray(host)
        d = self.H.idahip_dev_alloc(self.h, host.nbytes)
        if not d:
            raise IdaHipError("device allocation of %d bytes failed" % host.nbytes)
        self._chk(self.H.idahip_memcpy_h2d(self.h, d, host.ctypes.data_as(C.c_void_p), host.nbytes), "h2d")
        return d

    def dev_empty(self, nbytes):
        d = self.H.idahip_dev_alloc(self.h, nbytes)
        if not d:
            raise IdaHipError("device allocation of %d bytes failed" % nbytes)
        return d

    def to_host(self, d, shape, dtype=np.float64):
        out = np.empty(shape, dtype=dtype)
        self._chk(self.H.idahip_memcpy_d2h(self.h, out.ctypes.data_as(C.c_void_p), d, out.nbytes), "d2h")
        return out

    def dev_free(self, d):
        self.H.idahip_dev_free(self.h, d)

    def ls_setup(self, dA, dPiv, idx=None):
        idx = self.all_idx() if idx is None else _i32(idx)
        info = np.zeros(idx.size, dtype=np.int32)
        rc = self._chk(self.H.idahip_ls_setup(self.h, dA, dPiv, _p(info, i32p), _p(idx, i32p), idx.size), "ls_setup")
        return rc, info

    def ls_solve(self, dLU, dPiv, dX, dB, idx=None):
        idx = self.all_idx() if idx is None else _i32(idx)
        self._chk(self.H.idahip_ls_solve(self.h, dLU, dPiv, dX, dB, 0.0, _p(idx, i32p), idx.size), "ls_solve")
        self._chk(self.H.idahip_sync(self.h), "sync")

    def ls_setup_band(self, ml, mu, dAB, dPiv, idx=None):
        idx = self.all_idx() if idx is None else _i32(idx)
        info = np.zeros(idx.size, dtype=np.int32)
        rc = self._chk(self.H.idahip_ls_setup_band(self.h, int(ml), int(mu), dAB, dPiv, _p(info, i32p), _p(idx, i32p), idx.size), "ls_setup_band")
        return rc, info

    def ls_solve_band(self, ml, mu, dAB, dPiv, dX, dB, idx=None):
        idx = self.all_idx() if idx is None else _i32(idx)
        self._chk(self.H.idahip_ls_solve_band(self.h, int(ml), int(mu), dAB, dPiv, dX, dB, 0.0, _p(idx, i32p), idx.size), "ls_solve_band")
        self._chk(self.H.idahip_sync(self.h), "sync")

    def wrms(self, dX, dW, idx=None):
        idx = self.all_idx() if idx is None else _i32(idx)
        out = np.zeros(idx.size)
        self._chk(self.H.idahip_wrms(self.h, dX, dW, _p(out), _p(idx, i32p), idx.size), "wrms")
        return out

    def nls_sys(self, tn, cj, reset_ee, idx=None):
        idx = self.all_idx() if idx is None else _i32(idx)
        tn, cj = _f64(np.broadcast_to(tn, idx.shape)), _f64(np.broadcast_to(cj, idx.shape))
        self._chk(self.H.idahip_nls_sys(self.h, _p(tn), _p(cj), int(reset_ee), _p(idx, i32p), idx.size), "nls_sys")

    def nls_lsetup(self, tn, cj, idx=None):
        idx = self.all_idx() if idx is None else _i32(idx)
        tn, cj = _f64(np.broadcast_to(tn, idx.shape)), _f64(np.broadcast_to(cj, idx.shape))
        info = np.zeros(idx.size, dtype=np.int32)
        rc = self._chk(self.H.idahip_nls_lsetup(self.h, _p(tn), _p(cj), _p(info, i32p), _p(idx, i32p), idx.size), "nls_lsetup")
        return rc, info

    def nls_sys_setup(self, tn, cj, reset_ee=True, idx=None):
        idx = self.all_idx() if idx is None else _i32(idx)
        tn, cj = _f64(np.broadcast_to(tn, idx.shape)), _f64(np.broadcast_to(cj, idx.shape))
        info = np.zeros(idx.size, dtype=np.int32)
        rc = self._chk(self.H.idahip_nls_sys_setup(self.h, _p(tn), _p(cj), int(bool(reset_ee)), _p(info, i32p), _p(idx, i32p), idx.size),
                       "nls_sys_setup")
        return rc, info

    def newton_iter(self, scale, idx=None):
        idx = self.all_idx() if idx is None else _i32(idx)
        scale = _f64(np.broadcast_to(scale, idx.shape))
        out = np.zeros(idx.size)
        self._chk(self.H.idahip_newton_iter(self.h, _p(scale), _p(out), _p(idx, i32p), idx.size), "newton_iter")
        return out

    def newton_iter2(self, scale, tn, cj, toldel, ss, eps_newt, idx=None):
        idx = self.all_idx() if idx is None else _i32(idx)
        scale, tn, cj, toldel, ss, eps_newt = (_f64(np.broadcast_to(v, idx.shape)) for v in (scale, tn, cj, toldel, ss, eps_newt))
        dn = np.zeros((idx.size, 2))
        conv = np.zeros(idx.size, dtype=np.int32)
        self._chk(self.H.idahip_newton_iter2(self.h, _p(scale), _p(tn), _p(cj), _p(toldel), _p(ss), _p(eps_newt), _p(dn),
                                             _p(conv, i32p), _p(idx, i32p), idx.size), "newton_iter2")
        return dn, conv

    def init_first(self, idx=None):
        idx = self.all_idx() if idx is None else _i32(idx)
        a, b = np.zeros(idx.size), np.zeros(idx.size)
        self._chk(self.H.idahip_init_first(self.h, _p(a), _p(b), _p(idx, i32p), idx.size), "init_first")
        return a, b

    def scale_phi1(self, fac, idx=None):
        idx = self.all_idx() if idx is None else _i32(idx)
        fac = _f64(np.broadcast_to(fac, idx.shape))
        self._chk(self.H.idahip_scale_phi1(self.h, _p(fac), _p(idx, i32p), idx.size), "scale_phi1")

    def predict(self, kk, ns, beta, gamma, idx=None):
        idx = self.all_idx() if idx is None else _i32(idx)
        kkns = _i32(np.stack([np.broadcast_to(kk, idx.shape), np.broadcast_to(ns, idx.shape)], axis=1))
        beta = _f64(np.broadcast_to(beta, (idx.size, 6)))
        gamma = _f64(np.broadcast_to(gamma, (idx.size, 6)))
        self._chk(self.H.idahip_predict(self.h, _p(kkns, i32p), _p(beta), _p(gamma), _p(idx, i32p), idx.size), "predict")

    def post_newton(self, cj, kk, idx=None):
        idx = self.all_idx() if idx is None else _i32(idx)
        cj = _f64(np.broadcast_to(cj, idx.shape))
        kk = _i32(np.broadcast_to(kk, idx.shape))
        out = np.zeros((idx.size, 4))
        self._chk(self.H.idahip_post_newton(self.h, _p(cj), _p(kk, i32p), _p(out), _p(idx, i32p), idx.size), "post_newton")
        return out

    def restore(self, kk, ns, cvals, idx=None):
        idx = self.all_idx() if idx is None else _i32(idx)
        kkns = _i32(np.stack([np.broadcast_to(kk, idx.shape), np.broadcast_to(ns, idx.shape)], axis=1))
        cvals = _f64(np.broadcast_to(cvals, (idx.size, 6)))
        self._chk(self.H.idahip_restore(self.h, _p(kkns, i32p), _p(cvals), _p(idx, i32p), idx.size), "restore")

    def complete_step(self, kused, ck, maxord=5, idx=None):
        idx = self.all_idx() if idx is None else _i32(idx)
        kused = _i32(np.broadcast_to(kused, idx.shape))
        ck = _f64(np.broadcast_to(ck, idx.shape))
        nrm = np.zeros(idx.size)
        bad = np.zeros(idx.size, dtype=np.int32)
        self._chk(self.H.idahip_complete_step(self.h, _p(kused, i32p), _p(ck), int(maxord), _p(nrm), _p(bad, i32p), _p(idx, i32p),
                                              idx.size), "complete_step")
        return nrm, bad

    def get_solution(self, kord, cvals, dvals, idx=None):
        idx = self.all_idx() if idx is None else _i32(idx)
        kord = _i32(np.broadcast_to(kord, idx.shape))
        cvals = _f64(np.broadcast_to(cvals, (idx.size, 6)))
        dvals = _f64(np.broadcast_to(dvals, (idx.size, 5)))
        self._chk(self.H.idahip_get_solution(self.h, _p(kord, i32p), _p(cvals), _p(dvals), _p(idx, i32p), idx.size), "get_solution")

    def get_dky(self, kfirst, klast, cjk, idx=None):
        idx = self.all_idx() if idx is None else _i32(idx)
        kfirst = _i32(np.broadcast_to(kfirst, idx.shape))
        klast = _i32(np.broadcast_to(klast, idx.shape))
        cjk = _f64(np.broadcast_to(cjk, (idx.size, 6)))
        out = np.zeros((idx.size, self.n))
        self._chk(self.H.idahip_get_dky(self.h, _p(kfirst, i32p), _p(klast, i32p), _p(cjk), _p(out), _p(idx, i32p), idx.size), "get_dky")
        return out

    def snapshot_initial(self):
        self._chk(self.H.idahip_snapshot_initial(self.h), "snapshot_initial")

    def restore_initial(self, idx=None):
        idx = self.all_idx() if idx is None else _i32(idx)
        self._chk(self.H.idahip_restore_initial(self.h, _p(idx, i32p), idx.size), "restore_initial")

    def pow_batch(self, x, y):
        x, y = _f64(x), _f64(y)
        out = np.empty_like(x)
        self._chk(self.H.idahip_pow_batch(self.h, _p(x), _p(y), _p(out), x.size), "pow_batch")
        return out

    def set_lu_superpanel(self, on):
        self._chk(self.H.idahip_set_lu_superpanel(self.h, int(on)), "set_lu_superpanel")

    def lu_superpanel(self):
        return int(self.H.idahip_lu_superpanel(self.h))

    def set_lu_period(self, rounds):
        self._chk(self.H.idahip_set_lu_period(self.h, int(rounds)), "set_lu_period")

    def lu_period(self):
        return int(self.H.idahip_lu_period(self.h))

    def set_lu_variant(self, variant):
        self._chk(self.H.idahip_set_lu_variant(self.h, int(variant)), "set_lu_variant")

    def timing(self, on):
        self.H.idahip_timing_enable(self.h, int(on))

    def timing_reset(self):
        self.H.idahip_timing_reset(self.h)

    def timing_get(self):
        out = {}
        for k, name in enumerate(K_NAMES):
            ms, la, sy = C.c_double(), C.c_int64(), C.c_int64()
            self.H.idahip_timing_get(self.h, k, C.byref(ms), C.byref(la), C.byref(sy))
            out[name] = {"ms": ms.value, "launches": la.value, "systems": sy.value}
        return out


def band_ldab(ml, mu):
    return 2 * int(ml) + int(mu) + 1


def band_pack(dense, ml, mu):
    dense = np.asarray(dense, dtype=np.float64)
    n = dense.shape[-1]
    kv, ld = int(ml) + int(mu), band_ldab(ml, mu)
    ab = np.zeros(dense.shape[:-2] + (n, ld))
    for j in range(n):
        lo, hi = max(0, j - int(mu)), min(n - 1, j + int(ml))
        ab[..., j, kv + lo - j:kv + hi - j + 1] = dense[..., lo:hi + 1, j]
    return ab


def band_unpack(ab, n, ml, mu, fill=False):
    ab = np.asarray(ab, dtype=np.float64).reshape(np.shape(ab)[:-2] + (n, band_ldab(ml, mu)))
    kv = int(ml) + int(mu)
    top = kv if fill else int(mu)
    dense = np.zeros(ab.shape[:-2] + (n, n))
    for j in range(n):
        lo, hi = max(0, j - top), min(n - 1, j + int(ml))
        dense[..., lo:hi + 1, j] = ab[..., j, kv + lo - j:kv + hi - j + 1]
    return dense


def band_expand_factors(ab, piv, n, ml, mu):
    d = band_unpack(ab, n, ml, mu, fill=True)
    piv = np.asarray(piv, dtype=np.int64)
    L = np.tril(d, -1)
    U = np.triu(d)
    for j in range(n):
        p = int(piv[j])
        if p != j:
            L[[j, p], :j] = L[[p, j], :j]
    return L + U


COUNTERS = {"nst": 0, "nre": 1, "nje": 2, "nsetups": 3, "nni": 4, "netf": 5, "ncfn": 6, "n_attempts": 7, "nls_nconvfails": 8,
            "kused": 9, "kk": 10, "nge": 11, "nlufail": 12, "nconv_jcur": 13, "nfail_first": 14, "nli": 15, "ncfl": 16,
            "nre_dq": 17}
REALS = {"tn": 0, "hused": 1, "hh": 2, "h0u": 3, "tolsf": 4}


class Ensemble:

    def __init__(self, ctx, yy0, yp0):
        self.ctx = ctx
        self.E = ctx.E
        yy0, yp0 = _f64(yy0).reshape(ctx.batch, ctx.n), _f64(yp0).reshape(ctx.batch, ctx.n)
        h = C.c_void_p()
        rc = self.E.idaens_create(C.byref(h), ctx.h, _p(yy0), _p(yp0))
        if rc != 0:
            self.ctx.fail("idaens_create failed (%d): %s" % (rc, ctx.H.idahip_last_error(ctx.h).decode()))
        self.h = h
        ctx._ensembles = getattr(ctx, "_ensembles", 0) + 1

    def close(self):
        if getattr(self, "h", None) is not None and self.h.value:
            self.E.idaens_destroy(self.h)
            self.h = C.c_void_p()
            self.ctx._ensembles -= 1

    def __del__(self):
        try:
            self.close()
        except Exception:
            pass

    def set_max_num_steps(self, mxstep):
        self.E.idaens_set_max_num_steps(self.h, int(mxstep))

    def set_roots(self, comps, thresholds):
        comps, thr = _i32(comps), _f64(thresholds)
        if self.E.idaens_set_roots(self.h, comps.size, _p(comps, i32p), _p(thr)) != 0:
            raise IdaHipError("set_roots: %s" % (self.E.idaens_last_error(self.h) or b"").decode())
        self.nroots = comps.size

    def set_root_fn(self, nroots, fn):
        ens = self

        def thunk(user, sys, t, yy, yp, nr, gout):
            try:
                n = ens.ctx.n
                g = fn(int(sys), float(t), np.ctypeslib.as_array(yy, (n,)), np.ctypeslib.as_array(yp, (n,)))
                np.copyto(np.ctypeslib.as_array(gout, (nr,)), np.asarray(g, dtype=np.float64).reshape(nr))
                return 0
            except Exception as e:
                ens.ctx._cb_error = e
                return 1

        self._root_thunk = ROOT_FN(thunk)
        if self.E.idaens_set_root_fn(self.h, int(nroots), self._root_thunk, None) != 0:
            raise IdaHipError("set_root_fn: %s" % (self.E.idaens_last_error(self.h) or b"").decode())
        self.nroots = int(nroots)

    def roots_found(self):
        out = np.zeros((self.ctx.batch, getattr(self, "nroots", 0)), dtype=np.int32)
        if out.size:
            self.E.idaens_get_roots(self.h, _p(out, i32p))
        return out

    def set_fused_newton(self, on):
        self.E.idaens_set_fused_newton(self.h, int(on))

    def set_device_controller(self, on):
        rc = self.E.idaens_set_device_controller(self.h, int(on))
        if rc != 0:
            raise IdaHipError("set_device_controller(%d) refused (%d): %s" % (int(on), rc, self.E.idaens_last_error(self.h).decode()))

    def device_controller_active(self):
        return int(self.E.idaens_device_controller_active(self.h))

    def set_max_ord(self, maxord):
        if self.E.idaens_set_max_ord(self.h, int(maxord)) != 0:
            raise IdaHipError("set_max_ord(%d) rejected" % maxord)

    def solve(self, tout, itask=0, max_rounds=0):
        tret = np.zeros(self.ctx.batch)
        status = np.zeros(self.ctx.batch, dtype=np.int32)
        rc = self.E.idaens_solve(self.h, float(tout), int(itask), _p(tret), _p(status, i32p), int(max_rounds))
        if rc < 0:
            self.ctx.fail("idaens_solve failed (%d): %s" % (rc, self.E.idaens_last_error(self.h).decode()))
        return status, tret

    def solve_schedule(self, touts, max_rounds=0, outputs=False):
        touts = _f64(np.atleast_1d(touts))
        B, n = self.ctx.batch, self.ctx.n
        tret = np.zeros(B)
        status = np.zeros(B, dtype=np.int32)
        reached = np.zeros(B, dtype=np.int32)
        yo = np.full((touts.size, B, n), np.nan) if outputs else None
        ypo = np.full((touts.size, B, n), np.nan) if outputs else None
        rc = self.E.idaens_solve_schedule(self.h, _p(touts), touts.size, _p(tret), _p(status, i32p), _p(reached, i32p),
                                          _p(yo) if outputs else None, _p(ypo) if outputs else None, int(max_rounds))
        if rc < 0:
            self.ctx.fail("idaens_solve_schedule failed (%d): %s" % (rc, (self.E.idaens_last_error(self.h) or b"").decode()))
        return (status, tret, reached, yo, ypo) if outputs else (status, tret, reached)

    def stream(self, touts, max_rounds, stagger_rounds=0):
        touts = _f64(np.atleast_1d(touts))
        done = C.c_int64(0)
        rc = self.E.idaens_stream(self.h, _p(touts), touts.size, int(max_rounds), int(stagger_rounds), C.byref(done))
        if rc < 0:
            self.ctx.fail("idaens_stream failed (%d): %s" % (rc, (self.E.idaens_last_error(self.h) or b"").decode()))
        return done.value

    def counter(self, name):
        out = np.zeros(self.ctx.batch, dtype=np.int64)
        assert self.E.idaens_get_counter(self.h, COUNTERS[name], _p(out, i64p)) == 0
        return out

    def counters(self):
        return {k: self.counter(k) for k in COUNTERS}

    def real(self, name):
        out = np.zeros(self.ctx.batch)
        assert self.E.idaens_get_real(self.h, REALS[name], _p(out)) == 0
        return out

    def yy(self):
        out = np.empty((self.ctx.batch, self.ctx.n))
        assert self.E.idaens_get_yy(self.h, _p(out)) == 0
        return out

    def yp(self):
        out = np.empty((self.ctx.batch, self.ctx.n))
        assert self.E.idaens_get_yp(self.h, _p(out)) == 0
        return out

    def get_dky(self, t, k):
        out = np.full((self.ctx.batch, self.ctx.n), np.nan)
        status = np.zeros(self.ctx.batch, dtype=np.int32)
        rc = self.E.idaens_get_dky(self.h, float(t), int(k), _p(out), _p(status, i32p))
        if rc < 0:
            self.ctx.fail("idaens_get_dky failed (%d): %s" % (rc, (self.E.idaens_last_error(self.h) or b"").decode()))
        return status, out

    def total_newton_iters(self):
        return int(self.E.idaens_total_newton_iters(self.h))

    def total_rounds(self):
        return int(self.E.idaens_total_rounds(self.h))

    def trace_system(self, sys):
        self.E.idaens_trace_system(self.h, int(sys))

    def trace(self):
        k = self.E.idaens_trace_len(self.h)
        out = np.zeros((k, 3))
        if k:
            self.E.idaens_trace_get(self.h, _p(out))
        return out


def _group_handles(ensembles):
    arr = (C.c_void_p * len(ensembles))(*[e.h for e in ensembles])
    return arr


def stream_group(ensembles, touts, max_rounds, stagger_rounds=0, offset_us=0):
    touts = _f64(np.atleast_1d(touts))
    E = ensembles[0].E
    done = np.zeros(len(ensembles), dtype=np.int64)
    rc = E.idaens_stream_group(_group_handles(ensembles), len(ensembles), _p(touts), touts.size, int(max_rounds), int(stagger_rounds),
                               int(offset_us), _p(done, i64p))
    if rc < 0:
        texts = [(e.E.idaens_last_error(e.h) or b"").decode() for e in ensembles]
        raise IdaHipError("idaens_stream_group failed (%d): %s" % (rc, " | ".join(t for t in texts if t)))
    return done


def solve_schedule_group(ensembles, touts, max_rounds=0):
    touts = _f64(np.atleast_1d(touts))
    E = ensembles[0].E
    G = len(ensembles)
    tret = [np.zeros(e.ctx.batch) for e in ensembles]
    status = [np.zeros(e.ctx.batch, dtype=np.int32) for e in ensembles]
    reached = [np.zeros(e.ctx.batch, dtype=np.int32) for e in ensembles]
    pt = (dp * G)(*[_p(a) for a in tret])
    ps = (i32p * G)(*[_p(a, i32p) for a in status])
    pr = (i32p * G)(*[_p(a, i32p) for a in reached])
    rc = E.idaens_solve_schedule_group(_group_handles(ensembles), G, _p(touts), touts.size, pt, ps, pr, int(max_rounds))
    if rc < 0:
        texts = [(e.E.idaens_last_error(e.h) or b"").decode() for e in ensembles]
        raise IdaHipError("idaens_solve_schedule_group failed (%d): %s" % (rc, " | ".join(t for t in texts if t)))
    return list(zip(status, tret, reached))


def concurrent_streams(count, device=0):
    H, _ = load()
    arr = (C.c_void_p * count)()
    nc = C.c_int(0)
    rc = H.idahip_concurrent_streams(int(device), int(count), arr, C.byref(nc))
    if rc != 0:
        raise IdaHipError("idahip_concurrent_streams failed (%d)" % rc)
    return [C.c_void_p(arr[i]) for i in range(count)], nc.value


def release_streams(streams, device=0):
    H, _ = load()
    arr = (C.c_void_p * len(streams))(*[s.value if isinstance(s, C.c_void_p) else s for s in streams])
    H.idahip_release_streams(int(device), len(streams), arr)


def stream_pair_share(a, b, device=0):
    H, _ = load()
    f = C.c_double(0.0)
    rc = H.idahip_stream_pair_share(int(device), a, b, C.byref(f))
    if rc != 0:
        raise IdaHipError("idahip_stream_pair_share failed (%d)" % rc)
    return f.value
```

Before: 358,000.

## Add opt-in 4-wave trailing-update LU kernel and compact slow-path wavepanel launch

Adds a `MAXROWS<=512` variant of the 64-wide trailing-update kernel, selected by a new `lu_trail4` switch that is off by default. It uses 8-column L chunks with a two-deep register ring, buffer loads and stores, L11 read from global instead of shared memory, and direct U12 writes. The default kernel also changes: the per-strip loop is restructured into chunked L prefetching, pivot rows come from a lane permute, and the info early-exit is moved after the shared barrier. The slow-path wavepanel launch now uses one block per 64 systems and loops only over the flagged matrices, instead of launching one mostly idle block per system. The goals are fewer empty launches, better latency hiding in the trailing update, and higher occupancy, at the cost of extra code complexity and possible register pressure.

Measured after the change: 334,100. -6.7%, worse.

```diff
diff --git a/bindings/rust/ida-hip-sys/src/lib.rs b/bindings/rust/ida-hip-sys/src/lib.rs
--- a/bindings/rust/ida-hip-sys/src/lib.rs
+++ b/bindings/rust/ida-hip-sys/src/lib.rs
@@ -205,6 +205,8 @@
     pub fn idahip_lu_variant(ctx: *const idahip_ctx) -> c_int;
     pub fn idahip_set_lu_superpanel(ctx: *mut idahip_ctx, on: c_int) -> c_int;
     pub fn idahip_lu_superpanel(ctx: *const idahip_ctx) -> c_int;
+    pub fn idahip_set_lu_trail4(ctx: *mut idahip_ctx, on: c_int) -> c_int;
+    pub fn idahip_lu_trail4(ctx: *const idahip_ctx) -> c_int;
     pub fn idahip_set_lu_period(ctx: *mut idahip_ctx, rounds: c_int) -> c_int;
     pub fn idahip_lu_period(ctx: *const idahip_ctx) -> c_int;
     pub fn idahip_timing_build() -> c_int;
diff --git a/include/ida_hip.h b/include/ida_hip.h
--- a/include/ida_hip.h
+++ b/include/ida_hip.h
@@ -141,6 +141,8 @@
 int idahip_lu_variant(const idahip_ctx* ctx);
 int idahip_set_lu_superpanel(idahip_ctx* ctx, int on);
 int idahip_lu_superpanel(const idahip_ctx* ctx);
+int idahip_set_lu_trail4(idahip_ctx* ctx, int on);
+int idahip_lu_trail4(const idahip_ctx* ctx);
 int idahip_set_lu_period(idahip_ctx* ctx, int rounds);
 int idahip_lu_period(const idahip_ctx* ctx);
 int idahip_timing_build(void);
diff --git a/rust-ida_amd/csrc/common.hpp b/rust-ida_amd/csrc/common.hpp
--- a/rust-ida_amd/csrc/common.hpp
+++ b/rust-ida_amd/csrc/common.hpp
@@ -18,6 +18,8 @@
 constexpr int MXORDP1 = 6;
 constexpr int TINY_N = 8;
 constexpr int LU_NB = 32;
+constexpr int LU_TRAIL4_MAX_N = 512;
+constexpr int LU_TRAIL4_DEFAULT = 0;
 constexpr int LU_MAX_N = 1024;
 constexpr int LU_WIDE_ROWS = 2048;
 constexpr int LU_ZMAP_MIN_N = 2048;
@@ -67,6 +69,7 @@
     double* dky = nullptr;
     int lu_variant = 4;
     int lu_superpanel = 0;
+    int lu_trail4 = idahip::LU_TRAIL4_DEFAULT;
     int lu_period = 1;
 
     void* tiny_sys = nullptr;
diff --git a/rust-ida_amd/csrc/idahip.hip b/rust-ida_amd/csrc/idahip.hip
--- a/rust-ida_amd/csrc/idahip.hip
+++ b/rust-ida_amd/csrc/idahip.hip
@@ -111,6 +111,7 @@
     c->list_seen.assign(((size_t)batch + 63) / 64, 0);
     c->lu_superpanel = kind == IDAHIP_HEAT1D ? 1 : 0;
     if (const char* sp = std::getenv("IDAHIP_LU_SUPERPANEL")) c->lu_superpanel = std::strtol(sp, nullptr, 10) != 0 ? 1 : 0;
+    if (const char* t4 = std::getenv("IDAHIP_LU_TRAIL4")) c->lu_trail4 = std::strtol(t4, nullptr, 10) != 0 ? 1 : 0;
     if (const char* sp = std::getenv("IDAHIP_LU_PERIOD")) {
         const int v = (int)std::strtol(sp, nullptr, 10);
         if (v >= 1 && v <= 64) c->lu_period = v;
@@ -1724,6 +1725,12 @@
     return 0;
 }
 int idahip_lu_superpanel(const idahip_ctx* c) { return c ? c->lu_superpanel : -1; }
+int idahip_set_lu_trail4(idahip_ctx* c, int on) {
+    if (!c) return -1;
+    c->lu_trail4 = on != 0 ? 1 : 0;
+    return 0;
+}
+int idahip_lu_trail4(const idahip_ctx* c) { return c ? c->lu_trail4 : -1; }
 int idahip_set_lu_period(idahip_ctx* c, int rounds) {
     if (!c || rounds < 1 || rounds > 64) return -1;
     c->lu_period = rounds;
diff --git a/rust-ida_amd/csrc/lu_driver.hpp b/rust-ida_amd/csrc/lu_driver.hpp
--- a/rust-ida_amd/csrc/lu_driver.hpp
+++ b/rust-ida_amd/csrc/lu_driver.hpp
@@ -81,7 +81,7 @@
             KTimer kt(c, IDAHIP_K_LU_PANEL, nsys);
             const int ns = (n - k0 + 63) / 64;
 #define IDAHIP_WP_LAUNCH(NSV) \
-    hipLaunchKernelGGL((lu_wavepanel_kernel<false, NSV>), dim3(nsys), dim3(64), 0, c->stream, w, k0)
+    hipLaunchKernelGGL((lu_wavepanel_kernel<false, NSV>), dim3(nsys), dim3(64), 0, c->stream, w, k0, nsys)
 #define IDAHIP_WP_SWITCH()                                                                                    \
     switch (ns) {                                                                                              \
         case 1: IDAHIP_WP_LAUNCH(1); break;                                                                 \
@@ -94,7 +94,7 @@
         default: IDAHIP_WP_LAUNCH(8); break;                                                                \
     }
             IDAHIP_WP_SWITCH()
-            hipLaunchKernelGGL((lu_wavepanel_kernel<true, 0>), dim3(nsys), dim3(64), 0, c->stream, w, k0);
+            hipLaunchKernelGGL((lu_wavepanel_kernel<true, 0>), dim3((nsys + 63) / 64), dim3(64), 0, c->stream, w, k0, nsys);
 #undef IDAHIP_WP_SWITCH
 #undef IDAHIP_WP_LAUNCH
         } else {
@@ -117,7 +117,9 @@
                 const int nbs = nsplit > 1 ? std::min(ncb, LU_SPLIT_BLOCKS) : 0;
                 hipLaunchKernelGGL(lu_u12_zero_kernel, dim3(nsys8 * ncb), dim3(256), 0, c->stream, w, k0, nsys, ncb);
                 hipLaunchKernelGGL(lu_trail64w_kernel<LU_BIG_MAX_N>, dim3(nsys8 * (ncb + (nsplit - 1) * nbs)), dim3(256), 0, c->stream, w, k0, nsys, ncb, nsplit);
-            } else
+            } else if (n <= LU_TRAIL4_MAX_N && c->lu_trail4)
+                hipLaunchKernelGGL(lu_trail64w_kernel<LU_TRAIL4_MAX_N>, dim3(nsys8 * ncb), dim3(256), 0, c->stream, w, k0, nsys, ncb, 1);
+            else
                 hipLaunchKernelGGL(lu_trail64w_kernel<LU_MAX_N>, dim3(nsys8 * ncb), dim3(256), 0, c->stream, w, k0, nsys, ncb, 1);
         }
     }
diff --git a/rust-ida_amd/csrc/lu_kernels.hpp b/rust-ida_amd/csrc/lu_kernels.hpp
--- a/rust-ida_amd/csrc/lu_kernels.hpp
+++ b/rust-ida_amd/csrc/lu_kernels.hpp
@@ -784,8 +784,13 @@
 }
 
 template <int MAXROWS>
-__global__ __launch_bounds__(256, MAXROWS <= 1024 ? 3 : 2) void lu_trail64w_kernel(LuWs w, int k0, int nsys, int ncb, int nsplit_arg) {
-    constexpr int NB = 64, KC = 32;
+__global__ __launch_bounds__(256, MAXROWS <= 512 ? 4 : MAXROWS <= 1024 ? 3 : 2) void lu_trail64w_kernel(LuWs w, int k0, int nsys, int ncb, int nsplit_arg) {
+    constexpr int NB = 64, TS = 32;
+    constexpr bool FOUR = MAXROWS <= 512;
+    constexpr int KC = FOUR ? 8 : 32;
+    constexpr int NCH = NB / KC;
+    constexpr int LD_RING = FOUR ? 2 : 1;
+    constexpr int LDU = 64 + (FOUR ? 0 : tb::US_PAD);
     constexpr bool NOPRO = tb::NOPRO;
     const int nsplit = MAXROWS > 1024 ? nsplit_arg : 1;
     const int nbs = nsplit > 1 ? (ncb < LU_SPLIT_BLOCKS ? ncb : LU_SPLIT_BLOCKS) : 0;
@@ -795,9 +800,10 @@
     const int sm = slot % wpm, mi = (slot / wpm) * 8 + xcd;
     const int cbi = sm < ncb ? sm : (sm - ncb) / hs;
     const int split = sm < ncb ? 0 : 1 + (sm - ncb) % hs;
+    const int b = ldc(w.idx + (mi < nsys ? mi : nsys - 1));
     if (mi >= (w.cnt ? ldc(w.cnt) : nsys)) return;
-    const int b = w.idx[mi];
-    if (w.info[b] != 0) return;
+    const int info_b = ldc(w.info + b);
+    if (MAXROWS > 1024 && info_b != 0) return;
     if (MAXROWS > 1024 && ldc(w.bz + b * 64 + cbi) == 0) return;
     int nsp = 1;
     if (nsplit > 1) {
@@ -827,8 +833,10 @@
 #define TSTAMP(i) do { if (tb::STAMPS >= 0 && tst && t == 0) tst[i] = wall_clock64(); } while (0)
     TSTAMP(0);
 
-    __shared__ __align__(16) double Us[NB][64 + tb::US_PAD];
-    __shared__ __align__(16) double Ls[KC][64];
+    constexpr int LS_ROWS = FOUR ? KC : TS;
+    __shared__ __align__(16) double s_ul[NB * LDU + LS_ROWS * 64];
+    double (*__restrict__ Us)[LDU] = reinterpret_cast<double (*)[LDU]>(&s_ul[0]);
+    double (*__restrict__ Ls)[64] = reinterpret_cast<double (*)[64]>(&s_ul[NB * LDU]);
     __shared__ unsigned short s_live[MAXROWS];
     __shared__ int s_anyzero;
     __shared__ int s_nz[4];
@@ -849,20 +857,27 @@
         cok[j] = cj < ncols;
         coff[j] = (cb0 + (cok[j] ? cj : 0)) * n;
     }
+    const __amdgpu_buffer_rsrc_t rsrc = __builtin_amdgcn_make_buffer_rsrc(A, 0, FOUR ? n * n * 8 : 0, 0x00020000);
     constexpr int LPT = KC / 4;
     const int kq = lane >> 4, lr16 = lane & 15;
     const int lslot = 4 * (lr16 & 3) + (lr16 >> 2);
-    double lreg[LPT], creg[4][4];
+    double lreg[LD_RING][LPT], creg[4][4];
     int crow[4];
     bool rok[4];
 
-    auto load_L = [&](int s, int h) {
+    auto load_L = [&](const int s, const int h, const int d) __attribute__((always_inline)) {
         const int lr = s * 16 + lr16;
         const int lrow = s_live[lr < mrem ? lr : mrem - 1];
-#pragma unroll
-        for (int i = 0; i < LPT; ++i) lreg[i] = A[(k0 + h * KC + 4 * i + kq) * n + lrow];
+        if constexpr (FOUR) {
+            const unsigned lo = (unsigned)((k0 + kq) * n + lrow) * 8u;
+#pragma unroll
+            for (int i = 0; i < LPT; ++i) lreg[d][i] = buf_load_f64(rsrc, lo, (h * KC + 4 * i) * n * 8);
+        } else {
+#pragma unroll
+            for (int i = 0; i < LPT; ++i) lreg[d][i] = A[(k0 + h * KC + 4 * i + kq) * n + lrow];
+        }
     };
-    auto load_C = [&](int s) {
+    auto load_C = [&](const int s) __attribute__((always_inline)) {
 #pragma unroll
         for (int i = 0; i < 4; ++i) {
             const int ri = s * 16 + a + 4 * i;
@@ -872,9 +887,16 @@
 #pragma unroll
         for (int j = 0; j < 4; ++j)
 #pragma unroll
-            for (int i = 0; i < 4; ++i) creg[i][j] = A[coff[j] + crow[i]];
+            for (int i = 0; i < 4; ++i) {
+                if constexpr (FOUR) creg[i][j] = buf_load_f64(rsrc, (unsigned)(coff[j] + crow[i]) * 8u, 0);
+                else creg[i][j] = A[coff[j] + crow[i]];
+            }
     };
-
+    auto load_first = [&](const int s) __attribute__((always_inline)) {
+        load_C(s);
+#pragma unroll
+        for (int d = 0; d < LD_RING; ++d) load_L(s, d, d);
+    };
 
     __shared__ int s_fz[4];
     bool fast_ok = false;
@@ -886,11 +908,12 @@
 #pragma unroll
         for (int i = 0; i < 16; ++i) l11r[i] = l11[i * 256 + t];
         {
+            const int prv = prow[lane];
             const double* __restrict__ colp = A + (long)(cb0 + (real ? qc : 0)) * n;
 #pragma unroll
             for (int i = 0; i < 16; ++i) {
-                const int p0 = ldc(prow + 4 * i), p1 = ldc(prow + 4 * i + 1), p2 = ldc(prow + 4 * i + 2), p3 = ldc(prow + 4 * i + 3);
-                const int pr = part == 0 ? p0 : part == 1 ? p1 : part == 2 ? p2 : p3;
+                int pr = __builtin_amdgcn_ds_bpermute(4 * (4 * i + part), prv);
+                pr = (unsigned)pr < (unsigned)n ? pr : 0;
                 if constexpr (tb::NOGATHER) u[i] = 1.0e-3 * (double)(1 + ((i + pr) & 7));
                 else u[i] = colp[pr];
             }
@@ -903,11 +926,9 @@
         }
         if (t == 0) s_anyzero = 0;
         lds_barrier();
+        if (info_b != 0) return;
         TSTAMP(1);
-        if (s0 < nstrips) {
-            load_C(s0);
-            load_L(s0, 0);
-        }
+        if (s0 < nstrips) load_first(s0);
         const double* __restrict__ Lp = Lq + part * 16 + 2 * (part >> 1);
         bool anyz = false;
         static_for<0, 64>([&](auto kt) {
@@ -933,12 +954,20 @@
             const int qpl = 4 * (qc & 15) + (qc >> 4);
 #pragma unroll
             for (int i = 0; i < 16; ++i) Us[4 * i + part][qpl] = real ? u[i] : 0.0;
+            if constexpr (FOUR) {
+                if (real && split == 0) {
+                    double* __restrict__ Oc = w.out + (long)b * w.ostride + (long)(cb0 + qc) * n + k0 + part;
+#pragma unroll
+                    for (int i = 0; i < 16; ++i) Oc[4 * i] = u[i];
+                }
+            }
         }
         lds_barrier();
         TSTAMP(3);
       }
     }
     if (!fast_ok) {
+    if (MAXROWS <= 1024 && info_b != 0) return;
     bool nz = NOPRO;
     if (NOPRO) {
 #pragma unroll
@@ -967,11 +996,17 @@
     if (__ballot(nz) != 0ull && lane == 0) s_nz[wave] = 1;
     if (t == 0) s_anyzero = 0;
     auto stage_l11 = [&](const int R0) {
-#pragma unroll
-        for (int i = 0; i < (KC * 64) / 256; ++i) {
-            const int e = i * 256 + t;
-            Ls[e >> 6][e & 63] = l11[(R0 + (e >> 6)) * NB + (e & 63)];
-        }
+        if constexpr (!FOUR) {
+#pragma unroll
+            for (int i = 0; i < (TS * 64) / 256; ++i) {
+                const int e = i * 256 + t;
+                Ls[e >> 6][e & 63] = l11[(R0 + (e >> 6)) * NB + (e & 63)];
+            }
+        }
+    };
+    auto l11s = [&](const int R0, const int kk, const int col) -> double {
+        if constexpr (FOUR) return ldc(l11 + (R0 + kk) * NB + col);
+        else return Ls[kk][col];
     };
     if (MAXROWS <= 1024 && !NOPRO) stage_l11(0);
     lds_barrier();
@@ -991,39 +1026,39 @@
         lds_barrier();
     }
     auto trsm32 = [&](const int R0) {
-        double u[KC];
-#pragma unroll
-        for (int k = 0; k < KC; ++k) u[k] = Us[R0 + k][pl];
+        double u[TS];
+#pragma unroll
+        for (int k = 0; k < TS; ++k) u[k] = Us[R0 + k][pl];
         const bool real = lane < ncols;
         bool anyz = false;
 #pragma unroll
-        for (int kk = 0; kk < KC; ++kk) {
+        for (int kk = 0; kk < TS; ++kk) {
             const double ukk = u[kk];
             const bool z = real && (ukk == 0.0);
             anyz = anyz || z;
             if (__ballot(z) == 0ull) {
 #pragma unroll
-                for (int k = 0; k < KC; ++k)
-                    if (k > kk) u[k] = upd(u[k], ukk, Ls[kk][R0 + k]);
+                for (int k = 0; k < TS; ++k)
+                    if (k > kk) u[k] = upd(u[k], ukk, l11s(R0, kk, R0 + k));
             } else if (MAXROWS > 1024 && __ballot(real && !z) == 0ull) {
             } else {
 #pragma unroll
-                for (int k = 0; k < KC; ++k)
+                for (int k = 0; k < TS; ++k)
                     if (k > kk) {
-                        const double tn = upd(u[k], ukk, Ls[kk][R0 + k]);
+                        const double tn = upd(u[k], ukk, l11s(R0, kk, R0 + k));
                         u[k] = z ? u[k] : tn;
                     }
             }
         }
 #pragma unroll
-        for (int k = 0; k < KC; ++k) Us[R0 + k][pl] = u[k];
+        for (int k = 0; k < TS; ++k) Us[R0 + k][pl] = u[k];
         unsigned km = 0xffffffffu;
         unsigned long long cm = ~0ull;
         if (__ballot(anyz) != 0ull || s_anyzero != 0) {
             km = 0u;
             bool cnz = false;
 #pragma unroll
-            for (int k = 0; k < KC; ++k) {
+            for (int k = 0; k < TS; ++k) {
                 const bool e = real && u[k] != 0.0;
                 cnz = cnz || e;
                 km |= (__ballot(e) != 0ull) ? (1u << k) : 0u;
@@ -1031,61 +1066,57 @@
             cm = __ballot(cnz);
         }
         if (lane == 0) {
-            s_kmask[R0 / KC] = km;
-            s_cmask[R0 / KC] = cm;
+            s_kmask[R0 / TS] = km;
+            s_cmask[R0 / TS] = cm;
             if (__ballot(anyz) != 0ull) s_anyzero = 1;
         }
     };
 
     if (wave == 0 && !NOPRO) trsm32(0);
     else if (s0 < nstrips) {
-        load_C(s0);
-        load_L(s0, 0);
+        load_first(s0);
     }
     lds_barrier();
     if (!NOPRO) {
         const bool zpath = s_anyzero != 0;
         double v[8];
 #pragma unroll
-        for (int i = 0; i < 8; ++i) v[i] = Us[KC + wave * 8 + i][pl];
+        for (int i = 0; i < 8; ++i) v[i] = Us[TS + wave * 8 + i][pl];
         if (!zpath) {
 #pragma unroll
-            for (int kk = 0; kk < KC; ++kk) {
+            for (int kk = 0; kk < TS; ++kk) {
                 const double ut = Us[kk][pl];
 #pragma unroll
-                for (int i = 0; i < 8; ++i) v[i] = upd(v[i], ut, Ls[kk][KC + wave * 8 + i]);
+                for (int i = 0; i < 8; ++i) v[i] = upd(v[i], ut, l11s(0, kk, TS + wave * 8 + i));
             }
         } else {
 #pragma unroll 4
-            for (int kk = 0; kk < KC; ++kk) {
+            for (int kk = 0; kk < TS; ++kk) {
                 const double ut = Us[kk][pl];
                 if (MAXROWS > 1024 && __ballot(ut != 0.0) == 0ull) continue;
 #pragma unroll
                 for (int i = 0; i < 8; ++i) {
-                    const double tn = upd(v[i], ut, Ls[kk][KC + wave * 8 + i]);
+                    const double tn = upd(v[i], ut, l11s(0, kk, TS + wave * 8 + i));
                     v[i] = (ut != 0.0) ? tn : v[i];
                 }
             }
         }
 #pragma unroll
-        for (int i = 0; i < 8; ++i) Us[KC + wave * 8 + i][pl] = v[i];
+        for (int i = 0; i < 8; ++i) Us[TS + wave * 8 + i][pl] = v[i];
     }
     if (!NOPRO) {
     lds_barrier();
-    stage_l11(KC);
+    stage_l11(TS);
     lds_barrier();
     if (wave == 0) {
-        trsm32(KC);
-        if (s0 < nstrips) {
-            load_C(s0);
-            load_L(s0, 0);
-        }
+        trsm32(TS);
+        if (s0 < nstrips) load_first(s0);
     }
     }
     lds_barrier();
     }
     const bool slow = s_anyzero != 0;
-    if (split == 0) {
+    if (split == 0 && !(FOUR && fast_ok)) {
         double* __restrict__ O = w.out + (long)b * w.ostride;
 #pragma unroll 4
         for (int i = 0; i < 16; ++i) {
@@ -1113,7 +1144,7 @@
                         if (u != 0.0) v = upd(v, u, A[(long)(k0 + kk) * n + row]);
                     }
                     for (unsigned mk = kmask1; mk != 0u; mk &= mk - 1u) {
-                        const int kk = KC + __builtin_ctz(mk);
+                        const int kk = TS + __builtin_ctz(mk);
                         const double u = Us[kk][cs];
                         if (u != 0.0) v = upd(v, u, A[(long)(k0 + kk) * n + row]);
                     }
@@ -1125,8 +1156,8 @@
     }
     double (*__restrict__ Lw)[16] = reinterpret_cast<double (*)[16]>(&Ls[0][0] + wave * (KC * 16));
 
-    auto chunk = [&](double (&c)[4][4], const int kbase) {
-        if (!slow) {
+    auto chunk = [&](const bool slowp, double (&c)[4][4], const int kbase) __attribute__((always_inline)) {
+        if (!slowp) {
             double lvA[4], uvA[4], lvB[4], uvB[4];
             auto rd = [&](const int k, double (&lv)[4], double (&uv)[4]) {
 #pragma unroll
@@ -1159,7 +1190,8 @@
                 }
             }
         } else {
-            for (unsigned mk = kbase == 0 ? kmask0 : kmask1; mk != 0u; mk &= mk - 1u) {
+            const unsigned kmc = ((kbase < TS ? kmask0 : kmask1) >> (kbase % TS)) & (KC >= 32 ? 0xffffffffu : (1u << (KC % 32)) - 1u);
+            for (unsigned mk = kmc; mk != 0u; mk &= mk - 1u) {
                 const int k = __builtin_ctz(mk);
                 double lv[4], uv[4];
 #pragma unroll
@@ -1177,41 +1209,71 @@
         }
     };
 
+    auto strips = [&](const bool slowp) __attribute__((always_inline)) {
 #pragma unroll 1
     for (int s = s0; s < nstrips; s += sstep) {
-#pragma unroll
-        for (int i = 0; i < LPT; ++i) Lw[4 * i + kq][lslot] = lreg[i];
-        load_L(s, 1);
         double c[4][4];
         int srow[4];
         bool sok[4];
 #pragma unroll
-        for (int i = 0; i < 4; ++i) {
-            srow[i] = crow[i];
-            sok[i] = rok[i];
-#pragma unroll
-            for (int j = 0; j < 4; ++j) c[i][j] = creg[i][j];
-        }
-        if constexpr (tb::STAMPS >= 0) {
-            if (s == s0) { asm volatile("s_waitcnt vmcnt(0)" ::: "memory"); TSTAMP(5); }
-        }
-        chunk(c, 0);
-        if constexpr (tb::STAMPS >= 0) {
-            if (s == s0) TSTAMP(6);
-        }
-#pragma unroll
-        for (int i = 0; i < LPT; ++i) Lw[4 * i + kq][lslot] = lreg[i];
-        if (s + sstep < nstrips) {
+        for (int h = 0; h < NCH; ++h) {
+            const int d = h % LD_RING;
+#pragma unroll
+            for (int i = 0; i < LPT; ++i) Lw[4 * i + kq][lslot] = lreg[d][i];
+            if (h == NCH / 2 && !FOUR) {
+                if (s + sstep < nstrips) load_C(s + sstep);
+            }
+            if (h + LD_RING < NCH) {
+                load_L(s, h + LD_RING, d);
+            } else {
+                if (FOUR || s + sstep < nstrips) load_L(s + sstep, h + LD_RING - NCH, d);
+            }
+            if (h == 0) {
+#pragma unroll
+                for (int i = 0; i < 4; ++i) {
+                    if constexpr (!FOUR) {
+                        srow[i] = crow[i];
+                        sok[i] = rok[i];
+                    }
+#pragma unroll
+                    for (int j = 0; j < 4; ++j) c[i][j] = creg[i][j];
+                }
+                if constexpr (tb::STAMPS >= 0) {
+                    if (s == s0) { asm volatile("s_waitcnt vmcnt(0)" ::: "memory"); TSTAMP(5); }
+                }
+            }
+            chunk(slowp, c, h * KC);
+#pragma unroll
+            for (int j = 0; j < 4; ++j)
+#pragma unroll
+                for (int i = 0; i < 4; ++i) c[i][j] = opaque_vgpr(c[i][j]);
+            if constexpr (tb::STAMPS >= 0) {
+                if (h == NCH / 2 - 1 && s == s0) TSTAMP(6);
+            }
+        }
+#pragma unroll
+        for (int j = 0; j < 4; ++j)
+#pragma unroll
+            for (int i = 0; i < 4; ++i)
+                if constexpr (!FOUR) {
+                    if (cok[j] && sok[i]) A[coff[j] + srow[i]] = c[i][j];
+                }
+        if constexpr (FOUR) {
+#pragma unroll
+            for (int i = 0; i < 4; ++i) {
+                const int ri = s * 16 + a + 4 * i;
+                const bool ok = ri < mrem;
+                const int row = s_live[ok ? ri : mrem - 1];
+#pragma unroll
+                for (int j = 0; j < 4; ++j)
+                    if (cok[j] && ok) buf_store_f64(rsrc, (unsigned)(coff[j] + row) * 8u, 0, c[i][j]);
+            }
             load_C(s + sstep);
-            load_L(s + sstep, 0);
-        }
-        chunk(c, KC);
-#pragma unroll
-        for (int j = 0; j < 4; ++j)
-#pragma unroll
-            for (int i = 0; i < 4; ++i)
-                if (cok[j] && sok[i]) A[coff[j] + srow[i]] = c[i][j];
-    }
+        }
+    }
+    };
+    if (slow) strips(true);
+    else strips(false);
     TSTAMP(7);
 #undef TSTAMP
 }
diff --git a/rust-ida_amd/csrc/lu_wavepanel.hpp b/rust-ida_amd/csrc/lu_wavepanel.hpp
--- a/rust-ida_amd/csrc/lu_wavepanel.hpp
+++ b/rust-ida_amd/csrc/lu_wavepanel.hpp
@@ -9,10 +9,9 @@
 constexpr int WP_RING(int ns) { return !tb::WP_DEEP_RING ? 2 : (ns >= 1 && ns <= 2) ? 8 : (ns >= 3 && ns <= 7) ? 4 : 2; }
 
 template <bool SLOWK, int NS>
-__global__ __launch_bounds__(64, SLOWK ? 1 : (NS > 0 && NS <= 3 ? 4 : 2)) void lu_wavepanel_kernel(LuWs w, const int k0) {
+__device__ __forceinline__ void lu_wavepanel_matrix(const LuWs& w, const int k0, const int mi) {
     constexpr int BIG = 1 << 20;
-    if (w.cnt && (int)blockIdx.x >= *w.cnt) return;
-    const int b = w.idx[blockIdx.x];
+    const int b = w.idx[mi];
     if (w.info[b] != 0) return;
     const int n = w.n;
     double* __restrict__ A = w.mats + (long)b * w.mstride;
@@ -355,4 +354,23 @@
     });
 }
 
+template <bool SLOWK, int NS>
+__global__ __launch_bounds__(64, SLOWK ? 1 : (NS > 0 && NS <= 3 ? 4 : 2)) void lu_wavepanel_kernel(LuWs w, const int k0, const int nsys) {
+    if constexpr (!SLOWK) {
+        if (w.cnt && (int)blockIdx.x >= *w.cnt) return;
+        lu_wavepanel_matrix<false, NS>(w, k0, (int)blockIdx.x);
+    } else {
+        const int len = w.cnt ? *w.cnt : nsys;
+        const int mine = (int)blockIdx.x * 64 + (int)threadIdx.x;
+        bool flagged = false;
+        if (mine < len && mine < nsys) {
+            const int b = w.idx[mine];
+            flagged = w.info[b] == 0 && w.redo[b] != 0;
+        }
+#pragma unroll 1
+        for (unsigned long long m = __ballot(flagged); m != 0ull; m &= m - 1ull)
+            lu_wavepanel_matrix<true, NS>(w, k0, (int)blockIdx.x * 64 + __builtin_ctzll(m));
+    }
 }
+
+}
diff --git a/rust-ida_amd/idahip/__init__.py b/rust-ida_amd/idahip/__init__.py
--- a/rust-ida_amd/idahip/__init__.py
+++ b/rust-ida_amd/idahip/__init__.py
@@ -32,7 +32,7 @@
     "idahip_predict", "idahip_post_newton", "idahip_restore", "idahip_complete_step", "idahip_get_solution", "idahip_get_dky",
     "idahip_timing_enable", "idahip_timing_get", "idahip_timing_reset", "idahip_set_lu_variant", "idahip_snapshot_initial",
     "idahip_tiny_solve", "idahip_pow_batch", "idahip_round_solve", "idahip_lu_variant",
-    "idahip_restore_initial", "idahip_ls_type", "idahip_ls_num_iters", "idahip_ls_res_norm", "idahip_timing_build", "idahip_concurrent_streams", "idahip_release_streams", "idahip_stream_pair_share", "idahip_set_lu_superpanel", "idahip_lu_superpanel", "idahip_set_lu_period", "idahip_lu_period",
+    "idahip_restore_initial", "idahip_ls_type", "idahip_ls_num_iters", "idahip_ls_res_norm", "idahip_timing_build", "idahip_concurrent_streams", "idahip_release_streams", "idahip_stream_pair_share", "idahip_set_lu_superpanel", "idahip_lu_superpanel", "idahip_set_lu_trail4", "idahip_lu_trail4", "idahip_set_lu_period", "idahip_lu_period",
     "idahip_create_band", "idahip_band", "idahip_set_host_band_problem", "idahip_download_lu_band", "idahip_ls_setup_band", "idahip_ls_solve_band",
     "idahip_set_jacobian_dq", "idahip_jacobian_dq", "idahip_set_host_residual", "idahip_jac_dq", "idahip_nls_lsetup_dq",
 ]
@@ -86,6 +86,8 @@
     H.idahip_stream_pair_share.argtypes = [ci, vp, vp, C.POINTER(cd)]
     H.idahip_set_lu_superpanel.argtypes = [vp, ci]
     H.idahip_lu_superpanel.argtypes = [vp]
+    H.idahip_set_lu_trail4.argtypes = [vp, ci]
+    H.idahip_lu_trail4.argtypes = [vp]
     H.idahip_set_lu_period.argtypes = [vp, ci]
     H.idahip_lu_period.argtypes = [vp]
     H.idahip_last_error.argtypes = [vp]
@@ -523,6 +525,12 @@
     def lu_superpanel(self):
         return int(self.H.idahip_lu_superpanel(self.h))
 
+    def set_lu_trail4(self, on):
+        self._chk(self.H.idahip_set_lu_trail4(self.h, int(on)), "set_lu_trail4")
+
+    def lu_trail4(self):
+        return int(self.H.idahip_lu_trail4(self.h))
+
     def set_lu_period(self, rounds):
         self._chk(self.H.idahip_set_lu_period(self.h, int(rounds)), "set_lu_period")
 
```
